# syzhang092218-source/dgppo

Measured on AMD Instinct MI355X. Metric: env-steps/sec whole node, LidarSpread n=8 4096 envs, 1/2/4/8 GPUs, higher is better.
Workload: dtype f32

## Files before the change

dgppo_amd/csrc/attn.hip:

```cpp
#include "nn_attn.h"

static int32_t attn_check(const dgppo_env_cfg* cfg, int F, int H, int Kp, int G, AttnArgs& a) {
  int32_t rc = dgppo_validate_cfg(cfg);
  if (rc) return rc;
  a.t = make_topo(*cfg);
  DGPPO_REQUIRE(F >= 1 && F <= 64 && H >= 1 && H <= 8, "attn: bad F=%d H=%d", F, H);
  DGPPO_REQUIRE(Kp >= F + H * (F + 4) + 1, "attn: Kp=%d too small", Kp);
  DGPPO_REQUIRE(G >= 0, "attn: G < 0");
  a.F = F; a.H = H; a.Kp = Kp; a.G = G;
  return 0;
}

enum class AttnFamily { SLOT8, BD, MFMA, VALU, TILED };
size_t attn_image_bytes(const Topo& t, int F, int H, bool bwd) {
  if (bwd)
    return sizeof(float) * ((size_t)t.Ns * (F + 1) + (size_t)t.n * H * (F + 1) + (size_t)t.n * t.S * 4 + 2 * (size_t)t.n * t.S * H +
                            (size_t)t.n * H * (F + 5));
  return sizeof(float) * ((size_t)t.Ns * (F + 1) + (size_t)t.n * H * (F + 1) + (size_t)t.n * t.S * 5 + (size_t)t.n * t.S * H);
}
static AttnFamily attn_family(const Topo& t, int F, int H, int Kp, bool bwd, bool dXa) {
  int PS = 0;
  bool hits = false;
  if (attn_image_bytes(t, F, H, bwd) > 64 * 1024) return AttnFamily::TILED;
  if ((Kp & 3) == 0 && attn_slot8_shape(t, F, H) && !(bwd && dXa)) return AttnFamily::SLOT8;
  if ((Kp & 3) == 0 && attn_bd_shape(t, F, H, PS, hits)) return AttnFamily::BD;
  if ((F & 3) == 0 && (Kp & 3) == 0 && t.S <= 64 && attn_mfma_smem(t, F, H, bwd) <= 64 * 1024 && (!bwd || F >= 16)) return AttnFamily::MFMA;
  return AttnFamily::VALU;
}

static int32_t attn_launch(AttnFamily fam, AttnArgs& a, void* stream, bool bwd, const char* who) {
  const hipStream_t s = (hipStream_t)stream;
  bool launched = true;
  switch (fam) {
    case AttnFamily::SLOT8: launched = launch_attn_slot8(a, s, bwd); break;
    case AttnFamily::BD: launched = launch_attn_bd(a, s, bwd); break;
    case AttnFamily::MFMA: launch_attn_wg(a, s, bwd, true); break;
    case AttnFamily::VALU: launch_attn_wg(a, s, bwd, false); break;
    case AttnFamily::TILED: {
      const int32_t rc = launch_attn_tiled(a, s, bwd);
      if (rc) return rc;
      break;
    }
  }
  DGPPO_REQUIRE(launched, "%s: dispatch failed", who);
  DGPPO_LAUNCH_CHECK();
  return 0;
}
static void attn_set_fwd(AttnArgs& a, const float* qt, const float* Xa, const float* Xo, const float* efeat, const float* emask,
                         float* zcat, float* attn) {
  a.qt = qt; a.Xa = Xa; a.Xo = Xo; a.efeat = efeat; a.emask = emask; a.zcat = zcat; a.attn = attn;
}
static void attn_set_bwd(AttnArgs& a, const float* dzcat, const float* attn, const float* qt, const float* Xa, const float* Xo,
                         const float* efeat, float* dqt, float* dXa, float* dXo) {
  a.dzcat = dzcat; a.attn = (float*)attn; a.qt = qt; a.Xa = Xa; a.Xo = Xo; a.efeat = efeat; a.dqt = dqt; a.dXa = dXa; a.dXo = dXo;
}

extern "C" int32_t dgppo_attn_fwd(const dgppo_env_cfg* cfg, int32_t F, int32_t H, int32_t Kp, const float* qt,
                                  const float* Xa, const float* Xo, const float* efeat, const float* emask, float* zcat,
                                  float* attn, int32_t G, void* stream) {
  AttnArgs a{};
  int32_t rc = attn_check(cfg, F, H, Kp, G, a);
  if (rc) return rc;
  if (G == 0) return 0;
  DGPPO_REQUIRE(qt && Xa && efeat && emask && zcat, "attn_fwd: NULL operand");
  DGPPO_REQUIRE(a.t.Ns == a.t.n || Xo, "attn_fwd: Xo is NULL");
  attn_set_fwd(a, qt, Xa, Xo, efeat, emask, zcat, attn);
  return attn_launch(attn_family(a.t, F, H, Kp, false, false), a, stream, false, "attn_fwd");
}

extern "C" int32_t dgppo_attn_bwd(const dgppo_env_cfg* cfg, int32_t F, int32_t H, int32_t Kp, const float* dzcat,
                                  const float* attn, const float* qt, const float* Xa, const float* Xo,
                                  const float* efeat, float* dqt, float* dXa, float* dXo, int32_t relu_xo, int32_t G,
                                  void* stream) {
  AttnArgs a{};
  int32_t rc = attn_check(cfg, F, H, Kp, G, a);
  if (rc) return rc;
  if (G == 0) return 0;
  DGPPO_REQUIRE(dzcat && attn && qt && Xa && efeat && dqt, "attn_bwd: NULL operand");
  DGPPO_REQUIRE(a.t.Ns == a.t.n || Xo, "attn_bwd: Xo is NULL");
  DGPPO_REQUIRE(!(dXo && !dXa), "attn_bwd: dXo needs dXa");
  attn_set_bwd(a, dzcat, attn, qt, Xa, Xo, efeat, dqt, dXa, dXo);
  const AttnFamily fam = attn_family(a.t, F, H, Kp, true, dXa != nullptr);
  a.relu_xo = (relu_xo && dXo && fam == AttnFamily::BD) ? 1 : 0;
  rc = attn_launch(fam, a, stream, true, "attn_bwd");
  if (rc) return rc;
  if (relu_xo && dXo && !a.relu_xo)
    return dgppo_relu_bwd(dXo, Xo, (int64_t)G * (a.t.Ns - a.t.n) * F, stream);
  return 0;
}

static bool attn_xo_ok(const Topo& t, int F, int H, int Kp) {
  return t.Ns > t.n && attn_family(t, F, H, Kp, true, true) == AttnFamily::BD;
}
extern "C" int32_t dgppo_attn_xo_supported(const dgppo_env_cfg* cfg, int32_t F, int32_t H, int32_t Kp) {
  AttnArgs a{};
  if (attn_check(cfg, F, H, Kp, 0, a)) return 0;
  return attn_xo_ok(a.t, F, H, Kp) ? 1 : 0;
}
static int32_t attn_set_xo(AttnArgs& a, const float* Xo_raw, const float* Wo, int ldwo, const float* bo, const char* who) {
  DGPPO_REQUIRE(attn_xo_ok(a.t, a.F, a.H, a.Kp), "%s: no fused kernel for this topology (ask dgppo_attn_xo_supported)", who);
  a.Xo_raw = Xo_raw; a.Wo = Wo; a.ldwo = ldwo; a.bo = bo;
  return 0;
}
extern "C" int32_t dgppo_attn_fwd_xo(const dgppo_env_cfg* cfg, int32_t F, int32_t H, int32_t Kp, const float* qt, const float* Xa,
                                     const float* Xo_raw, const float* Wo, int32_t ldwo, const float* bo, const float* efeat,
                                     const float* emask, float* zcat, float* attn, int32_t G, void* stream) {
  AttnArgs a{};
  int32_t rc = attn_check(cfg, F, H, Kp, G, a);
  if (rc) return rc;
  if (G == 0) return 0;
  DGPPO_REQUIRE(qt && Xa && Xo_raw && Wo && bo && efeat && emask && zcat, "attn_fwd_xo: NULL operand");
  DGPPO_REQUIRE(ldwo >= 32, "attn_fwd_xo: ldwo=%d < 32", ldwo);
  rc = attn_set_xo(a, Xo_raw, Wo, ldwo, bo, "attn_fwd_xo");
  if (rc) return rc;
  attn_set_fwd(a, qt, Xa, nullptr, efeat, emask, zcat, attn);
  return attn_launch(AttnFamily::BD, a, stream, false, "attn_fwd_xo");
}
extern "C" int32_t dgppo_attn_bwd_xo(const dgppo_env_cfg* cfg, int32_t F, int32_t H, int32_t Kp, const float* dzcat,
                                     const float* attn, const float* qt, const float* Xa, const float* Xo_raw, const float* Wo,
                                     int32_t ldwo, const float* bo, const float* efeat, float* dqt, float* dXa, float* dXo,
                                     int32_t relu_xo, int32_t G, void* stream) {
  AttnArgs a{};
  int32_t rc = attn_check(cfg, F, H, Kp, G, a);
  if (rc) return rc;
  if (G == 0) return 0;
  DGPPO_REQUIRE(dzcat && attn && qt && Xa && Xo_raw && Wo && bo && efeat && dqt, "attn_bwd_xo: NULL operand");
  DGPPO_REQUIRE(ldwo >= 32, "attn_bwd_xo: ldwo=%d < 32", ldwo);
  DGPPO_REQUIRE(!(dXo && !dXa), "attn_bwd_xo: dXo needs dXa");
  rc = attn_set_xo(a, Xo_raw, Wo, ldwo, bo, "attn_bwd_xo");
  if (rc) return rc;
  attn_set_bwd(a, dzcat, attn, qt, Xa, nullptr, efeat, dqt, dXa, dXo);
  a.relu_xo = (relu_xo && dXo) ? 1 : 0;
  return attn_launch(AttnFamily::BD, a, stream, true, "attn_bwd_xo");
}

static bool attn_rows_ok(const dgppo_env_cfg& c, const Topo& t, int F, int H, int Kp) {
  return attn_slot8_rows_ok(c, t, F, H) && attn_family(t, F, H, Kp, false, false) == AttnFamily::SLOT8 &&
         attn_family(t, F, H, Kp, true, false) == AttnFamily::SLOT8;
}
extern "C" int32_t dgppo_attn_rows_supported(const dgppo_env_cfg* cfg, int32_t F, int32_t H) {
  AttnArgs a{};
  const int Kp = (F + H * (F + 4) + 1 + 3) / 4 * 4;
  if (F < 1 || H < 1 || attn_check(cfg, F, H, Kp, 0, a)) return 0;
  return attn_rows_ok(*cfg, a.t, F, H, Kp) ? 1 : 0;
}
extern "C" int32_t dgppo_attn_fwd_rows(const dgppo_env_cfg* cfg, int32_t F, int32_t H, int32_t Kp, const float* qt,
                                       const float* Xa, const float* Xo, const float* emask, float* zcat, float* attn,
                                       int32_t G, void* stream) {
  AttnArgs a{};
  int32_t rc = attn_check(cfg, F, H, Kp, G, a);
  if (rc) return rc;
  DGPPO_REQUIRE(attn_rows_ok(*cfg, a.t, F, H, Kp), "attn_fwd_rows: no such kernel for this configuration (ask dgppo_attn_rows_supported)");
  if (G == 0) return 0;
  DGPPO_REQUIRE(qt && Xa && emask && zcat, "attn_fwd_rows: NULL operand");
  DGPPO_REQUIRE(a.t.Ns == a.t.n || Xo, "attn_fwd_rows: Xo is NULL");
  attn_set_fwd(a, qt, Xa, Xo, nullptr, emask, zcat, attn);
  return attn_launch(AttnFamily::SLOT8, a, stream, false, "attn_fwd_rows");
}
extern "C" int32_t dgppo_attn_bwd_rows(const dgppo_env_cfg* cfg, int32_t F, int32_t H, int32_t Kp, const float* dzcat,
                                       const float* attn, const float* qt, const float* emask, const float* Xa, const float* Xo,
                                       float* dqt, int32_t G, void* stream) {
  AttnArgs a{};
  int32_t rc = attn_check(cfg, F, H, Kp, G, a);
  if (rc) return rc;
  DGPPO_REQUIRE(attn_rows_ok(*cfg, a.t, F, H, Kp), "attn_bwd_rows: no such kernel for this configuration (ask dgppo_attn_rows_supported)");
  if (G == 0) return 0;
  DGPPO_REQUIRE(dzcat && Xa && dqt, "attn_bwd_rows: NULL operand");
  DGPPO_REQUIRE(attn || (qt && emask), "attn_bwd_rows: without attn the weights need qt and emask");
  DGPPO_REQUIRE(a.t.Ns == a.t.n || Xo, "attn_bwd_rows: Xo is NULL");
  attn_set_bwd(a, dzcat, attn, qt, Xa, Xo, nullptr, dqt, nullptr, nullptr);
  a.emask = emask;
  return attn_launch(AttnFamily::SLOT8, a, stream, true, "attn_bwd_rows");
}

extern "C" int64_t dgppo_attn_xo_workspace_bytes(int32_t G) { return G < 0 ? 0 : (int64_t)G * ABD_DW_STRIDE * (int64_t)sizeof(float); }
extern "C" int32_t dgppo_attn_bwd_xo_dw(const dgppo_env_cfg* cfg, int32_t F, int32_t H, int32_t Kp, const float* dzcat,
                                        const float* attn, const float* qt, const float* Xa, const float* Xo_raw, const float* Wo,
                                        int32_t ldwo, const float* bo, const float* efeat, float* dqt, float* dXa, float* dWo,
                                        int32_t lddwo, float* dbo, float* workspace, int64_t workspace_bytes, int32_t G,
                                        void* stream) {
  AttnArgs a{};
  int32_t rc = attn_check(cfg, F, H, Kp, G, a);
  if (rc) return rc;
  if (G == 0) return 0;
  DGPPO_REQUIRE(dzcat && attn && qt && Xa && Xo_raw && Wo && bo && efeat && dqt && dXa && dWo && dbo && workspace,
                "attn_bwd_xo_dw: NULL operand");
  DGPPO_REQUIRE(ldwo >= 32 && lddwo >= 32, "attn_bwd_xo_dw: ldwo=%d lddwo=%d < 32", ldwo, lddwo);
  DGPPO_REQUIRE(workspace_bytes >= dgppo_attn_xo_workspace_bytes(G) && (reinterpret_cast<uintptr_t>(workspace) & 15) == 0,
                "attn_bwd_xo_dw: workspace too small or not 16-byte aligned");
  rc = attn_set_xo(a, Xo_raw, Wo, ldwo, bo, "attn_bwd_xo_dw");
  if (rc) return rc;
  attn_set_bwd(a, dzcat, attn, qt, Xa, nullptr, efeat, dqt, dXa, nullptr);
  a.relu_xo = 1;
  a.dwo_slab = workspace;
  const bool launched = launch_attn_bd(a, (hipStream_t)stream, true);
  DGPPO_REQUIRE(launched, "attn_bwd_xo_dw: dispatch failed");
  launch_attn_xo_dw_reduce(workspace, G, dWo, lddwo, dbo, (hipStream_t)stream);
  DGPPO_LAUNCH_CHECK();
  return 0;
}
```

dgppo_amd/csrc/attn_bd.hip:

```cpp
#include "nn_attn.h"

#ifdef DGPPO_STAMPS
__device__ unsigned long long g_astamps[32];
#define ASTAMP(i) do { if (blockIdx.x == 0 && threadIdx.x == 0) g_astamps[i] = __builtin_amdgcn_s_memtime(); } while (0)
extern "C" int32_t dgppo_debug_stamps_attn(unsigned long long* out) {
  return (int32_t)hipMemcpyFromSymbol(out, HIP_SYMBOL(g_astamps), sizeof(unsigned long long) * 32);
}
#else
#define ASTAMP(i)
#endif

#define ABD_XL 36
#define ABD_DZL 40
__device__ inline f32x4g mfma4(float a_, float b_, f32x4g c_) { return __builtin_amdgcn_mfma_f32_4x4x1f32(a_, b_, c_, 0, 0, 0); }
__device__ inline const float* f4e(const float4& v) { return reinterpret_cast<const float*>(&v); }

__device__ inline int opaque_zero(int bits) {
  asm("v_and_b32 %0, 0, %0" : "+v"(bits));
  return bits;
}
__device__ inline int f4bits(const float4& v) { return __float_as_int(v.x) | __float_as_int(v.y) | __float_as_int(v.z) | __float_as_int(v.w); }

template <int PS, bool HITS> struct AbdLds {
  static constexpr int NSP = PS * 8, PC = NSP + (HITS ? 8 : 0), PL = PC + 4;
  static constexpr int XS = NSP * ABD_XL, XH = HITS ? 64 * ABD_XL + 64 : 0;
  static constexpr int QP = (32 * ABD_XL > 32 * PL) ? 32 * ABD_XL : 32 * PL;
  static constexpr int FWD = XS + XH + QP;
  static constexpr int DZ = 32 * ABD_DZL, PTL = NSP + 1, PT = 32 * PTL, DL = 32 * PL;
  static constexpr int BWD = XS + XH + DZ + PT + DL;
};

#define ABD_KR 8
template <int GT> struct AbdXoRegs { float ag[GT][2], ah[4][2], wo[2][2], bo[2]; };
template <int GT, bool HITS>
__device__ inline void abd_xo_load(AbdXoRegs<GT>& x, const AttnArgs& a, const float* raw, int n_shared_other, int ng, int hit0,
                                   int n_hits, int li, int lq, bool first) {
  if (first) {
#pragma unroll
    for (int s_ = 0; s_ < 2; ++s_)
#pragma unroll
      for (int ct = 0; ct < 2; ++ct) x.wo[s_][ct] = a.Wo[(lq + 4 * s_) * a.ldwo + ct * 16 + li];
#pragma unroll
    for (int ct = 0; ct < 2; ++ct) x.bo[ct] = a.bo[ct * 16 + li];
#pragma unroll
    for (int t = 0; t < GT; ++t) {
      int o = t * 16 + li;
      o = o < n_shared_other ? o : n_shared_other - 1;
      o = o < 0 ? 0 : o;
#pragma unroll
      for (int s_ = 0; s_ < 2; ++s_) x.ag[t][s_] = raw[o * ABD_KR + lq + 4 * s_];
    }
  }
  if constexpr (HITS) {
#pragma unroll
    for (int t = 0; t < 4; ++t) {
      int hb = hit0 + t * 16 + li;
      hb = hb < n_hits ? hb : n_hits - 1;
#pragma unroll
      for (int s_ = 0; s_ < 2; ++s_) x.ah[t][s_] = raw[(ng + hb) * ABD_KR + lq + 4 * s_];
    }
  }
}
template <int GT, bool HITS>
__device__ inline void abd_xo_emit(const AbdXoRegs<GT>& x, float* XS, float* XH, int n, int n_shared_other, int li, int lq, bool first) {
  auto tile = [&](const float (&ar)[2], f32x4g (&v)[2]) {
#pragma unroll
    for (int ct = 0; ct < 2; ++ct) {
      v[ct] = f32x4g{0.f, 0.f, 0.f, 0.f};
      v[ct] = __builtin_amdgcn_mfma_f32_16x16x4f32(ar[0], x.wo[0][ct], v[ct], 0, 0, 0);
      v[ct] = __builtin_amdgcn_mfma_f32_16x16x4f32(ar[1], x.wo[1][ct], v[ct], 0, 0, 0);
    }
  };
  if (first) {
#pragma unroll
    for (int t = 0; t < GT; ++t) {
      f32x4g v[2];
      tile(x.ag[t], v);
#pragma unroll
      for (int ct = 0; ct < 2; ++ct)
#pragma unroll
        for (int r = 0; r < 4; ++r) {
          const int o = t * 16 + lq * 4 + r;
          if (o < n_shared_other) XS[(n + o) * ABD_XL + ct * 16 + li] = relu_nan(v[ct][r] + x.bo[ct]);
        }
    }
  }
  if constexpr (HITS) {
#pragma unroll
    for (int t = 0; t < 4; ++t) {
      f32x4g v[2];
      tile(x.ah[t], v);
#pragma unroll
      for (int ct = 0; ct < 2; ++ct)
#pragma unroll
        for (int r = 0; r < 4; ++r) {
          const int hr = t * 16 + lq * 4 + r;
          XH[hr * ABD_XL + (hr >> 3) * 8 + ct * 16 + li] = relu_nan(v[ct][r] + x.bo[ct]);
        }
    }
  }
}
template <int GT> __device__ inline int abd_xo_bits(const AbdXoRegs<GT>& x, bool hits) {
  int b = 0;
#pragma unroll
  for (int t = 0; t < GT; ++t) b |= __float_as_int(x.ag[t][0]) | __float_as_int(x.ag[t][1]);
  if (hits) {
#pragma unroll
    for (int t = 0; t < 4; ++t) b |= __float_as_int(x.ah[t][0]) | __float_as_int(x.ah[t][1]);
  }
  b |= __float_as_int(x.wo[0][0]) | __float_as_int(x.wo[0][1]) | __float_as_int(x.wo[1][0]) | __float_as_int(x.wo[1][1]);
  b |= __float_as_int(x.bo[0]) | __float_as_int(x.bo[1]);
  return b;
}

template <int PS, bool HITS>
__device__ __forceinline__ int abd_slot(const Topo& t, int NSH, int ic, int p, int sub) {
  if (HITS && p == PS) return t.n + t.gs + sub;
  const int j = p * 8 + sub;
  return (j < NSH) ? slot_of(t, j, ic) : -1;
}

template <int PS, bool HITS, int AB, bool XOF>
__global__ void __launch_bounds__(128) attn_fwd_bd_kernel(AttnArgs a) {
  extern __shared__ float4 abd_sm[];
  using L = AbdLds<PS, HITS>;
  constexpr int F = 32, NSP = L::NSP, PC = L::PC, PL = L::PL, NPR = PS + (HITS ? 1 : 0), Wd = F + 4;
  const Topo& t = a.t;
  const int lane = threadIdx.x & 63, wave = threadIdx.x >> 6;
  const int g = __builtin_amdgcn_readfirstlane(blockIdx.x * 2 + wave);
  if (g >= a.G) return;
  const int n = t.n, S = t.S, Ns = t.Ns, H = a.H, Kp = a.Kp;
  const int NSH = HITS ? t.n + t.ng : Ns;
  const int kc = F + H * Wd;
  float* XS = reinterpret_cast<float*>(abd_sm) + wave * L::FWD;
  float* XH = XS + L::XS;
  float* QP = XH + L::XH;
  const float4* Xa4 = reinterpret_cast<const float4*>(a.Xa + (size_t)g * n * F);
  const float4* Xo4 = reinterpret_cast<const float4*>(a.Xo + (size_t)g * (Ns - n) * F);
  const float4* qt4 = reinterpret_cast<const float4*>(a.qt + (size_t)g * n * H * F);
  float* zc = a.zcat + (size_t)g * n * Kp;
  const int il = lane >> 3, sub = lane & 7, g2 = (lane >> 2) & 1, c = lane & 3, hA = lane & 3;
  ASTAMP(0);
  float4 vs[PS];
#pragma unroll
  for (int p = 0; p < PS; ++p) {
    const int row = p * 8 + il;
    const int ra = row < n ? row : n - 1, ro = (row < NSH ? row : NSH - 1) - n;
    const float4* src = (XOF || row < n || NSH == n) ? Xa4 + ra * 8 + sub : Xo4 + ro * 8 + sub;
    vs[p] = *src;
  }
  constexpr int GT = (NSP + 15) / 16;
  AbdXoRegs<GT> xo;
  const float* raw = XOF ? a.Xo_raw + (size_t)g * (Ns - n) * ABD_KR : nullptr;
  const int li_ = lane & 15, lq_ = lane >> 4;
  const float* mk = a.emask + (size_t)g * n * S;
  const float4* ef4 = reinterpret_cast<const float4*>(a.efeat + (size_t)g * n * S * 4);
  float* at = a.attn + (size_t)g * n * S * H;
#pragma unroll
  for (int ab = 0; ab < AB; ++ab) {
    const int i = ab * 8 + il;
    const bool live = i < n;
    const int ic = live ? i : n - 1;
    float4 vh[HITS ? 8 : 1], vq[4];
    if constexpr (XOF) abd_xo_load<GT, HITS>(xo, a, raw, NSH - n, t.ng, ab * 64, n * 8, li_, lq_, ab == 0);
    if constexpr (HITS && !XOF) {
#pragma unroll
      for (int k = 0; k < 8; ++k) {
        int hb = ab * 64 + k * 8 + il;
        hb = hb < n * 8 ? hb : n * 8 - 1;
        vh[k] = Xo4[(t.ng + hb) * 8 + sub];
      }
    }
#pragma unroll
    for (int k = 0; k < 4; ++k) {
      const int row = k * 8 + il;
      int ri = ab * 8 + (row >> 2), rh = row & 3;
      ri = ri < n ? ri : n - 1; rh = rh < H ? rh : H - 1;
      vq[k] = qt4[(ri * H + rh) * 8 + sub];
    }
    int slot[NPR];
    float mkv[NPR];
    float4 efv[NPR];
#pragma unroll
    for (int p = 0; p < NPR; ++p) {
      const int sl = abd_slot<PS, HITS>(t, NSH, ic, p, sub);
      slot[p] = live ? sl : -1;
      const int sc = sl < 0 ? 0 : sl;
      mkv[p] = mk[ic * S + sc];
      efv[p] = ef4[ic * S + sc];
    }
    ASTAMP(1);
    int pin = 0;
#pragma unroll
    for (int p = 0; p < NPR; ++p) pin |= __float_as_int(mkv[p]) | f4bits(efv[p]);
    if constexpr (XOF) pin |= abd_xo_bits<GT>(xo, HITS);
    const int pin0 = opaque_zero(pin);
    if (ab == 0) {
#pragma unroll
      for (int p = 0; p < PS; ++p) {
        float4 v = vs[p];
        if (XOF && p * 8 + il >= n) v = make_float4(0.f, 0.f, 0.f, 0.f);
        *reinterpret_cast<float4*>(XS + pin0 + (p * 8 + il) * ABD_XL + sub * 4) = v;
      }
    }
    if constexpr (XOF) abd_xo_emit<GT, HITS>(xo, XS + pin0, XH + pin0, n, NSH - n, li_, lq_, ab == 0);
    if constexpr (HITS && !XOF) {
#pragma unroll
      for (int k = 0; k < 8; ++k) *reinterpret_cast<float4*>(XH + pin0 + (k * 8 + il) * ABD_XL + k * 8 + sub * 4) = vh[k];
    }
#pragma unroll
    for (int k = 0; k < 4; ++k) *reinterpret_cast<float4*>(QP + pin0 + (k * 8 + il) * ABD_XL + sub * 4) = vq[k];
#pragma unroll
    for (int p = 0; p < NPR; ++p) mkv[p] = (slot[p] >= 0) ? mkv[p] : 0.0f;
    if constexpr (HITS) {
      if (mkv[PS] == 0.0f) {
#pragma unroll
        for (int k = 0; k < 8; ++k) *reinterpret_cast<float4*>(XH + lane * ABD_XL + il * 8 + k * 4) = make_float4(0.f, 0.f, 0.f, 0.f);
      }
    }
    ASTAMP(2);
    f32x4g acc[NPR];
#pragma unroll
    for (int p = 0; p < NPR; ++p) acc[p] = f32x4g{0.f, 0.f, 0.f, 0.f};
    {
      const float* qrow = QP + (il * 4 + hA) * ABD_XL;
#pragma unroll
      for (int k = 0; k < 8; ++k) {
        const float4 q = *reinterpret_cast<const float4*>(qrow + k * 4);
        float4 x[NPR];
#pragma unroll
        for (int p = 0; p < NPR; ++p) {
          if (HITS && p == PS) x[p] = *reinterpret_cast<const float4*>(XH + lane * ABD_XL + il * 8 + k * 4);
          else x[p] = *reinterpret_cast<const float4*>(XS + (p * 8 + sub) * ABD_XL + k * 4);
        }
#pragma unroll
        for (int u = 0; u < 4; ++u)
#pragma unroll
          for (int p = 0; p < NPR; ++p) acc[p] = mfma4(f4e(q)[u], f4e(x[p])[u], acc[p]);
      }
    }
    ASTAMP(3);
    float* PT = QP;
#pragma unroll
    for (int h = 0; h < 4; ++h) {
      if (h < H) {
        float l[NPR];
        float mx = -INFINITY;
#pragma unroll
        for (int p = 0; p < NPR; ++p) { l[p] = (mkv[p] != 0.0f) ? acc[p][h] : -INFINITY; mx = fmaxf(mx, l[p]); }
        mx = grp8_max(mx);
        float den = 0.0f;
#pragma unroll
        for (int p = 0; p < NPR; ++p) { l[p] = (l[p] == -INFINITY) ? 0.0f : __expf(l[p] - mx); den += l[p]; }
        den = grp8_sum(den);
        const float inv = (den > 0.0f) ? 1.0f / den : 0.0f;
        float z0 = 0.f, z1 = 0.f, z2 = 0.f, z3 = 0.f;
#pragma unroll
        for (int p = 0; p < NPR; ++p) {
          const float av = l[p] * inv;
          acc[p][h] = av;
          if (slot[p] >= 0) {
            if (a.attn != nullptr) at[(i * S + slot[p]) * H + h] = av;
            if (av != 0.0f) {
              const float4 e = efv[p];
              z0 = fmaf(av, e.x, z0); z1 = fmaf(av, e.y, z1); z2 = fmaf(av, e.z, z2); z3 = fmaf(av, e.w, z3);
            }
          }
        }
        z0 = grp8_sum(z0); z1 = grp8_sum(z1); z2 = grp8_sum(z2); z3 = grp8_sum(z3);
        if (live && sub == 0) *reinterpret_cast<float4*>(zc + i * Kp + F + h * Wd + F) = make_float4(z0, z1, z2, z3);
      } else {
#pragma unroll
        for (int p = 0; p < NPR; ++p) acc[p][h] = 0.0f;
      }
#pragma unroll
      for (int p = 0; p < NPR; ++p) PT[(il * 4 + h) * PL + p * 8 + sub] = acc[p][h];
    }
    ASTAMP(4);
    {
      float pa[PC];
#pragma unroll
      for (int k = 0; k < PC / 4; ++k) {
        const float4 v = *reinterpret_cast<const float4*>(PT + (il * 4 + hA) * PL + k * 4);
        pa[k * 4] = v.x; pa[k * 4 + 1] = v.y; pa[k * 4 + 2] = v.z; pa[k * 4 + 3] = v.w;
      }
      f32x4g az[4];
#pragma unroll
      for (int q = 0; q < 4; ++q) az[q] = f32x4g{0.f, 0.f, 0.f, 0.f};
      const int fq = (g2 * 4 + c) * 4;
#pragma unroll
      for (int kk = 0; kk < NSP; ++kk) {
        const float4 b = *reinterpret_cast<const float4*>(XS + kk * ABD_XL + fq);
#pragma unroll
        for (int q = 0; q < 4; ++q) az[q] = mfma4(pa[kk], f4e(b)[q], az[q]);
      }
      if constexpr (HITS) {
#pragma unroll
        for (int m = 0; m < 8; ++m) {
          const float4 b = *reinterpret_cast<const float4*>(XH + (il * 8 + m) * ABD_XL + il * 8 + fq);
#pragma unroll
          for (int q = 0; q < 4; ++q) az[q] = mfma4(pa[NSP + m], f4e(b)[q], az[q]);
        }
      }
      if (live) {
#pragma unroll
        for (int h = 0; h < 4; ++h)
          if (h < H) *reinterpret_cast<float4*>(zc + i * Kp + F + h * Wd + fq) = make_float4(az[0][h], az[1][h], az[2][h], az[3][h]);
      }
    }
  }
  ASTAMP(5);
#pragma unroll
  for (int p = 0; p < PS; ++p) {
    const int row = p * 8 + il;
    if (row < n) *reinterpret_cast<float4*>(zc + row * Kp + sub * 4) = *reinterpret_cast<const float4*>(XS + row * ABD_XL + sub * 4);
  }
  {
    const int wpad = Kp - kc;
    for (int i = lane; i < n; i += 64)
      for (int cc = 0; cc < wpad; ++cc) zc[i * Kp + kc + cc] = (cc == 0) ? ones_col(a.t, mk + i * S) : 0.0f;
  }
  ASTAMP(6);
}

template <int PS, bool HITS, bool XOF>
struct AbdFwdRegs {
  float4 vs[PS], vq[4], vh[(HITS && !XOF) ? 8 : 1];
  AbdXoRegs<(PS * 8 + 15) / 16> xo;
  float mkv[PS + (HITS ? 1 : 0)];
  float4 efv[PS + (HITS ? 1 : 0)];
};
template <int PS, bool HITS, bool XOF>
__global__ void __launch_bounds__(128) attn_fwd_bdp_kernel(AttnArgs a) {
  extern __shared__ float4 abd_sm[];
  using L = AbdLds<PS, HITS>;
  constexpr int F = 32, NSP = L::NSP, PC = L::PC, PL = L::PL, NPR = PS + (HITS ? 1 : 0), Wd = F + 4, GT = (NSP + 15) / 16;
  const Topo& t = a.t;
  const int lane = threadIdx.x & 63, wave = threadIdx.x >> 6;
  int g = __builtin_amdgcn_readfirstlane(blockIdx.x * 2 + wave);
  const int stride = gridDim.x * 2;
  if (g >= a.G) return;
  const int n = t.n, S = t.S, Ns = t.Ns, H = a.H, Kp = a.Kp;
  const int NSH = HITS ? t.n + t.ng : Ns;
  const int kc = F + H * Wd;
  float* XS = reinterpret_cast<float*>(abd_sm) + wave * L::FWD;
  float* XH = XS + L::XS;
  float* QP = XH + L::XH;
  const int il = lane >> 3, sub = lane & 7, g2 = (lane >> 2) & 1, c = lane & 3, hA = lane & 3;
  const int li_ = lane & 15, lq_ = lane >> 4;
  const int i = il;
  const bool live = i < n;
  const int ic = live ? i : n - 1;
  int slot[NPR], sc[NPR];
#pragma unroll
  for (int p = 0; p < NPR; ++p) {
    const int sl = abd_slot<PS, HITS>(t, NSH, ic, p, sub);
    slot[p] = live ? sl : -1;
    sc[p] = sl < 0 ? 0 : sl;
  }
  using Regs = AbdFwdRegs<PS, HITS, XOF>;
  auto load = [&](int gg, Regs& R) {
    const float4* Xa4 = reinterpret_cast<const float4*>(a.Xa + (size_t)gg * n * F);
    const float4* Xo4 = reinterpret_cast<const float4*>(a.Xo + (size_t)gg * (Ns - n) * F);
    const float4* qt4 = reinterpret_cast<const float4*>(a.qt + (size_t)gg * n * H * F);
#pragma unroll
    for (int p = 0; p < PS; ++p) {
      const int row = p * 8 + il;
      const int ra = row < n ? row : n - 1, ro = (row < NSH ? row : NSH - 1) - n;
      const float4* src = (XOF || row < n || NSH == n) ? Xa4 + ra * 8 + sub : Xo4 + ro * 8 + sub;
      R.vs[p] = *src;
    }
    if constexpr (XOF) abd_xo_load<GT, HITS>(R.xo, a, a.Xo_raw + (size_t)gg * (Ns - n) * ABD_KR, NSH - n, t.ng, 0, n * 8, li_, lq_, true);
    if constexpr (HITS && !XOF) {
#pragma unroll
      for (int k = 0; k < 8; ++k) {
        int hb = k * 8 + il;
        hb = hb < n * 8 ? hb : n * 8 - 1;
        R.vh[k] = Xo4[(t.ng + hb) * 8 + sub];
      }
    }
#pragma unroll
    for (int k = 0; k < 4; ++k) {
      const int row = k * 8 + il;
      int ri = row >> 2, rh = row & 3;
      ri = ri < n ? ri : n - 1; rh = rh < H ? rh : H - 1;
      R.vq[k] = qt4[(ri * H + rh) * 8 + sub];
    }
    const float* mk = a.emask + (size_t)gg * n * S;
    const float4* ef4 = reinterpret_cast<const float4*>(a.efeat + (size_t)gg * n * S * 4);
#pragma unroll
    for (int p = 0; p < NPR; ++p) {
      R.mkv[p] = mk[ic * S + sc[p]];
      R.efv[p] = ef4[ic * S + sc[p]];
    }
  };
  auto stage = [&](Regs& R) {
    int pin = 0;
#pragma unroll
    for (int p = 0; p < NPR; ++p) pin |= __float_as_int(R.mkv[p]) | f4bits(R.efv[p]);
    if constexpr (XOF) pin |= abd_xo_bits<GT>(R.xo, HITS);
    const int pin0 = opaque_zero(pin);
#pragma unroll
    for (int p = 0; p < PS; ++p) {
      float4 v = R.vs[p];
      if (XOF && p * 8 + il >= n) v = make_float4(0.f, 0.f, 0.f, 0.f);
      *reinterpret_cast<float4*>(XS + pin0 + (p * 8 + il) * ABD_XL + sub * 4) = v;
    }
    if constexpr (XOF) abd_xo_emit<GT, HITS>(R.xo, XS + pin0, XH + pin0, n, NSH - n, li_, lq_, true);
    if constexpr (HITS && !XOF) {
#pragma unroll
      for (int k = 0; k < 8; ++k) *reinterpret_cast<float4*>(XH + pin0 + (k * 8 + il) * ABD_XL + k * 8 + sub * 4) = R.vh[k];
    }
#pragma unroll
    for (int k = 0; k < 4; ++k) *reinterpret_cast<float4*>(QP + pin0 + (k * 8 + il) * ABD_XL + sub * 4) = R.vq[k];
#pragma unroll
    for (int p = 0; p < NPR; ++p) R.mkv[p] = (slot[p] >= 0) ? R.mkv[p] : 0.0f;
    if constexpr (HITS) {
      if (R.mkv[PS] == 0.0f) {
#pragma unroll
        for (int k = 0; k < 8; ++k) *reinterpret_cast<float4*>(XH + lane * ABD_XL + il * 8 + k * 4) = make_float4(0.f, 0.f, 0.f, 0.f);
      }
    }
  };
  auto compute = [&](int gg, const Regs& R) {
    float* zc = a.zcat + (size_t)gg * n * Kp;
    float* at = a.attn + (size_t)gg * n * S * H;
    f32x4g acc[NPR];
#pragma unroll
    for (int p = 0; p < NPR; ++p) acc[p] = f32x4g{0.f, 0.f, 0.f, 0.f};
    {
      const float* qrow = QP + (il * 4 + hA) * ABD_XL;
#pragma unroll
      for (int k = 0; k < 8; ++k) {
        const float4 q = *reinterpret_cast<const float4*>(qrow + k * 4);
        float4 x[NPR];
#pragma unroll
        for (int p = 0; p < NPR; ++p) {
          if (HITS && p == PS) x[p] = *reinterpret_cast<const float4*>(XH + lane * ABD_XL + il * 8 + k * 4);
          else x[p] = *reinterpret_cast<const float4*>(XS + (p * 8 + sub) * ABD_XL + k * 4);
        }
#pragma unroll
        for (int u = 0; u < 4; ++u)
#pragma unroll
          for (int p = 0; p < NPR; ++p) acc[p] = mfma4(f4e(q)[u], f4e(x[p])[u], acc[p]);
      }
    }
    float* PT = QP;
#pragma unroll
    for (int h = 0; h < 4; ++h) {
      if (h < H) {
        float l[NPR];
        float mx = -INFINITY;
#pragma unroll
        for (int p = 0; p < NPR; ++p) { l[p] = (R.mkv[p] != 0.0f) ? acc[p][h] : -INFINITY; mx = fmaxf(mx, l[p]); }
        mx = grp8_max(mx);
        float den = 0.0f;
#pragma unroll
        for (int p = 0; p < NPR; ++p) { l[p] = (l[p] == -INFINITY) ? 0.0f : __expf(l[p] - mx); den += l[p]; }
        den = grp8_sum(den);
        const float inv = (den > 0.0f) ? 1.0f / den : 0.0f;
        float z0 = 0.f, z1 = 0.f, z2 = 0.f, z3 = 0.f;
#pragma unroll
        for (int p = 0; p < NPR; ++p) {
          const float av = l[p] * inv;
          acc[p][h] = av;
          if (slot[p] >= 0) {
            if (a.attn != nullptr) at[(i * S + slot[p]) * H + h] = av;
            if (av != 0.0f) {
              const float4 e = R.efv[p];
              z0 = fmaf(av, e.x, z0); z1 = fmaf(av, e.y, z1); z2 = fmaf(av, e.z, z2); z3 = fmaf(av, e.w, z3);
            }
          }
        }
        z0 = grp8_sum(z0); z1 = grp8_sum(z1); z2 = grp8_sum(z2); z3 = grp8_sum(z3);
        if (live && sub == 0) *reinterpret_cast<float4*>(zc + i * Kp + F + h * Wd + F) = make_float4(z0, z1, z2, z3);
      } else {
#pragma unroll
        for (int p = 0; p < NPR; ++p) acc[p][h] = 0.0f;
      }
#pragma unroll
      for (int p = 0; p < NPR; ++p) PT[(il * 4 + h) * PL + p * 8 + sub] = acc[p][h];
    }
    {
      float pa[PC];
#pragma unroll
      for (int k = 0; k < PC / 4; ++k) {
        const float4 v = *reinterpret_cast<const float4*>(PT + (il * 4 + hA) * PL + k * 4);
        pa[k * 4] = v.x; pa[k * 4 + 1] = v.y; pa[k * 4 + 2] = v.z; pa[k * 4 + 3] = v.w;
      }
      f32x4g az[4];
#pragma unroll
      for (int q = 0; q < 4; ++q) az[q] = f32x4g{0.f, 0.f, 0.f, 0.f};
      const int fq = (g2 * 4 + c) * 4;
#pragma unroll
      for (int kk = 0; kk < NSP; ++kk) {
        const float4 b = *reinterpret_cast<const float4*>(XS + kk * ABD_XL + fq);
#pragma unroll
        for (int q = 0; q < 4; ++q) az[q] = mfma4(pa[kk], f4e(b)[q], az[q]);
      }
      if constexpr (HITS) {
#pragma unroll
        for (int m = 0; m < 8; ++m) {
          const float4 b = *reinterpret_cast<const float4*>(XH + (il * 8 + m) * ABD_XL + il * 8 + fq);
#pragma unroll
          for (int q = 0; q < 4; ++q) az[q] = mfma4(pa[NSP + m], f4e(b)[q], az[q]);
        }
      }
      if (live) {
#pragma unroll
        for (int h = 0; h < 4; ++h)
          if (h < H) *reinterpret_cast<float4*>(zc + i * Kp + F + h * Wd + fq) = make_float4(az[0][h], az[1][h], az[2][h], az[3][h]);
      }
    }
#pragma unroll
    for (int p = 0; p < PS; ++p) {
      const int row = p * 8 + il;
      if (row < n) *reinterpret_cast<float4*>(zc + row * Kp + sub * 4) = *reinterpret_cast<const float4*>(XS + row * ABD_XL + sub * 4);
    }
    {
      const int wpad = Kp - kc;
      for (int ii = lane; ii < n; ii += 64)
        for (int cc = 0; cc < wpad; ++cc) zc[ii * Kp + kc + cc] = (cc == 0) ? ones_col(a.t, a.emask + ((size_t)gg * n + ii) * a.t.S) : 0.0f;
    }
  };
  Regs cur;
  load(g, cur);
  for (;;) {
    stage(cur);
    const int gn = g + stride;
    const bool more = gn < a.G;
    Regs nxt;
    if (more) load(gn, nxt);
    compute(g, cur);
    if (!more) break;
    cur = nxt;
    g = gn;
  }
}

template <int PS, bool HITS, int AB, bool XOF>
__global__ void __launch_bounds__(64) attn_bwd_bd_kernel(AttnArgs a) {
  extern __shared__ float4 abd_sm[];
  using L = AbdLds<PS, HITS>;
  constexpr int F = 32, NSP = L::NSP, PC = L::PC, PL = L::PL, PTL = L::PTL, NPR = PS + (HITS ? 1 : 0), Wd = F + 4;
  constexpr int RTS = (NSP + 15) / 16;
  const Topo& t = a.t;
  const int lane = threadIdx.x & 63;
  const int g = blockIdx.x;
  if (g >= a.G) return;
  const int n = t.n, S = t.S, Ns = t.Ns, H = a.H, Kp = a.Kp;
  const int NSH = HITS ? t.n + t.ng : Ns;
  float* XS = reinterpret_cast<float*>(abd_sm);
  float* XH = XS + L::XS;
  float* DZ = XH + L::XH;
  float* PT = DZ + L::DZ;
  float* DL = PT + L::PT;
  const float4* Xa4 = reinterpret_cast<const float4*>(a.Xa + (size_t)g * n * F);
  const float4* Xo4 = reinterpret_cast<const float4*>(a.Xo + (size_t)g * (Ns - n) * F);
  const float* qt = a.qt + (size_t)g * n * H * F;
  const float* dzc = a.dzcat + (size_t)g * n * Kp;
  const bool want_dx = a.dXa != nullptr;
  const int il = lane >> 3, sub = lane & 7, g2 = (lane >> 2) & 1, c = lane & 3, hA = lane & 3;
  const int li = lane & 15, lq = lane >> 4;
  float4 vs[PS];
#pragma unroll
  for (int p = 0; p < PS; ++p) {
    const int row = p * 8 + il;
    const int ra = row < n ? row : n - 1, ro = (row < NSH ? row : NSH - 1) - n;
    const float4* src = (XOF || row < n || NSH == n) ? Xa4 + ra * 8 + sub : Xo4 + ro * 8 + sub;
    vs[p] = *src;
  }
  constexpr int GT = (NSP + 15) / 16;
  AbdXoRegs<GT> xo;
  const float* raw = XOF ? a.Xo_raw + (size_t)g * (Ns - n) * ABD_KR : nullptr;
  const int li_ = lane & 15, lq_ = lane >> 4;
  float dir[RTS][2][4];
#pragma unroll
  for (int rt = 0; rt < RTS; ++rt)
#pragma unroll
    for (int ft = 0; ft < 2; ++ft)
#pragma unroll
      for (int r = 0; r < 4; ++r) {
        const int node = rt * 16 + lq * 4 + r;
        dir[rt][ft][r] = dzc[(node < n ? node : n - 1) * Kp + ft * 16 + li];
      }
  f32x4g dxs[RTS][2];
#pragma unroll
  for (int rt = 0; rt < RTS; ++rt)
#pragma unroll
    for (int ft = 0; ft < 2; ++ft) dxs[rt][ft] = f32x4g{0.f, 0.f, 0.f, 0.f};
  f32x4g dwacc[2] = {f32x4g{0.f, 0.f, 0.f, 0.f}, f32x4g{0.f, 0.f, 0.f, 0.f}};
  float rbg[NSP / 4];
  const float4* ef4 = reinterpret_cast<const float4*>(a.efeat + (size_t)g * n * S * 4);
  const float* at = a.attn + (size_t)g * n * S * H;
#pragma unroll
  for (int ab = 0; ab < AB; ++ab) {
    const int i = ab * 8 + il;
    const bool live = i < n;
    const int ic = live ? i : n - 1;
    float4 vh[HITS ? 8 : 1], vz[5];
    if constexpr (XOF) abd_xo_load<GT, HITS>(xo, a, raw, NSH - n, t.ng, ab * 64, n * 8, li_, lq_, ab == 0);
    float rbh[HITS ? 16 : 1];
    if constexpr (XOF && HITS) {
#pragma unroll
      for (int s_ = 0; s_ < 16; ++s_) {
        int hb = ab * 64 + s_ * 4 + lq;
        hb = hb < n * 8 ? hb : n * 8 - 1;
        rbh[s_] = raw[(t.ng + hb) * ABD_KR + (li & 7)];
      }
    }
    if constexpr (XOF) {
      if (ab == 0) {
#pragma unroll
        for (int s_ = 0; s_ < NSP / 4; ++s_) {
          int o = s_ * 4 + lq;
          o = o < NSH - n ? o : NSH - n - 1;
          o = o < 0 ? 0 : o;
          rbg[s_] = raw[o * ABD_KR + (li & 7)];
        }
      }
    }
    if constexpr (HITS && !XOF) {
#pragma unroll
      for (int k = 0; k < 8; ++k) {
        int hb = ab * 64 + k * 8 + il;
        hb = hb < n * 8 ? hb : n * 8 - 1;
        vh[k] = Xo4[(t.ng + hb) * 8 + sub];
      }
    }
#pragma unroll
    for (int k = 0; k < 5; ++k) {
      int tt = k * 64 + lane;
      tt = tt < 288 ? tt : 287;
      const int row = tt / 9, ch = tt - row * 9;
      int ri = ab * 8 + (row >> 2), rh = row & 3;
      ri = ri < n ? ri : n - 1; rh = rh < H ? rh : H - 1;
      vz[k] = *reinterpret_cast<const float4*>(dzc + ri * Kp + F + rh * Wd + ch * 4);
    }
    int slot[NPR];
    float4 efv[NPR];
    float av[NPR][4];
#pragma unroll
    for (int p = 0; p < NPR; ++p) {
      const int sl = abd_slot<PS, HITS>(t, NSH, ic, p, sub);
      slot[p] = live ? sl : -1;
      const int sc = sl < 0 ? 0 : sl;
      efv[p] = ef4[ic * S + sc];
#pragma unroll
      for (int h = 0; h < 4; ++h) av[p][h] = at[(ic * S + sc) * H + (h < H ? h : H - 1)];
    }
    float4 q8[4][2];
    if constexpr (HITS) {
#pragma unroll
      for (int h = 0; h < 4; ++h) {
        const float4* qr = reinterpret_cast<const float4*>(qt + (size_t)(ic * H + (h < H ? h : H - 1)) * F + c * 8);
        q8[h][0] = qr[0]; q8[h][1] = qr[1];
      }
    }
    float bQ[8][2];
#pragma unroll
    for (int ks = 0; ks < 8; ++ks) {
      const int ri = ab * 8 + ks;
      const float* qr = qt + (size_t)((ri < n ? ri : n - 1) * H + (lq < H ? lq : H - 1)) * F;
#pragma unroll
      for (int ft = 0; ft < 2; ++ft) bQ[ks][ft] = qr[ft * 16 + li];
    }
    int pin = 0;
#pragma unroll
    for (int p = 0; p < NPR; ++p) {
      pin |= f4bits(efv[p]);
#pragma unroll
      for (int h = 0; h < 4; ++h) pin |= __float_as_int(av[p][h]);
    }
    if constexpr (HITS) {
#pragma unroll
      for (int h = 0; h < 4; ++h) pin |= f4bits(q8[h][0]) | f4bits(q8[h][1]);
    }
#pragma unroll
    for (int ks = 0; ks < 8; ++ks) pin |= __float_as_int(bQ[ks][0]) | __float_as_int(bQ[ks][1]);
    if (ab == 0) {
#pragma unroll
      for (int rt = 0; rt < RTS; ++rt)
#pragma unroll
        for (int ft = 0; ft < 2; ++ft)
#pragma unroll
          for (int r = 0; r < 4; ++r) pin |= __float_as_int(dir[rt][ft][r]);
    }
    if constexpr (XOF) pin |= abd_xo_bits<GT>(xo, HITS);
    if constexpr (XOF && HITS) {
#pragma unroll
      for (int s_ = 0; s_ < 16; ++s_) pin |= __float_as_int(rbh[s_]);
    }
    if constexpr (XOF) {
      if (ab == 0) {
#pragma unroll
        for (int s_ = 0; s_ < NSP / 4; ++s_) pin |= __float_as_int(rbg[s_]);
      }
    }
    const int pin0 = opaque_zero(pin);
    if (ab == 0) {
#pragma unroll
      for (int p = 0; p < PS; ++p) {
        float4 v = vs[p];
        if (XOF && p * 8 + il >= n) v = make_float4(0.f, 0.f, 0.f, 0.f);
        *reinterpret_cast<float4*>(XS + pin0 + (p * 8 + il) * ABD_XL + sub * 4) = v;
      }
    }
    if constexpr (XOF) abd_xo_emit<GT, HITS>(xo, XS + pin0, XH + pin0, n, NSH - n, li_, lq_, ab == 0);
    if constexpr (HITS && !XOF) {
#pragma unroll
      for (int k = 0; k < 8; ++k) *reinterpret_cast<float4*>(XH + pin0 + (k * 8 + il) * ABD_XL + k * 8 + sub * 4) = vh[k];
    }
#pragma unroll
    for (int k = 0; k < 5; ++k) {
      const int tt = k * 64 + lane, row = tt / 9, ch = tt - row * 9;
      if (tt < 288) *reinterpret_cast<float4*>(DZ + pin0 + row * ABD_DZL + ch * 4) = vz[k];
    }
#pragma unroll
    for (int p = 0; p < NPR; ++p)
#pragma unroll
      for (int h = 0; h < 4; ++h) av[p][h] = (slot[p] >= 0 && h < H) ? av[p][h] : 0.0f;
    if constexpr (HITS) {
      if (av[PS][0] == 0.0f && av[PS][1] == 0.0f && av[PS][2] == 0.0f && av[PS][3] == 0.0f) {
#pragma unroll
        for (int k = 0; k < 8; ++k) *reinterpret_cast<float4*>(XH + lane * ABD_XL + il * 8 + k * 4) = make_float4(0.f, 0.f, 0.f, 0.f);
      }
    }
    f32x4g acc[NPR];
#pragma unroll
    for (int p = 0; p < NPR; ++p) acc[p] = f32x4g{0.f, 0.f, 0.f, 0.f};
    {
      const float* zrow = DZ + (il * 4 + hA) * ABD_DZL;
#pragma unroll
      for (int k = 0; k < 8; ++k) {
        const float4 q = *reinterpret_cast<const float4*>(zrow + k * 4);
        float4 x[NPR];
#pragma unroll
        for (int p = 0; p < NPR; ++p) {
          if (HITS && p == PS) x[p] = *reinterpret_cast<const float4*>(XH + lane * ABD_XL + il * 8 + k * 4);
          else x[p] = *reinterpret_cast<const float4*>(XS + (p * 8 + sub) * ABD_XL + k * 4);
        }
#pragma unroll
        for (int u = 0; u < 4; ++u)
#pragma unroll
          for (int p = 0; p < NPR; ++p) acc[p] = mfma4(f4e(q)[u], f4e(x[p])[u], acc[p]);
      }
    }
#pragma unroll
    for (int h = 0; h < 4; ++h) {
      const float4 dze = *reinterpret_cast<const float4*>(DZ + (il * 4 + h) * ABD_DZL + F);
      float dot = 0.0f;
#pragma unroll
      for (int p = 0; p < NPR; ++p) {
        const float w = av[p][h];
        const float4 e = efv[p];
        const float dA = (w != 0.0f) ? acc[p][h] + fmaf(dze.x, e.x, fmaf(dze.y, e.y, fmaf(dze.z, e.z, dze.w * e.w))) : 0.0f;
        acc[p][h] = dA;
        dot = fmaf(w, dA, dot);
      }
      dot = grp8_sum(dot);
#pragma unroll
      for (int p = 0; p < NPR; ++p) {
        acc[p][h] = av[p][h] * (acc[p][h] - dot);
        DL[(il * 4 + h) * PL + p * 8 + sub] = acc[p][h];
        if (p < PS) PT[(il * 4 + h) * PTL + p * 8 + sub] = av[p][h];
      }
    }
    {
      float pa[PC];
#pragma unroll
      for (int k = 0; k < PC / 4; ++k) {
        const float4 v = *reinterpret_cast<const float4*>(DL + (il * 4 + hA) * PL + k * 4);
        pa[k * 4] = v.x; pa[k * 4 + 1] = v.y; pa[k * 4 + 2] = v.z; pa[k * 4 + 3] = v.w;
      }
      f32x4g az[4];
#pragma unroll
      for (int q = 0; q < 4; ++q) az[q] = f32x4g{0.f, 0.f, 0.f, 0.f};
      const int fq = (g2 * 4 + c) * 4;
#pragma unroll
      for (int kk = 0; kk < NSP; ++kk) {
        const float4 b = *reinterpret_cast<const float4*>(XS + kk * ABD_XL + fq);
#pragma unroll
        for (int q = 0; q < 4; ++q) az[q] = mfma4(pa[kk], f4e(b)[q], az[q]);
      }
      if constexpr (HITS) {
#pragma unroll
        for (int m = 0; m < 8; ++m) {
          const float4 b = *reinterpret_cast<const float4*>(XH + (il * 8 + m) * ABD_XL + il * 8 + fq);
#pragma unroll
          for (int q = 0; q < 4; ++q) az[q] = mfma4(pa[NSP + m], f4e(b)[q], az[q]);
        }
      }
      if (live) {
        float* dq = a.dqt + ((size_t)g * n + i) * H * F;
#pragma unroll
        for (int h = 0; h < 4; ++h)
          if (h < H) *reinterpret_cast<float4*>(dq + h * F + fq) = make_float4(az[0][h], az[1][h], az[2][h], az[3][h]);
      }
    }
    if (want_dx) {
#pragma unroll
      for (int ks = 0; ks < 8; ++ks) {
        const int prow = ks * 4 + lq;
        float bD[2];
#pragma unroll
        for (int ft = 0; ft < 2; ++ft) bD[ft] = DZ[prow * ABD_DZL + ft * 16 + li];
#pragma unroll
        for (int rt = 0; rt < RTS; ++rt) {
          const int col = (rt * 16 + li < NSP) ? rt * 16 + li : NSP - 1;
          const float aP = PT[prow * PTL + col], aL = DL[prow * PL + col];
#pragma unroll
          for (int ft = 0; ft < 2; ++ft) {
            dxs[rt][ft] = __builtin_amdgcn_mfma_f32_16x16x4f32(aP, bD[ft], dxs[rt][ft], 0, 0, 0);
            dxs[rt][ft] = __builtin_amdgcn_mfma_f32_16x16x4f32(aL, bQ[ks][ft], dxs[rt][ft], 0, 0, 0);
          }
        }
      }
      if constexpr (HITS) {
        if (a.dXo != nullptr || (XOF && a.dwo_slab != nullptr)) {
          f32x4g af[8];
#pragma unroll
          for (int q = 0; q < 8; ++q) af[q] = f32x4g{0.f, 0.f, 0.f, 0.f};
#pragma unroll
          for (int h = 0; h < 4; ++h) {
            const float4 d0 = *reinterpret_cast<const float4*>(DZ + (il * 4 + h) * ABD_DZL + c * 8);
            const float4 d1 = *reinterpret_cast<const float4*>(DZ + (il * 4 + h) * ABD_DZL + c * 8 + 4);
            const float pw = av[PS][h], dw = acc[PS][h];
#pragma unroll
            for (int q = 0; q < 4; ++q) {
              af[q] = mfma4(pw, f4e(d0)[q], af[q]);
              af[q + 4] = mfma4(pw, f4e(d1)[q], af[q + 4]);
              af[q] = mfma4(dw, f4e(q8[h][0])[q], af[q]);
              af[q + 4] = mfma4(dw, f4e(q8[h][1])[q], af[q + 4]);
            }
          }
          float4 x0[4], x1[4];
#pragma unroll
          for (int m = 0; m < 4; ++m) {
            const float* xr = XH + (il * 8 + g2 * 4 + m) * ABD_XL + il * 8 + c * 8;
            x0[m] = *reinterpret_cast<const float4*>(xr);
            x1[m] = *reinterpret_cast<const float4*>(xr + 4);
          }
          const bool to_slab = XOF && a.dwo_slab != nullptr;
#pragma unroll
          for (int m = 0; m < 4; ++m) {
            const int hb = ab * 64 + il * 8 + g2 * 4 + m;
            float4 v0 = make_float4(af[0][m], af[1][m], af[2][m], af[3][m]);
            float4 v1 = make_float4(af[4][m], af[5][m], af[6][m], af[7][m]);
            if (a.relu_xo || to_slab) {
              v0.x = x0[m].x > 0.f ? v0.x : 0.f; v0.y = x0[m].y > 0.f ? v0.y : 0.f; v0.z = x0[m].z > 0.f ? v0.z : 0.f; v0.w = x0[m].w > 0.f ? v0.w : 0.f;
              v1.x = x1[m].x > 0.f ? v1.x : 0.f; v1.y = x1[m].y > 0.f ? v1.y : 0.f; v1.z = x1[m].z > 0.f ? v1.z : 0.f; v1.w = x1[m].w > 0.f ? v1.w : 0.f;
            }
            if (to_slab) {
              float* xr = XH + (il * 8 + g2 * 4 + m) * ABD_XL + il * 8 + c * 8;
              *reinterpret_cast<float4*>(xr) = v0;
              *reinterpret_cast<float4*>(xr + 4) = v1;
            } else if (hb < n * 8) {
              float* o = a.dXo + ((size_t)g * (Ns - n) + t.ng + hb) * F + c * 8;
              *reinterpret_cast<float4*>(o) = v0;
              *reinterpret_cast<float4*>(o + 4) = v1;
            }
          }
          if constexpr (XOF) {
            if (to_slab) {
#pragma unroll
              for (int s_ = 0; s_ < 16; ++s_) {
                const int hr = s_ * 4 + lq;
                const float bv = li < 8 ? rbh[s_] : (li == 8 ? 1.0f : 0.0f);
#pragma unroll
                for (int ft = 0; ft < 2; ++ft) {
                  const float av_ = XH[hr * ABD_XL + (hr >> 3) * 8 + ft * 16 + li];
                  dwacc[ft] = __builtin_amdgcn_mfma_f32_16x16x4f32(av_, bv, dwacc[ft], 0, 0, 0);
                }
              }
            }
          }
        }
      }
    }
  }
  if (want_dx) {
    float xm[RTS][2][4];
#pragma unroll
    for (int rt = 0; rt < RTS; ++rt)
#pragma unroll
      for (int ft = 0; ft < 2; ++ft)
#pragma unroll
        for (int r = 0; r < 4; ++r) {
          const int node = rt * 16 + lq * 4 + r;
          xm[rt][ft][r] = (node < NSP) ? XS[node * ABD_XL + ft * 16 + li] : 0.0f;
        }
#pragma unroll
    for (int rt = 0; rt < RTS; ++rt)
#pragma unroll
      for (int ft = 0; ft < 2; ++ft)
#pragma unroll
        for (int r = 0; r < 4; ++r) {
          const int node = rt * 16 + lq * 4 + r, f = ft * 16 + li;
          float v = dxs[rt][ft][r];
          if (node < n) a.dXa[((size_t)g * n + node) * F + f] = v + dir[rt][ft][r];
          else if (XOF && a.dwo_slab != nullptr) {
            if (node < NSP) XS[node * ABD_XL + f] = (node < NSH && xm[rt][ft][r] > 0.0f) ? v : 0.0f;
          } else if (node < NSH && a.dXo != nullptr) {
            if (a.relu_xo) v = (xm[rt][ft][r] > 0.0f) ? v : 0.0f;
            a.dXo[((size_t)g * (Ns - n) + (node - n)) * F + f] = v;
          }
        }
    if constexpr (XOF) {
      if (a.dwo_slab != nullptr) {
        const int nsho = NSH - n;
#pragma unroll
        for (int s_ = 0; s_ < NSP / 4; ++s_) {
          const int o = s_ * 4 + lq;
          const float bv = li < 8 ? rbg[s_] : (li == 8 ? 1.0f : 0.0f);
#pragma unroll
          for (int ft = 0; ft < 2; ++ft) {
            const int node = n + o;
            const float av_ = (o < nsho && node < NSP) ? XS[(node < NSP ? node : NSP - 1) * ABD_XL + ft * 16 + li] : 0.0f;
            dwacc[ft] = __builtin_amdgcn_mfma_f32_16x16x4f32(av_, bv, dwacc[ft], 0, 0, 0);
          }
        }
        if (li <= 8) {
          float* o = a.dwo_slab + (size_t)g * ABD_DW_STRIDE + li * 32 + lq * 4;
#pragma unroll
          for (int ft = 0; ft < 2; ++ft)
            *reinterpret_cast<float4*>(o + ft * 16) = make_float4(dwacc[ft][0], dwacc[ft][1], dwacc[ft][2], dwacc[ft][3]);
        }
      }
    }
  }
}

bool attn_bd_shape(const Topo& t, int F, int H, int& PS, bool& hits) {
  if (F != 32 || H < 1 || H > 4 || t.n > 16) return false;
  const int n_priv = t.Ns - t.n - t.ng;
  hits = t.lidar && n_priv > 0;
  if (hits && (t.per != 8 || n_priv != t.n * 8)) return false;
  const int nsh = hits ? t.n + t.ng : t.Ns;
  PS = (nsh + 7) / 8;
  return PS >= 1 && PS <= 4;
}
template <int PS, bool HITS, int AB, bool XOF>
static void launch_attn_bd_x(const AttnArgs& a, hipStream_t s, bool bwd) {
  using L = AbdLds<PS, HITS>;
  if (bwd) { hipLaunchKernelGGL((attn_bwd_bd_kernel<PS, HITS, AB, XOF>), dim3(a.G), dim3(64), sizeof(float) * L::BWD, s, a); return; }
  if constexpr (AB == 1) {
    static thread_local int cap = 0;
    if (cap == 0) {
      int per_cu = 0, dev = 0, cus = 256;
      if (hipOccupancyMaxActiveBlocksPerMultiprocessor(&per_cu, reinterpret_cast<const void*>(&attn_fwd_bdp_kernel<PS, HITS, XOF>), 128,
                                                       sizeof(float) * 2 * L::FWD) != hipSuccess || per_cu < 1) per_cu = 1;
      if (hipGetDevice(&dev) != hipSuccess || hipDeviceGetAttribute(&cus, hipDeviceAttributeMultiprocessorCount, dev) != hipSuccess ||
          cus < 1) cus = 256;
      cap = per_cu * cus;
    }
    if ((a.G + 1) / 2 > 2 * cap) {
      hipLaunchKernelGGL((attn_fwd_bdp_kernel<PS, HITS, XOF>), dim3(cap), dim3(128), sizeof(float) * 2 * L::FWD, s, a);
      return;
    }
  }
  hipLaunchKernelGGL((attn_fwd_bd_kernel<PS, HITS, AB, XOF>), dim3((a.G + 1) / 2), dim3(128), sizeof(float) * 2 * L::FWD, s, a);
}
template <int PS, bool HITS, int AB>
static void launch_attn_bd_one(const AttnArgs& a, hipStream_t s, bool bwd) {
  if (a.Xo_raw != nullptr) launch_attn_bd_x<PS, HITS, AB, true>(a, s, bwd);
  else launch_attn_bd_x<PS, HITS, AB, false>(a, s, bwd);
}
bool launch_attn_bd(const AttnArgs& a, hipStream_t s, bool bwd) {
  int PS = 0;
  bool hits = false;
  if (!attn_bd_shape(a.t, a.F, a.H, PS, hits)) return false;
  const int AB = (a.t.n + 7) / 8;
  switch ((PS * 2 + (hits ? 1 : 0)) * 4 + AB) {
#define DGPPO_BD(P, HT, B) case ((P) * 2 + (HT)) * 4 + (B): launch_attn_bd_one<P, (HT) != 0, B>(a, s, bwd); return true;
    DGPPO_BD(1, 0, 1) DGPPO_BD(1, 1, 1) DGPPO_BD(2, 0, 1) DGPPO_BD(2, 1, 1) DGPPO_BD(2, 0, 2) DGPPO_BD(2, 1, 2)
    DGPPO_BD(3, 0, 1) DGPPO_BD(3, 1, 1) DGPPO_BD(3, 0, 2) DGPPO_BD(3, 1, 2)
    DGPPO_BD(4, 0, 1) DGPPO_BD(4, 1, 1) DGPPO_BD(4, 0, 2) DGPPO_BD(4, 1, 2)
#undef DGPPO_BD
    default: return false;
  }
}

__global__ void __launch_bounds__(320) attn_xo_dw_reduce_kernel(const float* slab, int G, float* dWo, int lddwo, float* dbo) {
  const int e = threadIdx.x;
  if (e >= 288) return;
  const int per = (G + gridDim.x - 1) / gridDim.x;
  const int g0 = blockIdx.x * per, g1 = min(G, g0 + per);
  float sacc[8] = {0.f, 0.f, 0.f, 0.f, 0.f, 0.f, 0.f, 0.f};
  int g = g0;
  for (; g + 7 < g1; g += 8) {
#pragma unroll
    for (int u = 0; u < 8; ++u) sacc[u] += slab[(size_t)(g + u) * ABD_DW_STRIDE + e];
  }
  for (; g < g1; ++g) sacc[0] += slab[(size_t)g * ABD_DW_STRIDE + e];
  const float sum = ((sacc[0] + sacc[1]) + (sacc[2] + sacc[3])) + ((sacc[4] + sacc[5]) + (sacc[6] + sacc[7]));
  if (g0 >= g1) return;
  if (e < 256) atomicAdd(dWo + (size_t)(e >> 5) * lddwo + (e & 31), sum);
  else atomicAdd(dbo + (e - 256), sum);
}
void launch_attn_xo_dw_reduce(const float* slab, int G, float* dWo, int lddwo, float* dbo, hipStream_t s) {
  int blocks = (G + 31) / 32;
  blocks = blocks < 1 ? 1 : (blocks > 1024 ? 1024 : blocks);
  hipLaunchKernelGGL(attn_xo_dw_reduce_kernel, dim3(blocks), dim3(320), 0, s, slab, G, dWo, lddwo, dbo);
}
```

dgppo_amd/csrc/nn_attn.h:

```cpp
#pragma once
#include "graph_topo.h"

__device__ inline int slot_of(const Topo& t, int nd, int i) {
  if (nd < t.n) return nd;
  if (nd < t.n + t.ng) {
    const int g = nd - t.n;
    return t.spread ? t.n + g : (g == i ? t.n : -1);
  }
  const int q = nd - t.n - t.ng;
  if (t.lidar) return (q / t.per == i) ? t.n + t.gs + (q - i * t.per) : -1;
  return t.n + t.gs + q;
}

__device__ inline float ones_col(const Topo& t, const float* mrow) {
  if (t.gs > 0) return 1.0f;
  for (int s = 0; s < t.S; ++s)
    if (mrow[s] != 0.0f) return 1.0f;
  return 0.0f;
}

#define ABD_DW_STRIDE 320
struct AttnArgs {
  Topo t;
  int F, H, Kp;
  const float* qt;
  const float* Xa;
  const float* Xo;
  const float* efeat;
  const float* emask;
  float* zcat;
  float* attn;
  const float* dzcat;
  float* dqt;
  float* dXa;
  float* dXo;
  int relu_xo;
  int G;
  const float* Xo_raw; const float* Wo; const float* bo; int ldwo;
  float* dwo_slab;
  int TI;
};

using f32x4g = __attribute__((ext_vector_type(4))) float;

template <typename FA, typename FB, typename FC>
__device__ inline void mfma_tiles(int RTn, int CTn, int K4, int wave, int lane, FA fa, FB fb, FC fc) {
  const int li = lane & 15, lq = lane >> 4;
  for (int tile = wave; tile < RTn * CTn; tile += 4) {
    const int rt = tile / CTn, ct = tile - rt * CTn;
    f32x4g acc = {0.f, 0.f, 0.f, 0.f};
    int k4 = 0;
    for (; k4 + 4 <= K4; k4 += 4) {
      float av[4], bv[4];
#pragma unroll
      for (int u = 0; u < 4; ++u) { av[u] = fa(rt * 16 + li, (k4 + u) * 4 + lq); bv[u] = fb((k4 + u) * 4 + lq, ct * 16 + li); }
#pragma unroll
      for (int u = 0; u < 4; ++u) acc = __builtin_amdgcn_mfma_f32_16x16x4f32(av[u], bv[u], acc, 0, 0, 0);
    }
    for (; k4 < K4; ++k4) acc = __builtin_amdgcn_mfma_f32_16x16x4f32(fa(rt * 16 + li, k4 * 4 + lq), fb(k4 * 4 + lq, ct * 16 + li), acc, 0, 0, 0);
#pragma unroll
    for (int r = 0; r < 4; ++r) fc(rt * 16 + lq * 4 + r, ct * 16 + li, acc[r]);
  }
}

__device__ inline void put4(float* d, float4 v) { d[0] = v.x; d[1] = v.y; d[2] = v.z; d[3] = v.w; }

template <int CTRL> __device__ inline float dpp_f(float v) {
  return __int_as_float(__builtin_amdgcn_update_dpp(0, __float_as_int(v), CTRL, 0xf, 0xf, false));
}
__device__ inline float grp8_sum(float v) {
  v += dpp_f<0xB1>(v);
  v += dpp_f<0x4E>(v);
  v += dpp_f<0x141>(v);
  return v;
}
__device__ inline float grp8_max(float v) {
  v = fmaxf(v, dpp_f<0xB1>(v));
  v = fmaxf(v, dpp_f<0x4E>(v));
  v = fmaxf(v, dpp_f<0x141>(v));
  return v;
}

#pragma GCC visibility push(hidden)
size_t attn_image_bytes(const Topo& t, int F, int H, bool bwd);
size_t attn_mfma_smem(const Topo& t, int F, int H, bool bwd);
void launch_attn_wg(const AttnArgs& a, hipStream_t s, bool bwd, bool mfma);
bool attn_slot8_shape(const Topo& t, int F, int H);
bool attn_slot8_rows_ok(const dgppo_env_cfg& c, const Topo& t, int F, int H);
bool launch_attn_slot8(const AttnArgs& a, hipStream_t s, bool bwd);
bool attn_bd_shape(const Topo& t, int F, int H, int& PS, bool& hits);
bool launch_attn_bd(const AttnArgs& a, hipStream_t s, bool bwd);
void launch_attn_xo_dw_reduce(const float* slab, int G, float* dWo, int lddwo, float* dbo, hipStream_t s);
int32_t launch_attn_tiled(AttnArgs& a, hipStream_t s, bool bwd);
#pragma GCC visibility pop
```

dgppo_amd/engine.py:

```python
from __future__ import annotations

import dataclasses
from typing import Callable, Dict, Optional

import numpy as np
import os
import torch

from . import _native as N
from . import nets
from . import ops_algo as OA
from . import ops_env as OE
from . import ops_nn as K
from .utils import checkpoint as CK


@dataclasses.dataclass
class Hyper:
    gamma: float = 0.99
    gae_lambda: float = 0.95
    clip_eps: float = 0.25
    coef_ent: float = 1e-2
    max_grad_norm: float = 2.0
    lr_actor: float = 3e-4
    lr_Vl: float = 1e-3
    lr_Vh: float = 1e-3
    batch_size: int = 16384
    rnn_step: int = 16
    alpha: float = 10.0
    cbf_eps: float = 1e-2
    cbf_weight: float = 1.0
    cbf_schedule: bool = True
    train_steps: int = 100000
    actor_gnn_layers: int = 2
    Vl_gnn_layers: int = 2
    Vh_gnn_layers: int = 1
    use_rnn: bool = True
    use_lstm: bool = False
    rnn_layers: int = 1
    lagr_init: float = 0.78
    lr_lagr: float = 1e-7
    cost_weight: float = 0.0
    cost_schedule: bool = False


class RolloutData:

    def __init__(self, cfg: N.EnvCfg, B: int, T: int, device, stochastic: bool, carry_dim: int = nets.HID):
        n = cfg.n_agents
        self.cfg, self.B, self.T, self.stochastic = cfg, B, T, stochastic
        z = lambda *s: torch.empty(*s, device=device)
        step, env = OE.record_fields(cfg)
        self.step_tm = {k: z(T + 1, B, *shape) for k, shape in step.items()}
        self.env = {k: z(B, *shape) for k, shape in env.items()}
        self.step: Dict[str, torch.Tensor] = {}
        for k in OE.STEP_FIELDS:
            setattr(self, k + "_tm", self.step_tm.get(k))
            setattr(self, k, None)
        for k in OE.ENV_FIELDS:
            setattr(self, k, self.env.get(k))
        self.action_tm = z(T, B, n, 2)
        self.log_pi_tm = z(T, B, n) if stochastic else None
        self.rnn_tm = z(T + 1, B, n, carry_dim)
        self.reward_tm = z(T, B)
        self.cost_tm = z(T, B, n, cfg.n_cost)
        self._env_major = False
        views = {k: v.unbind(0) for k, v in self.step_tm.items()}
        self.states_tm = [OE.State({k: v[t] for k, v in views.items()}, self.env) for t in range(T + 1)]

    def finalize(self):
        if self._env_major:
            return self

        def tr(name, x):
            if x is None:
                return None
            cur = getattr(self, name, None)
            want = (x.shape[1], x.shape[0]) + tuple(x.shape[2:])
            if cur is None or tuple(cur.shape) != want:
                cur = torch.empty(want, device=x.device, dtype=x.dtype)
            cur.copy_(x.transpose(0, 1))
            return cur
        for k, v in self.step_tm.items():
            self.step[k] = tr(k, v)
            setattr(self, k, self.step[k])
        self.actions = tr("actions", self.action_tm)
        self.log_pis = tr("log_pis", self.log_pi_tm) if self.stochastic else None
        T, x = self.T, self.rnn_tm
        want = (x.shape[1], T + 2) + tuple(x.shape[2:])
        cur = getattr(self, "_rnn_em", None)
        if cur is None or tuple(cur.shape) != want:
            cur = torch.empty(want, device=x.device, dtype=x.dtype)
        cur[:, :T + 1].copy_(x.transpose(0, 1))
        self._rnn_em = cur
        self.rnn_states = self._rnn_em[:, :T] if self.stochastic else self._rnn_em[:, 1:T + 1]
        self.rewards = tr("rewards", self.reward_tm)
        self.costs = tr("costs", self.cost_tm)
        self._env_major = True
        return self


class OptState:
    def __init__(self, n: int, device):
        self.m = torch.zeros(n, device=device)
        self.v = torch.zeros(n, device=device)
        self.state = torch.zeros(N.OPT_STATE_FLOATS, device=device)


class Engine:
    def __init__(self, cfg: N.EnvCfg, hyper: Hyper, device, T: int = 128,
                 allreduce: Optional[Callable[[torch.Tensor], None]] = None, world: int = 1, prepass_graphs: int = 1 << 20,
                 use_graphs: bool = False, multi_stream: bool = False, algo: str = "dgppo", rank: int = 0,
                 fused_step: bool = True, lean_attn0: bool = True):
        self.cfg, self.hp, self.device, self.T = cfg, hyper, device, T
        assert algo in ("dgppo", "informarl", "hcbfcrpo", "informarl_lagr"), algo
        self.algo = algo
        self.use_graphs = use_graphs and os.environ.get("DGPPO_HIPGRAPH", "1") != "0"
        self.multi_stream = multi_stream and os.environ.get("DGPPO_MULTI_STREAM", "1") != "0"
        self._side_streams = None
        self.fused_step = bool(fused_step) and OE.act_step_feats_supported(cfg, nets.input_width(cfg), nets.H_HEADS)
        self.lean_attn0 = bool(lean_attn0)
        self._ro_cache: Dict[tuple, dict] = {}
        self._upd_graph: dict = {}
        self.n_cost = cfg.n_cost
        spec = [("policy", "policy", hyper.actor_gnn_layers, 2), ("Vl", "Vl", hyper.Vl_gnn_layers, 1)]
        if algo == "dgppo":
            spec.append(("Vh", "Vh", hyper.Vh_gnn_layers, self.n_cost))
        elif algo == "informarl_lagr":
            spec.append(("Vh", "Vhg", hyper.Vh_gnn_layers, self.n_cost))
        def rnn_kw(name):
            if not hyper.use_rnn:
                return dict(rnn="none", rnn_layers=0)
            if name == "Vh" and algo == "dgppo":
                return dict(rnn="gru", rnn_layers=1)
            return dict(rnn="lstm" if hyper.use_lstm else "gru", rnn_layers=hyper.rnn_layers)
        sizes = [nets.make_layout(kind, cfg.node_dim, layers, n_out, **rnn_kw(k)).size for k, kind, layers, n_out in spec]
        offs, tot = [], 0
        for sz in sizes:
            offs.append(tot)
            tot += (sz + 3) // 4 * 4
        self.flat_grads = torch.zeros(tot + 4 * 8, device=device)
        self.n_reduced = tot + 3 * 8
        self.stats = self.flat_grads[tot:tot + 32].view(4, 8)
        built = {k: nets.Net(kind, cfg, layers, n_out, device, grads=self.flat_grads[o:o + sz], lean_attn0=self.lean_attn0, **rnn_kw(k))
                 for (k, kind, layers, n_out), o, sz in zip(spec, offs, sizes)}
        if algo == "informarl_lagr":
            self.lagr = torch.full((cfg.n_agents, self.n_cost), float(hyper.lagr_init), device=device)
            self.lagr_sums = torch.zeros(cfg.n_agents * self.n_cost, device=device)
        self.policy, self.Vl, self.Vh = built["policy"], built["Vl"], built.get("Vh")
        self.HC = self.policy.carry_dim
        self.opt = {k: OptState(net.layout.size, device) for k, net in self.nets.items()}
        self.arena = nets.Arena(device)
        self.allreduce = allreduce
        self.world, self.rank = int(world), int(rank)
        assert self.world >= 1 and (allreduce is not None or self.world == 1), "world > 1 needs an allreduce"
        assert 0 <= self.rank < self.world, f"rank {rank} outside world {world}"
        self.prepass_graphs = int(os.environ.get("DGPPO_PREPASS_GRAPHS", prepass_graphs))
        self.lam_pow = OA.lam_pow_table(hyper.gae_lambda, T, device)
        self.eps_hat = torch.zeros(cfg.n_agents, 2, device=device)
        self.reset_failed = torch.zeros(1, dtype=torch.int32, device=device)
        self.grad_hook: Optional[Callable[[str, nets.Net, int], None]] = None
        self._mb = 0

    @property
    def nets(self) -> Dict[str, nets.Net]:
        d = {"policy": self.policy, "Vl": self.Vl}
        if self.Vh is not None:
            d["Vh"] = self.Vh
        return d

    def set_entropy_noise(self, seed: int):
        OE.randn(seed, 0, self.eps_hat.view(-1))

    _CFG_IDENTITY = ("kind", "n_agents", "n_obs", "n_rays", "top_k", "node_dim", "n_cost")

    def _identity(self) -> dict:
        ident = {"algo": CK.encode_str(self.algo)}
        ident.update({f"cfg.{k}": int(getattr(self.cfg, k)) for k in self._CFG_IDENTITY})
        for f in dataclasses.fields(Hyper):
            v = getattr(self.hp, f.name)
            ident[f"hyper.{f.name}"] = int(v) if isinstance(v, (bool, int)) else float(v)
        ident["T"], ident["world"] = int(self.T), int(self.world)
        ident.update({f"size.{k}": int(net.layout.size) for k, net in self.nets.items()})
        return ident

    def _state_tensors(self) -> Dict[str, torch.Tensor]:
        t = {}
        for k, net in self.nets.items():
            opt = self.opt[k]
            t.update({f"{k}/params": net.params, f"{k}/m": opt.m, f"{k}/v": opt.v, f"{k}/state": opt.state})
        t["eps_hat"] = self.eps_hat
        if self.algo == "informarl_lagr":
            t["lagr"] = self.lagr
        return t

    def state_dict(self) -> dict:
        out = {"identity": self._identity()}
        for path, x in self._state_tensors().items():
            node = out
            *dirs, leaf = path.split("/")
            for d in dirs:
                node = node.setdefault(d, {})
            node[leaf] = x.detach().cpu().numpy().copy()
        return out

    def load_state_dict(self, d: dict) -> None:
        mine, theirs = self._identity(), d.get("identity", {})
        show = lambda v: repr(CK.decode_str(v)) if isinstance(v, np.ndarray) else repr(v)
        for k, v in mine.items():
            if k not in theirs:
                raise ValueError(f"state dict does not fit this engine: it has no identity field '{k}'")
            if not np.array_equal(np.asarray(v), np.asarray(theirs[k])):
                raise ValueError(f"state dict does not fit this engine: '{k}' is {show(theirs[k])} there, {show(v)} here")
        src = {}
        for path, x in self._state_tensors().items():
            node = d
            for part in path.split("/"):
                node = node.get(part) if isinstance(node, dict) else None
            if not isinstance(node, np.ndarray) or node.dtype != np.float32 or node.shape != tuple(x.shape):
                raise ValueError(f"state dict does not fit this engine: '{path}' is not a float32 array of shape {tuple(x.shape)}")
            src[path] = node
        for path, x in self._state_tensors().items():
            x.copy_(torch.from_numpy(src[path]).to(self.device))
        for net in self.nets.values():
            net.prepare()

    def _feats(self, tag, st: OE.State, n_env, n_time=1, slots=1, env_ids=None):
        f = nets.GraphFeats(self.cfg, n_env * n_time, self.arena, tag)
        return f.compute_record(st.step, slots, st.env, env_ids, n_env, n_time)

    def _rollout_steps(self, ro: RolloutData, eps, B: int, stochastic: bool, start: int = 0):
        cfg, T, n = self.cfg, ro.T, self.cfg.n_agents
        tag = "ro" if stochastic else "rod"
        if self.fused_step:
            pol, R = self.policy, B * n
            feats = self._feats(tag, ro.states_tm[start], B)
            Mcat, cvec = pol.pp("gnn0.Mcat"), pol.pp("gnn0.cvec")
            qt0 = pol.arena.get(f"{tag}.qt0", R, Mcat.shape[1])
            K.dense_fwd(feats.Xa, Mcat, cvec, qt0)
            for t in range(start, T):
                act = pol.forward(feats, n_seq=R, T=1, h0=ro.rnn_tm[t].view(R, self.HC), tag=tag,
                                  hs_out=ro.rnn_tm[t + 1].view(R, self.HC), train=False, qt0=qt0)
                nxt = dict(Xa=feats.Xa, Xo=feats.Xo, efeat=feats.efeat, emask=feats.emask, Fp=feats.Fp, Mcat=Mcat, cvec=cvec,
                           qt0=qt0, H=nets.H_HEADS) if t + 1 < T else {}
                OE.act_step_feats(cfg, ro.states_tm[t], act["ms"], eps[t] if stochastic else None, ro.action_tm[t],
                                  ro.log_pi_tm[t] if stochastic else None, ro.states_tm[t + 1], ro.reward_tm[t], ro.cost_tm[t],
                                  **nxt)
                feats.edges_from_rows = cfg.state_dim == 4
            return
        for t in range(start, T):
            feats = self._feats(tag, ro.states_tm[t], B)
            act = self.policy.forward(feats, n_seq=B * n, T=1, h0=ro.rnn_tm[t].view(B * n, self.HC), tag=tag,
                                      hs_out=ro.rnn_tm[t + 1].view(B * n, self.HC), train=False)
            a_t = ro.action_tm[t].view(B * n, 2)
            if stochastic:
                K.policy_head(act["ms"], eps[t], None, a_t, ro.log_pi_tm[t].view(B * n), None, n, 0)
            else:
                K.policy_head(act["ms"], None, None, a_t, None, None, n, 1)
            OE.step(cfg, ro.states_tm[t], ro.action_tm[t], ro.states_tm[t + 1], ro.reward_tm[t], ro.cost_tm[t])

    def rollout(self, seeds: torch.Tensor, stochastic: bool, noise_seed: int = 0) -> RolloutData:
        cfg, T = self.cfg, self.T
        B = int(seeds.shape[0])
        n = cfg.n_agents
        slot = None
        if self.use_graphs:
            slot = self._ro_cache.setdefault((B, stochastic), {"ro": None, "graph": None, "gen": -1, "calls": 0})
            if slot["ro"] is None:
                slot["ro"] = RolloutData(cfg, B, T, self.device, stochastic, self.HC)
            ro = slot["ro"]
            ro._env_major = False
        else:
            ro = RolloutData(cfg, B, T, self.device, stochastic, self.HC)
        OE.reset(cfg, seeds, ro.states_tm[0], self.reset_failed)
        ro.rnn_tm[0].zero_()
        eps = None
        if stochastic:
            eps = self.arena.get("ro.eps", T, B * n, 2)
            OE.randn_rows(noise_seed, eps.view(T, B * n * 2), self.world * B * n * 2, self.rank * B * n * 2)
        if slot is None:
            self._rollout_steps(ro, eps, B, stochastic)
            return ro
        slot["calls"] += 1
        if slot["graph"] is not None and slot["gen"] != self._arena_generation():
            slot["graph"] = None
        if slot["graph"] is not None:
            slot["graph"].replay()
            K.FLOPS[0] += slot.get("flops", 0.0)
            return ro
        f0 = K.FLOPS[0]
        self._rollout_steps(ro, eps, B, stochastic)
        slot["flops"] = K.FLOPS[0] - f0
        if not slot.get("failed", False):
            graph = torch.cuda.CUDAGraph()
            try:
                f1 = K.FLOPS[0]
                with torch.cuda.graph(graph, capture_error_mode="thread_local"):
                    self._rollout_steps(ro, eps, B, stochastic)
                K.FLOPS[0] = f1 + slot["flops"]
                slot["graph"], slot["gen"] = graph, self._arena_generation()
                graph.replay()
            except Exception as ex:
                slot["failed"] = True
                torch.cuda.synchronize()
                print(f"[dgppo_amd] HIP-graph capture of the rollout loop failed ({type(ex).__name__}: {ex}); "
                      f"continuing with eager launches", flush=True)
        return ro

    def _update_generation(self) -> int:
        return self.arena.generation + sum(net.arena.generation + net.ws_arena.generation for net in self.nets.values())

    def _arena_generation(self) -> int:
        return self.arena.generation + self.policy.arena.generation

    def rollout_pair(self, seeds: torch.Tensor, det_seeds: torch.Tensor, noise_seed: int = 0):
        if not (self.multi_stream and self.device.type == "cuda"):
            return self.rollout(seeds, True, noise_seed), self.rollout(det_seeds, False)
        main = torch.cuda.current_stream(self.device)
        s0, s1 = self._net_streams()[:2]
        out = [None, None]
        for k, (st, sd, stoch) in enumerate(((s0, seeds, True), (s1, det_seeds, False))):
            st.wait_stream(main)
            with torch.cuda.stream(st):
                out[k] = self.rollout(sd, stoch, noise_seed if stoch else 0)
        main.wait_stream(s0)
        main.wait_stream(s1)
        return out[0], out[1]

    def _block_feats(self, tag, ro: RolloutData, e0, Eb, t0, n_time, env_ids=None):
        envs = slice(e0, None) if env_ids is None else slice(None)
        st = OE.State({k: v[envs, t0] for k, v in ro.step.items()}, {k: v[envs] for k, v in ro.env.items()})
        return self._feats(tag, st, Eb, n_time, self.T + 1, env_ids)

    def _vh_carry(self, ro: RolloutData, e0: int, Eb: int) -> torch.Tensor:
        return ro.rnn_states[e0:e0 + Eb][..., :nets.HID]

    def _final_carry(self, ro: RolloutData, e0: int, Eb: int) -> torch.Tensor:
        T, n, HC = self.T, self.cfg.n_agents, self.HC
        fin = self._block_feats("fin", ro, e0, Eb, T, 1)
        h_last = self.arena.get("pre.hlast", Eb * n, HC)
        h_last.view(Eb, n, HC).copy_(ro.rnn_states[e0:e0 + Eb, T - 1])
        hstar = self.arena.get("pre.hstar", Eb * n, HC)
        self.policy.forward(fin, n_seq=Eb * n, T=1, h0=h_last, tag="fin", hs_out=hstar, train=False)
        return hstar

    def values_prepass(self, ro: RolloutData, want_Vl: bool, want_Vh: bool = True):
        cfg, T, B = self.cfg, self.T, ro.B
        n, nh, H = cfg.n_agents, self.n_cost, nets.HID
        kind = "ro" if ro.stochastic else "det"
        Vl_buf = self.arena.get(f"tg.Vl.{kind}", B, T + 1) if want_Vl else None
        Vh_buf = self.arena.get(f"tg.Vh.{kind}", B, T + 1, n, nh) if want_Vh else None
        block = max(1, min(B, self.prepass_graphs // (T + 1)))
        for e0 in range(0, B, block):
            Eb = min(block, B - e0)
            feats = self._block_feats("pre", ro, e0, Eb, 0, T + 1)
            if want_Vl:
                act = self.Vl.forward(feats, n_seq=Eb, T=T + 1, h0=None, tag="pre", train=False)
                Vl_buf[e0:e0 + Eb].copy_(act["v"].view(Eb, T + 1))
            if not want_Vh:
                continue
            HC = self.HC
            hstar = self._final_carry(ro, e0, Eb)
            if not self.hp.use_rnn:
                h0 = None
            elif HC == H:
                s0 = 0 if ro.stochastic else 1
                ro._rnn_em[e0:e0 + Eb, s0 + T].copy_(hstar.view(Eb, n, H))
                h0 = K.H0Blocks(ro._rnn_em[e0, s0], (T + 1) * n, (T + 2) * n * H, Eb)
            else:
                h0_all = self.arena.get("pre.h0all", Eb, T + 1, n, H)
                h0_all[:, :T].copy_(self._vh_carry(ro, e0, Eb))
                h0_all[:, T].copy_(hstar.view(Eb, n, HC)[..., :H])
                h0 = h0_all.view(-1, H)
            act = self.Vh.forward(feats, n_seq=Eb * (T + 1) * n, T=1, h0=h0, tag="pre", train=False)
            Vh_buf[e0:e0 + Eb].copy_(act["v"].view(Eb, T + 1, n, nh))
        return Vl_buf, Vh_buf

    def require_landscape(self, what: str = "vh_landscape"):
        if self.algo != "dgppo":
            why = {"informarl_lagr": "its constraint-value net carries its own scan state, which needs a sequence pass first"}
            raise ValueError(f"{what}: algo '{self.algo}' is not supported: "
                             + why.get(self.algo, "it has no constraint-value network"))
        if self.cfg.is_vmas:
            raise ValueError(f"{what}: VMASReverseTransport is not supported")

    def vh_landscape(self, ro: RolloutData, env_index: int, agent_id: int, frame_ids, xs, ys,
                     events: Optional[list] = None) -> torch.Tensor:
        self.require_landscape()
        cfg, T = self.cfg, self.T
        n, nh, H = cfg.n_agents, self.n_cost, nets.HID
        ro.finalize()
        if not 0 <= int(env_index) < ro.B:
            raise ValueError(f"vh_landscape: env_index {env_index} outside [0, {ro.B})")
        if not 0 <= int(agent_id) < n:
            raise ValueError(f"vh_landscape: agent_id {agent_id} outside [0, {n})")
        frames = np.asarray(frame_ids, dtype=np.int64).reshape(-1)
        if frames.size == 0 or frames.min() < 0 or frames.max() >= T:
            raise ValueError(f"vh_landscape: frame_ids must be a non-empty subset of [0, {T})")
        xs, ys = K.sweep_axis(xs, "xs", self.device), K.sweep_axis(ys, "ys", self.device)
        nx, ny, F = int(xs.numel()), int(ys.numel()), int(frames.size)
        e = int(env_index)
        step = {k: v[e] for k, v in ro.step.items()}
        env = {k: v[e] for k, v in ro.env.items()}
        rc, rs = OE._rays(cfg, self.device)
        carry = self._vh_carry(ro, e, 1)[0] if self.hp.use_rnn else None
        out = torch.empty(F, ny, nx, n, nh, device=self.device)
        ids_dev = torch.from_numpy(frames.astype(np.int32)).to(self.device)
        cap = max(1, self.prepass_graphs)
        fb = max(1, cap // (ny * nx))
        yb = ny if cap >= ny * nx else max(1, cap // nx)
        xb = nx if cap >= nx else cap
        for f0 in range(0, F, fb):
            f1 = min(F, f0 + fb)
            fr = frames[f0:f1]
            for y0 in range(0, ny, yb):
                y1 = min(ny, y0 + yb)
                for x0 in range(0, nx, xb):
                    x1 = min(nx, x0 + xb)
                    P = (y1 - y0) * (x1 - x0)
                    Gb = (f1 - f0) * P
                    feats = nets.GraphFeats(cfg, Gb, self.arena, "land")
                    ev = [torch.cuda.Event(enable_timing=True) for _ in range(3)] if events is not None else None
                    if ev:
                        ev[0].record()
                    feats.compute_sweep(step, env, ids_dev[f0:f1], f1 - f0, agent_id, xs[x0:x1], ys[y0:y1], rc, rs,
                                        frame_max=int(fr.max()))
                    if ev:
                        ev[1].record()
                    h0 = None
                    if carry is not None:
                        h0 = self.arena.get("land.h0", Gb * n, H)
                        for j, t in enumerate(fr):
                            h0.view(f1 - f0, P, n, H)[j].copy_(carry[int(t)].unsqueeze(0).expand(P, n, H))
                    act = self.Vh.forward(feats, n_seq=Gb * n, T=1, h0=h0, tag="land", train=False)
                    out[f0:f1, y0:y1, x0:x1].copy_(act["v"].view(f1 - f0, y1 - y0, x1 - x0, n, nh))
                    if ev:
                        ev[2].record()
                        events.append(tuple(ev))
        return out

    def cost_landscape(self, ro: RolloutData, env_index: int, agent_id: int, frame_ids, xs, ys) -> torch.Tensor:
        cfg, T = self.cfg, self.T
        if cfg.is_vmas:
            raise ValueError("cost_landscape: VMASReverseTransport is not supported")
        n = cfg.n_agents
        ro.finalize()
        if not 0 <= int(env_index) < ro.B:
# ... 660 lines not shown
```

dgppo_amd/nets.py:

```python
from __future__ import annotations

import math
from typing import Dict, List, Optional, Tuple

import numpy as np
import torch

from . import _native as N
from . import ops_nn as K

H_HEADS = 3
MSG_DIM = 32
OUT_DIM = 64
HID = 64


def _ceil4(x):
    return (x + 3) // 4 * 4


class Layout:
    def __init__(self):
        self.entries: Dict[str, Tuple[int, Tuple[int, ...]]] = {}
        self.size = 0

    def add(self, name, *shape):
        n = int(np.prod(shape))
        self.size = (self.size + 3) // 4 * 4
        self.entries[name] = (self.size, tuple(shape))
        self.size += n

    def view(self, flat: torch.Tensor, name: str) -> torch.Tensor:
        off, shape = self.entries[name]
        return flat[off:off + math.prod(shape)].view(shape)


def make_layout(kind: str, node_dim: int, gnn_layers: int, n_out: int, rnn: str = "gru", rnn_layers: int = 1) -> Layout:
    L = Layout()
    f = node_dim
    for l in range(gnn_layers):
        d = OUT_DIM if l == gnn_layers - 1 else MSG_DIM
        hd = H_HEADS * d
        for nm, shp in (("Wq", (f, hd)), ("bq", (hd,)), ("Wk", (f, hd)), ("bk", (hd,)), ("Wv", (f, hd)), ("bv", (hd,)),
                        ("We", (4, hd)), ("Wu", (f, d)), ("bu", (d,))):
            L.add(f"gnn{l}.{nm}", *shp)
        f = d
    for i in (1, 2):
        L.add(f"mlp.W{i}", 2 * HID if (kind == "Vhg" and i == 1) else HID, HID)
        L.add(f"mlp.b{i}", HID)
        L.add(f"mlp.g{i}", HID)
        L.add(f"mlp.be{i}", HID)
    assert rnn in ("gru", "lstm", "none"), rnn
    for l in range(rnn_layers if rnn == "lstm" else 0):
        L.add(f"lstm{l}.Wi", HID, 4 * HID)
        L.add(f"lstm{l}.Wh", HID, 4 * HID)
        L.add(f"lstm{l}.bh", 4 * HID)
    for l in range(rnn_layers if rnn == "gru" else 0):
        pre = "gru" if l == 0 else f"gru{l}"
        L.add(f"{pre}.Wi", HID, 3 * HID)
        L.add(f"{pre}.bi", 3 * HID)
        L.add(f"{pre}.Wh", HID, 3 * HID)
        L.add(f"{pre}.bhn", HID)
    if kind == "policy":
        L.add("head.Ws", HID, HID)
        L.add("head.bs", HID)
        L.add("head.Wms", HID, 2 * n_out)
        L.add("head.bms", 2 * n_out)
    else:
        L.add("head.Wo", HID, n_out)
        L.add("head.bo", n_out)
    return L


class Arena:

    def __init__(self, device):
        self.device = device
        self.bufs: Dict[str, torch.Tensor] = {}
        self.generation = 0

    def get(self, name: str, *shape, dtype=torch.float32, zero=False) -> torch.Tensor:
        n = math.prod(shape)
        b = self.bufs.get(name)
        if b is None or b.numel() < n or b.dtype != dtype:
            if b is not None:
                self.generation += 1
            b = torch.empty(max(n, 1), dtype=dtype, device=self.device)
            self.bufs[name] = b
        v = b[:n].view(shape)
        if zero:
            v.zero_()
        return v


class GraphFeats:

    def __init__(self, cfg: N.EnvCfg, G: int, arena: Arena, tag: str):
        self.cfg, self.G = cfg, G
        n, S = cfg.n_agents, cfg.fan_in
        self.n_other = cfg.num_nodes - 1 - n
        self.Fp = input_width(cfg)
        self.Xa = arena.get(f"{tag}.Xa0", G * n, self.Fp)
        self.Xo = arena.get(f"{tag}.Xo0", max(G * self.n_other, 1), self.Fp)[:G * self.n_other]
        self.efeat = arena.get(f"{tag}.efeat", G * n, S, 4)
        self.emask = arena.get(f"{tag}.emask", G * n, S)
        self.edges_from_rows = False

    def compute(self, agent, agent_se, agent_st, goal, obst, hits, hits_se, hits_st, env_ids, n_env, n_time):
        assert n_env * n_time == self.G
        K.graph_feats(self.cfg, agent, agent_se, agent_st, goal, obst, hits, hits_se, hits_st, env_ids, n_env, n_time,
                      self.Xa, self.Xo if self.n_other > 0 else None, self.efeat, self.emask, self.Fp)
        self.edges_from_rows = self.cfg.state_dim == 4
        return self

    def compute_record(self, step, slots: int, env, env_ids, n_env, n_time):
        cfg, n = self.cfg, self.cfg.n_agents
        se, st = slots, int(slots > 1)
        if cfg.is_vmas:
            return self.compute_vmas(step["agent"], se * n * 4, st * n * 4, step["body"], se * 4, st * 4, env["scene"], env_ids,
                                     n_env, n_time)
        ia, ih = n * cfg.state_dim, n * cfg.top_k * 2
        return self.compute(step["agent"], se * ia, st * ia, env["goal"], env.get("obst"), step.get("hits"), se * ih, st * ih,
                            env_ids, n_env, n_time)

    def compute_sweep(self, step, env, frame_ids, n_frames, agent_id, xs, ys, ray_cos=None, ray_sin=None, hits_out=None,
                      frame_max=None):
        cfg, n = self.cfg, self.cfg.n_agents
        if cfg.is_vmas:
            raise ValueError("compute_sweep: VMASReverseTransport has no sweep entry point")
        K.graph_feats_sweep(cfg, step["agent"], n * cfg.state_dim, env["goal"], env.get("obst"), step.get("hits"),
                            n * cfg.top_k * 2, ray_cos, ray_sin, frame_ids, n_frames, agent_id, xs, ys, self.Xa,
                            self.Xo if self.n_other > 0 else None, self.efeat, self.emask, self.Fp, hits_out, frame_max)
        self.edges_from_rows = False
        return self

    def compute_action_sweep(self, step, env, frame_ids, n_frames, agent_id, us, vs, frame_max=None):
        cfg, n = self.cfg, self.cfg.n_agents
        if cfg.is_vmas:
            raise ValueError("compute_action_sweep: VMASReverseTransport has no sweep entry point")
        K.graph_feats_action_sweep(cfg, step["agent"], n * cfg.state_dim, env["goal"], env.get("obst"), step.get("hits"),
                                   n * cfg.top_k * 2, frame_ids, n_frames, agent_id, us, vs, self.Xa,
                                   self.Xo if self.n_other > 0 else None, self.efeat, self.emask, self.Fp, frame_max)
        self.edges_from_rows = False
        return self

    def compute_team_action_sweep(self, st, nst, a_pol, us, vs):
        if self.cfg.is_vmas:
            raise ValueError("compute_team_action_sweep: VMASReverseTransport has no sweep entry point")
        K.graph_feats_team_action_sweep(self.cfg, st.step["agent"], nst.step["agent"], st.env["goal"], st.env.get("obst"),
                                        nst.step.get("hits"), a_pol, us, vs, self.Xa, self.Xo if self.n_other > 0 else None,
                                        self.efeat, self.emask, self.Fp)
        self.edges_from_rows = False
        return self

    def compute_vmas(self, agent, agent_se, agent_st, body, body_se, body_st, scene, env_ids, n_env, n_time):
        assert n_env * n_time == self.G
        K.vmas_graph_feats(self.cfg, agent, agent_se, agent_st, body, body_se, body_st, scene, env_ids, n_env, n_time,
                           self.Xa, self.efeat, self.emask, self.Fp)
        self.edges_from_rows = False
        return self


def input_width(cfg: N.EnvCfg) -> int:
    return _ceil4(cfg.node_dim) if cfg.is_vmas else 8


class Net:

    def __init__(self, kind: str, cfg: N.EnvCfg, gnn_layers: int, n_out: int, device, grads: Optional[torch.Tensor] = None,
                 rnn: str = "gru", rnn_layers: int = 1, lean_attn0: bool = True):
        assert kind in ("policy", "Vl", "Vh", "Vhg")
        self.kind, self.cfg, self.gnn_layers, self.n_out, self.device = kind, cfg, gnn_layers, n_out, device
        self.rnn, self.rnn_layers = rnn, (rnn_layers if rnn != "none" else 0)
        self.lean_attn0 = bool(lean_attn0) and K.attn_rows_supported(cfg, input_width(cfg), H_HEADS)
        self.carry_dim = HID * max(self.rnn_layers, 1) * (2 if rnn == "lstm" else 1)
        self.layout = make_layout(kind, cfg.node_dim, gnn_layers, n_out, rnn, rnn_layers)
        self.params = torch.zeros(self.layout.size, device=device)
        if grads is None:
            grads = torch.zeros(self.layout.size, device=device)
        assert grads.shape == (self.layout.size,) and grads.is_contiguous() and grads.data_ptr() % 16 == 0
        self.grads = grads
        self.arena = Arena(device)
        self.ws_arena = Arena(device)
        self._views: Dict[tuple, torch.Tensor] = {}
        self.dims = []
        f = cfg.node_dim
        for l in range(gnn_layers):
            d = OUT_DIM if l == gnn_layers - 1 else MSG_DIM
            fp = input_width(cfg) if l == 0 else f
            kp = _ceil4(fp + H_HEADS * (fp + 4) + 1)
            self.dims.append((f, fp, d, kp))
            f = d
        self.prep_layout = Layout()
        for l, (f, fp, d, kp) in enumerate(self.dims):
            self.prep_layout.add(f"gnn{l}.Mcat", fp, H_HEADS * fp)
            self.prep_layout.add(f"gnn{l}.cvec", H_HEADS * fp)
            self.prep_layout.add(f"gnn{l}.Wout", kp, d)
        self.prep = torch.zeros(self.prep_layout.size, device=device)
        self.prep_grads = torch.zeros(self.prep_layout.size, device=device)

    def _cached(self, kind: str, layout, flat, name):
        key = (kind, name)
        v = self._views.get(key)
        if v is None:
            v = self._views[key] = layout.view(flat, name)
        return v

    def p(self, name):
        return self._cached("p", self.layout, self.params, name)

    def g(self, name):
        return self._cached("g", self.layout, self.grads, name)

    def pp(self, name):
        return self._cached("pp", self.prep_layout, self.prep, name)

    def pg(self, name):
        return self._cached("pg", self.prep_layout, self.prep_grads, name)

    def prepare(self):
        for l, (f, fp, d, kp) in enumerate(self.dims):
            q = lambda nm: self.p(f"gnn{l}.{nm}")
            K.gnn_prep(q("Wq"), q("bq"), q("Wk"), q("Wv"), q("bv"), q("We"), q("Wu"), self.pp(f"gnn{l}.Mcat"),
                       self.pp(f"gnn{l}.cvec"), self.pp(f"gnn{l}.Wout"), f, fp, d, H_HEADS, kp)

    def _xo_fusable(self, l: int) -> bool:
        if l != 0 or self.gnn_layers != 2:
            return False
        key = "_xo_ok"
        if not hasattr(self, key):
            f1, fp1, d1, kp1 = self.dims[1]
            setattr(self, key, self.dims[0][1] == 8 and self.dims[0][2] == 32 and fp1 == 32 and
                    K.attn_xo_supported(self.cfg, fp1, H_HEADS, kp1))
        return getattr(self, key)

    def zero_grads(self):
        self.grads.zero_()

    def forward(self, feats: GraphFeats, n_seq: int, T: int, h0: Optional[torch.Tensor], tag: str = "f",
                hs_out: Optional[torch.Tensor] = None, train: bool = True, qt0: Optional[torch.Tensor] = None):
        cfg, G, A = self.cfg, feats.G, self.arena
        n = cfg.n_agents
        R = G * n
        Ro = G * feats.n_other
        act = {"feats": feats, "G": G, "n_seq": n_seq, "T": T}
        Xa, Xo = feats.Xa, feats.Xo
        xo_fused = None
        for l, (f, fp, d, kp) in enumerate(self.dims):
            if l == 0 and qt0 is not None:
                assert tuple(qt0.shape) == (R, H_HEADS * fp), (tuple(qt0.shape), R, H_HEADS * fp)
                qt = qt0
            else:
                qt = A.get(f"{tag}.qt{l}", R, H_HEADS * fp)
                K.dense_fwd(Xa, self.pp(f"gnn{l}.Mcat"), self.pp(f"gnn{l}.cvec"), qt)
            zcat = A.get(f"{tag}.zcat{l}", R, kp)
            lean = l == 0 and self.lean_attn0 and feats.edges_from_rows
            attn = A.get(f"{tag}.attn{l}", R, cfg.fan_in, H_HEADS) if train and not lean else None
            if lean:
                K.attn_fwd_rows(cfg, fp, H_HEADS, kp, qt, Xa, Xo if Ro > 0 else None, feats.emask, zcat, None, G)
            elif xo_fused is not None:
                K.attn_fwd_xo(cfg, fp, H_HEADS, kp, qt, Xa, xo_fused[0], xo_fused[1], xo_fused[2], feats.efeat, feats.emask, zcat, attn, G)
            else:
                K.attn_fwd(cfg, fp, H_HEADS, kp, qt, Xa, Xo if Ro > 0 else None, feats.efeat, feats.emask, zcat, attn, G)
            act[f"xo_fused{l}"] = xo_fused
            xo_fused = None
            Xa_n = A.get(f"{tag}.Xa{l + 1}", R, d)
            K.dense_fwd(zcat, self.pp(f"gnn{l}.Wout"), self.p(f"gnn{l}.bu"), Xa_n, act=1)
            act[f"Xa{l}"], act[f"Xo{l}"], act[f"qt{l}"], act[f"zcat{l}"], act[f"attn{l}"] = Xa, Xo, qt, zcat, attn
            act[f"lean{l}"] = lean
            if l < self.gnn_layers - 1 and Ro > 0:
                if self._xo_fusable(l):
                    xo_fused = (Xo, self.pp(f"gnn{l}.Wout")[:fp], self.p(f"gnn{l}.bu"))
                    Xo = None
                else:
                    Xo_n = A.get(f"{tag}.Xo{l + 1}", Ro, d)
                    K.dense_fwd(Xo, self.pp(f"gnn{l}.Wout")[:fp], self.p(f"gnn{l}.bu"), Xo_n, act=1)
                    Xo = Xo_n
            Xa = Xa_n
        act[f"Xa{self.gnn_layers}"] = Xa
        if self.kind == "Vl":
            pooled = A.get(f"{tag}.pool", G, OUT_DIM)
            K.mean_agents(Xa, pooled, G, n, OUT_DIM)
            x, Rh, n_inner = pooled, G, 1
        else:
            x, Rh, n_inner = Xa, R, n
        if self.kind == "Vhg":
            pooled = A.get(f"{tag}.pool", G, OUT_DIM)
            K.mean_agents(Xa, pooled, G, n, OUT_DIM)
            xcat = A.get(f"{tag}.xcat", R, 2 * OUT_DIM)
            xcat[:, :OUT_DIM].copy_(Xa)
            xcat.view(G, n, 2 * OUT_DIM)[:, :, OUT_DIM:].copy_(pooled.view(G, 1, OUT_DIM).expand(G, n, OUT_DIM))
            x = xcat
        act["Rh"], act["n_inner"], act["mlp_in"] = Rh, n_inner, x
        gi = A.get(f"{tag}.gi", Rh, 3 * HID)
        if self.kind == "Vhg" or self.rnn != "gru":
            sv = {nm: A.get(f"{tag}.{nm}", Rh, w) for nm, w in (("p1", HID), ("y1", HID), ("st1", 2), ("p2", HID), ("y2", HID), ("st2", 2))}
            K.dense_fwd(x, self.p("mlp.W1"), self.p("mlp.b1"), sv["p1"])
            K.ln_relu_fwd(sv["p1"], self.p("mlp.g1"), self.p("mlp.be1"), sv["y1"], sv["st1"])
            K.dense_fwd(sv["y1"], self.p("mlp.W2"), self.p("mlp.b2"), sv["p2"])
            K.ln_relu_fwd(sv["p2"], self.p("mlp.g2"), self.p("mlp.be2"), sv["y2"], sv["st2"])
            if self.rnn == "gru":
                K.dense_fwd(sv["y2"], self.p("gru.Wi"), self.p("gru.bi"), gi)
            act.update(sv)
        else:
            saves = None
            if train:
                saves = tuple(A.get(f"{tag}.{nm}{i}", Rh, w) for i in (1, 2) for nm, w in (("p", HID), ("y", HID), ("st", 2)))
                for i in (1, 2):
                    act[f"p{i}"], act[f"y{i}"], act[f"st{i}"] = saves[3 * (i - 1):3 * i]
            K.mlp_gi_fwd(x, self.p("mlp.W1"), self.p("mlp.b1"), self.p("mlp.g1"), self.p("mlp.be1"), self.p("mlp.W2"),
                         self.p("mlp.b2"), self.p("mlp.g2"), self.p("mlp.be2"), self.p("gru.Wi"), self.p("gru.bi"), gi, saves)
        assert n_seq * T == Rh, (n_seq, T, Rh)
        L, CD = self.rnn_layers, self.carry_dim
        h0_blocks = isinstance(h0, K.H0Blocks)
        if h0_blocks:
            assert self.rnn == "gru" and L == 1 and T == 1 and not train and self.kind != "policy", \
                "a blocked h0 serves the one-cell GRU value nets' T = 1 inference pass"
        elif h0 is not None:
            assert tuple(h0.shape) == (n_seq, CD), (tuple(h0.shape), n_seq, CD)
        if hs_out is not None:
            assert tuple(hs_out.shape) == (Rh, CD), (tuple(hs_out.shape), Rh, CD)
        act["gi"] = gi
        simple = (self.rnn == "gru" and L == 1)
        if simple:
            hs = hs_out if hs_out is not None else A.get(f"{tag}.hs", Rh, HID)
            hprev_is_h0 = train and T == 1 and h0 is not None and self.kind != "policy"
            hprev = A.get(f"{tag}.hprev", Rh, HID) if (train and not hprev_is_h0) else None
            gates = A.get(f"{tag}.gates", Rh, 4 * HID) if train else None
            feat = hs
            act["hs"], act["hprev"], act["gates"] = hs, hprev, gates
        fused_tail = (simple and T == 1 and self.kind == "policy")
        if simple and not fused_tail:
            if h0_blocks:
                K.gru_fwd_h0_blocks(gi, self.p("gru.Wh"), self.p("gru.bhn"), h0, hs, hprev, gates, n_seq, T, n_inner)
            else:
                K.gru_fwd(gi, self.p("gru.Wh"), self.p("gru.bhn"), h0, hs, hprev, gates, n_seq, T, n_inner)
            if hprev_is_h0:
                act["hprev"] = act["h0"] = h0
        if self.rnn == "none":
            feat = act["y2"]
            if hs_out is not None:
                if h0 is not None and T == 1:
                    hs_out.copy_(h0)
                else:
                    hs_out.zero_()
        elif self.rnn == "lstm":
            x_l = act["y2"]
            act["stack"] = []
            for l in range(L):
                zi = A.get(f"{tag}.zi{l}", Rh, 4 * HID)
                for half in (slice(0, 2 * HID), slice(2 * HID, 4 * HID)):
                    K.dense_fwd(x_l, self.p(f"lstm{l}.Wi")[:, half], None, zi[:, half])
                c0_l = h0_l = None
                if h0 is not None:
                    c0_l, h0_l = A.get(f"{tag}.c0_{l}", n_seq, HID), A.get(f"{tag}.h0_{l}", n_seq, HID)
                    c0_l.copy_(h0[:, (2 * l) * HID:(2 * l + 1) * HID])
                    h0_l.copy_(h0[:, (2 * l + 1) * HID:(2 * l + 2) * HID])
                cs_l, hs_l = A.get(f"{tag}.cs{l}", Rh, HID), A.get(f"{tag}.hs{l}", Rh, HID)
                cprev_l = A.get(f"{tag}.cprev{l}", Rh, HID) if train else None
                hprev_l = A.get(f"{tag}.hprev{l}", Rh, HID) if train else None
                gates_l = A.get(f"{tag}.gates{l}", Rh, 4 * HID) if train else None
                K.lstm_fwd(zi, self.p(f"lstm{l}.Wh"), self.p(f"lstm{l}.bh"), c0_l, h0_l, cs_l, hs_l, cprev_l, hprev_l, gates_l,
                           n_seq, T, n_inner)
                if hs_out is not None:
                    hs_out[:, (2 * l) * HID:(2 * l + 1) * HID].copy_(cs_l)
                    hs_out[:, (2 * l + 1) * HID:(2 * l + 2) * HID].copy_(hs_l)
                act["stack"].append(dict(x=x_l, hs=hs_l, cprev=cprev_l, hprev=hprev_l, gates=gates_l))
                x_l = hs_l
            feat = x_l
        elif not simple:
            x_l = None
            act["stack"] = []
            for l in range(L):
                pre = "gru" if l == 0 else f"gru{l}"
                gi_l = gi if l == 0 else A.get(f"{tag}.gi{l}", Rh, 3 * HID)
                if l > 0:
                    K.dense_fwd(x_l, self.p(f"{pre}.Wi"), self.p(f"{pre}.bi"), gi_l)
                h0_l = None
                if h0 is not None:
                    h0_l = A.get(f"{tag}.h0_{l}", n_seq, HID)
                    h0_l.copy_(h0[:, l * HID:(l + 1) * HID])
                hs_l = A.get(f"{tag}.hs{l}", Rh, HID)
                hprev_l = A.get(f"{tag}.hprev{l}", Rh, HID) if train else None
                gates_l = A.get(f"{tag}.gates{l}", Rh, 4 * HID) if train else None
                K.gru_fwd(gi_l, self.p(f"{pre}.Wh"), self.p(f"{pre}.bhn"), h0_l, hs_l, hprev_l, gates_l, n_seq, T, n_inner)
                if hs_out is not None:
                    hs_out[:, l * HID:(l + 1) * HID].copy_(hs_l)
                act["stack"].append(dict(x=x_l, gi=gi_l, hs=hs_l, hprev=hprev_l, gates=gates_l))
                x_l = hs_l
            feat = x_l
        act["feat"] = feat
        if self.kind == "policy":
            u = A.get(f"{tag}.u", Rh, HID) if (train or not fused_tail) else None
            ms = A.get(f"{tag}.ms", Rh, 4)
            if fused_tail:
                K.gru1_head_fwd(gi, self.p("gru.Wh"), self.p("gru.bhn"), h0, self.p("head.Ws"), self.p("head.bs"),
                                self.p("head.Wms"), self.p("head.bms"), hs, hprev, gates, u, ms)
            else:
                K.dense_fwd(feat, self.p("head.Ws"), self.p("head.bs"), u)
                K.dense_fwd(u, self.p("head.Wms"), self.p("head.bms"), ms)
            act["u"], act["ms"] = u, ms
        else:
            v = A.get(f"{tag}.v", Rh, self.n_out)
            K.dense_fwd(feat, self.p("head.Wo"), self.p("head.bo"), v)
            act["v"] = v
        return act

    def backward(self, act, dout: torch.Tensor, tag: str = "b"):
        A = self.arena
        ws_floats = getattr(self, "_bwdw_floats", 16 << 20)

        def _alloc(n_floats):
            self._bwdw_floats = max(ws_floats, n_floats)
            return self.ws_arena.get(f"{tag}.bwdw_ws", self._bwdw_floats)
        batch = K.BwdWBatch(self.device, _alloc) if dout.is_cuda else None
        if batch is not None:
            batch.__enter__()
        try:
            self._backward_body(act, dout, tag)
        except BaseException:
            if batch is not None:
                batch.__exit__(RuntimeError, None, None)
            raise
        if batch is not None:
            batch.__exit__(None, None, None)
        for l, (f, fp, d, kp) in enumerate(self.dims):
            q = lambda nm: self.p(f"gnn{l}.{nm}")
            gq = lambda nm: self.g(f"gnn{l}.{nm}")
            K.gnn_unprep(self.pg(f"gnn{l}.Mcat"), self.pg(f"gnn{l}.cvec"), self.pg(f"gnn{l}.Wout"), q("Wq"), q("bq"), q("Wk"),
                         gq("Wq"), gq("bq"), gq("Wk"), gq("Wv"), gq("bv"), gq("We"), gq("Wu"), f, fp, d, H_HEADS, kp)
        self.prep_grads.zero_()

    @staticmethod
    def _gru_t1_in_pass(act, T, row_operands) -> bool:
        return (T == 1 and act.get("h0") is not None and act["hprev"] is act["h0"]
                and all(t.is_cuda and t.data_ptr() % 16 == 0 for t in row_operands))

    def _backward_body(self, act, dout: torch.Tensor, tag: str):
        cfg, A = self.cfg, self.arena
        G, Rh, n_inner, n_seq, T = act["G"], act["Rh"], act["n_inner"], act["n_seq"], act["T"]
        n = cfg.n_agents
        R = G * n
        feats: GraphFeats = act["feats"]
        Ro = G * feats.n_other
        feat = act["feat"]
        fused_trunk = self.rnn == "gru" and self.rnn_layers == 1 and self.kind != "Vhg" and dout.is_cuda
        dgi0 = None
        dhs = A.get(f"{tag}.dhs", Rh, HID)
        if dout.is_cuda:
            if self.kind == "policy":
                K.head_bwd(feat, act["u"], dout, self.p("head.Ws"), self.p("head.Wms"), dhs, self.g("head.Ws"), self.g("head.bs"),
                           self.g("head.Wms"), self.g("head.bms"))
            else:
                K.head_bwd(feat, None, dout, self.p("head.Wo"), None, dhs, self.g("head.Wo"), self.g("head.bo"))
        elif self.kind == "policy":
            K.dense_bwd_w(act["u"], dout, self.g("head.Wms"), self.g("head.bms"))
            du = A.get(f"{tag}.du", Rh, HID)
            K.dense_fwd(dout, self.p("head.Wms"), None, du, trans_w=True)
            K.dense_bwd_w(feat, du, self.g("head.Ws"), self.g("head.bs"))
            K.dense_fwd(du, self.p("head.Ws"), None, dhs, trans_w=True)
        else:
            K.dense_bwd_w(feat, dout, self.g("head.Wo"), self.g("head.bo"))
            K.dense_fwd(dout, self.p("head.Wo"), None, dhs, trans_w=True)
        if self.rnn == "none":
            dy = dhs
        elif self.rnn == "lstm":
            stack = act["stack"]
            for l in range(len(stack) - 1, -1, -1):
                st = stack[l]
                dz = A.get(f"{tag}.dz_lstm{l}", Rh, 4 * HID)
                K.lstm_bwd(dhs, self.p(f"lstm{l}.Wh"), st["cprev"], st["gates"], dz, n_seq, T, n_inner)
                for half in (slice(0, 2 * HID), slice(2 * HID, 4 * HID)):
                    K.dense_bwd_w(st["hprev"], dz[:, half], self.g(f"lstm{l}.Wh")[:, half], self.g(f"lstm{l}.bh")[half])
                    K.dense_bwd_w(st["x"], dz[:, half], self.g(f"lstm{l}.Wi")[:, half], None)
                dx = A.get(f"{tag}.dy" if l == 0 else f"{tag}.dx{l}", Rh, HID)
                K.dense_fwd(dz, self.p(f"lstm{l}.Wi"), None, dx, trans_w=True)
                dhs = dx
            dy = dhs
        else:
            stack = act.get("stack") or [dict(x=None, gi=act["gi"], hs=act["hs"], hprev=act["hprev"], gates=act["gates"])]
            if act.get("stack") is None and dout.is_cuda:
                st = stack[0]
                dgi = A.get(f"{tag}.dgi0", Rh, 3 * HID)
                gW = (self.g("gru.Wi"), self.g("gru.bi"), self.g("gru.Wh"), self.g("gru.bhn"))
                if self._gru_t1_in_pass(act, T, (act["y2"], st["hprev"], dhs, st["gates"], dgi)):
                    K.gru_bwd_w_t1(act["y2"], st["hprev"], dhs, st["gates"], dgi, *gW)
                else:
                    dhn = A.get(f"{tag}.dhn0", Rh, HID)
                    K.gru_bwd_dhn(dhs, self.p("gru.Wh"), st["hprev"], st["gates"], dgi, dhn, n_seq, T, n_inner)
                    K.gru_bwd_w(act["y2"], st["hprev"], dgi, dhn, *gW)
                if fused_trunk:
                    dgi0 = dgi
                else:
                    dhs = A.get(f"{tag}.dy", Rh, HID)
                    K.dense_fwd(dgi, self.p("gru.Wi"), None, dhs, trans_w=True)
                stack = []
            for l in range(len(stack) - 1, -1, -1):
                st = stack[l]
                pre = "gru" if l == 0 else f"gru{l}"
                dgi = A.get(f"{tag}.dgi{l}", Rh, 3 * HID)
                dgh = A.get(f"{tag}.dgh{l}", Rh, 3 * HID)
                K.gru_bwd(dhs, self.p(f"{pre}.Wh"), st["hprev"], st["gates"], dgi, dgh, n_seq, T, n_inner)
                K.dense_bwd_w(st["hprev"], dgh[:, :2 * HID], self.g(f"{pre}.Wh")[:, :2 * HID], None)
                K.dense_bwd_w(st["hprev"], dgh[:, 2 * HID:], self.g(f"{pre}.Wh")[:, 2 * HID:], self.g(f"{pre}.bhn"))
                x_l = act["y2"] if l == 0 else st["x"]
                K.dense_bwd_w(x_l, dgi, self.g(f"{pre}.Wi"), self.g(f"{pre}.bi"))
                if l == 0 and fused_trunk:
                    dgi0 = dgi
                    break
                dx = A.get(f"{tag}.dy" if l == 0 else f"{tag}.dx{l}", Rh, HID)
                K.dense_fwd(dgi, self.p(f"{pre}.Wi"), None, dx, trans_w=True)
                dhs = dx
            dy = dhs
        x_in = {1: act["mlp_in"], 2: act["y1"]}
        top = act[f"Xa{self.gnn_layers}"]
        if fused_trunk:
            dy = A.get(f"{tag}.dyy1", Rh, HID)
            K.mlp_gi_bwd_w(dgi0, self.p("gru.Wi"), self.p("mlp.W2"), self.p("mlp.W1"), self.p("mlp.g2"), self.p("mlp.g1"),
                           act["p2"], act["y2"], act["st2"], act["p1"], act["y1"], act["st1"], x_in[1],
                           top if self.kind in ("policy", "Vh") else None, dy,
                           self.g("mlp.g2"), self.g("mlp.be2"), self.g("mlp.g1"), self.g("mlp.be1"),
                           self.g("mlp.W2"), self.g("mlp.b2"), self.g("mlp.W1"), self.g("mlp.b1"))
        for i in (() if fused_trunk else (2, 1)):
            dpre = A.get(f"{tag}.dpre{i}", Rh, HID)
            K.ln_relu_bwd(act[f"p{i}"], act[f"y{i}"], act[f"st{i}"], self.p(f"mlp.g{i}"), dy, dpre, self.g(f"mlp.g{i}"),
                          self.g(f"mlp.be{i}"))
            K.dense_bwd_w(x_in[i], dpre, self.g(f"mlp.W{i}"), self.g(f"mlp.b{i}"))
            dy = A.get(f"{tag}.dyy{i}", Rh, HID if not (self.kind == "Vhg" and i == 1) else 2 * HID)
            K.dense_fwd(dpre, self.p(f"mlp.W{i}"), None, dy, trans_w=True,
                        relu_mask=top if (i == 1 and self.kind in ("policy", "Vh")) else None)
        if self.kind == "Vl":
            dXa = A.get(f"{tag}.dXaL", R, OUT_DIM)
            K.mean_agents(dy, dXa, G, n, OUT_DIM, backward=True, relu_mask=top)
        elif self.kind == "Vhg":
            dXa = A.get(f"{tag}.dXaL", R, OUT_DIM)
            dXa.copy_(dy[:, :OUT_DIM])
            dglob = A.get(f"{tag}.dglob", R, OUT_DIM)
            dglob.copy_(dy[:, OUT_DIM:])
            dpool = A.get(f"{tag}.dpool", G, OUT_DIM)
            K.mean_agents(dglob, dpool, G, n, OUT_DIM)
            K.mean_agents(dpool, dXa, G, n, OUT_DIM, backward=2, relu_mask=top)
        else:
            dXa = dy
        dXo = None
        for l in range(self.gnn_layers - 1, -1, -1):
            f, fp, d, kp = self.dims[l]
            dz = A.get(f"{tag}.dz{l}", R, kp)
            K.dense_bwd_xw(act[f"zcat{l}"], dXa, self.pp(f"gnn{l}.Wout"), dz, self.pg(f"gnn{l}.Wout"), self.g(f"gnn{l}.bu"))
            if dXo is not None:
                K.dense_bwd_w(act[f"Xo{l}"], dXo, self.pg(f"gnn{l}.Wout")[:fp], self.g(f"gnn{l}.bu"))
            dqt = A.get(f"{tag}.dqt{l}", R, H_HEADS * fp)
            need_dx = l > 0
            dXa_l = A.get(f"{tag}.dXa{l}", R, fp) if need_dx else None
            dXo_prev = dXo
            dXo_l = A.get(f"{tag}.dXo{l}", Ro, fp) if (need_dx and Ro > 0) else None
            more_dXo = dXo_prev is not None and dXo_l is not None
            xf = act.get(f"xo_fused{l}")
            if act.get(f"lean{l}"):
                K.attn_bwd_rows(cfg, fp, H_HEADS, kp, dz, None, act[f"qt{l}"], feats.emask, act[f"Xa{l}"],
                                act[f"Xo{l}"] if Ro > 0 else None, dqt, G)
            elif xf is not None and dXa_l is not None and not more_dXo:
                ws = A.get(f"{tag}.xo_ws", K.attn_xo_workspace_floats(G), 1).view(-1)
                K.attn_bwd_xo_dw(cfg, fp, H_HEADS, kp, dz, act[f"attn{l}"], act[f"qt{l}"], act[f"Xa{l}"], xf[0], xf[1], xf[2],
                                 feats.efeat, dqt, dXa_l, self.pg(f"gnn{l - 1}.Wout")[:self.dims[l - 1][1]], self.g(f"gnn{l - 1}.bu"), ws, G)
# ... 102 lines not shown
```

dgppo_amd/ops_nn.py:

```python
from __future__ import annotations

import ctypes as C
from typing import Optional

import numpy as np
import torch

from . import _native as N

FLOPS = [0.0]


def _mat(t: torch.Tensor, name: str):
    if t.dim() != 2:
        raise ValueError(f"{name} must be 2-D, got {tuple(t.shape)}")
    if not t.is_cuda:
        raise RuntimeError(f"{name} must live on the GPU (the HIP path has no CPU fallback)")
    if t.dtype != torch.float32:
        raise TypeError(f"{name} must be float32")
    if t.shape[1] > 1 and t.stride(1) != 1:
        raise ValueError(f"{name} must have unit inner stride")
    ld = t.stride(0) if t.shape[0] > 1 else max(t.shape[1], t.stride(0))
    return C.c_void_p(t.data_ptr()), int(ld), int(t.shape[0]), int(t.shape[1])

# ... 322 lines not shown
        _p(ray_cos, "ray_cos") if cast else null, _p(ray_sin, "ray_sin") if cast else null,
        _p(ids_dev, "frame_ids", torch.int32), C.c_int32(n_frames), C.c_int32(int(agent_id)), _p(xs, "xs"), C.c_int32(nx),
        _p(ys, "ys"), C.c_int32(ny), _p(Xa, "Xa"), _p(Xo, "Xo") if n_other > 0 else null, _p(efeat, "efeat"), _p(emask, "emask"),
        _p(hits_out, "hits_out") if (cast and hits_out is not None) else null, C.c_int32(Fp), N.stream_ptr())
    N.check(rc, "dgppo_graph_feats_sweep")


def cost_sweep(cfg: N.EnvCfg, agent, agent_st, obst, hits, hits_st, ray_cos, ray_sin, frame_ids, n_frames, agent_id, xs, ys,
               cost, hits_out=None, frame_max=None):
    fn = "cost_sweep"
    if cfg.is_vmas:
        raise ValueError(f"{fn}: VMASReverseTransport has no sweep entry point")
    if hits_out is not None and not (cfg.is_lidar and cfg.n_obs > 0):
        raise ValueError(f"{fn}: hits_out needs a LiDAR kind with obstacles (nothing is cast here)")
    nx, ny, ids, ids_dev, last = _sweep_grid(fn, cfg, frame_ids, n_frames, agent_id, xs, ys, frame_max)
    G = n_frames * ny * nx
    N.expect_shape(cost, (G, cfg.n_agents, cfg.n_cost), "cost")
    cast = _sweep_record(fn, cfg, agent, agent_st, obst, hits, hits_st, ray_cos, ray_sin, last, hits_out, G)
    if ids is not None:
        ids_dev = torch.from_numpy(ids.astype(np.int32)).to(agent.device)
    null = C.c_void_p(0)
    rc = N.lib().dgppo_cost_sweep(
        C.byref(cfg), C.c_void_p(agent.data_ptr()), C.c_int64(agent_st), _p(obst, "obst") if cfg.n_obs > 0 else null,
        C.c_void_p(hits.data_ptr()) if cast else null, C.c_int64(hits_st), _p(ray_cos, "ray_cos") if cast else null,
        _p(ray_sin, "ray_sin") if cast else null, _p(ids_dev, "frame_ids", torch.int32), C.c_int32(n_frames),
        C.c_int32(int(agent_id)), _p(xs, "xs"), C.c_int32(nx), _p(ys, "ys"), C.c_int32(ny), _p(cost, "cost"),
        _p(hits_out, "hits_out") if cast and hits_out is not None else null, N.stream_ptr())
    N.check(rc, "dgppo_cost_sweep")


ACTION_SWEEP_TILE = 64


def graph_feats_action_sweep(cfg: N.EnvCfg, agent, agent_st, goal, obst, hits, hits_st, frame_ids, n_frames, agent_id, us, vs,
                             Xa, Xo, efeat, emask, Fp, frame_max=None):
    fn = "graph_feats_action_sweep"
    if cfg.is_vmas:
        raise ValueError(f"{fn}: VMASReverseTransport has no sweep entry point")
    n, S = cfg.n_agents, cfg.fan_in
    nu, nv, ids, ids_dev, last = _sweep_grid(fn, cfg, frame_ids, n_frames, agent_id, us, vs, frame_max, ("us", "vs"))
    G = n_frames * nv * nu
    n_other = cfg.num_nodes - 1 - n
    N.expect_shape(Xa, (G * n, Fp), "Xa")
    if n_other > 0:
        N.expect_shape(Xo, (G * n_other, Fp), "Xo")
    N.expect_shape(efeat, (G * n, S, 4), "efeat")
    N.expect_shape(emask, (G * n, S), "emask")
    N.expect_shape(goal, (cfg.n_goals, cfg.state_dim), "goal")
    _check_strided(fn, "agent", agent, 0, agent_st, (n, cfg.state_dim), None, 1, last + 2)
    rec_hits = cfg.is_lidar and cfg.n_obs > 0
    discs = (not cfg.is_lidar) and cfg.n_obs > 0
    if rec_hits:
        if hits is None:
            raise ValueError(f"{fn}: hits is required for a LiDAR kind with obstacles")
        _check_strided(fn, "hits", hits, 0, hits_st, (n, cfg.top_k, 2), None, 1, last + 2)
    if discs:
        if obst is None:
            raise ValueError(f"{fn}: obst is required when n_obs > 0")
        N.expect_shape(obst, (cfg.n_obs, cfg.obst_stride), "obst")
    if ids is not None:
        ids_dev = torch.from_numpy(ids.astype(np.int32)).to(agent.device)
    null = C.c_void_p(0)
    rc = N.lib().dgppo_graph_feats_action_sweep(
        C.byref(cfg), C.c_void_p(agent.data_ptr()), C.c_int64(agent_st), _p(goal, "goal"), _p(obst, "obst") if discs else null,
        C.c_void_p(hits.data_ptr()) if rec_hits else null, C.c_int64(hits_st), _p(ids_dev, "frame_ids", torch.int32),
        C.c_int32(n_frames), C.c_int32(int(agent_id)), _p(us, "us"), C.c_int32(nu), _p(vs, "vs"), C.c_int32(nv), _p(Xa, "Xa"),
        _p(Xo, "Xo") if n_other > 0 else null, _p(efeat, "efeat"), _p(emask, "emask"), C.c_int32(Fp), N.stream_ptr())
    N.check(rc, "dgppo_graph_feats_action_sweep")


def _dense(fn: str, name: str, t_, shape, dtype=torch.float32):
    if not (torch.is_tensor(t_) and t_.is_cuda and t_.dtype == dtype and t_.is_contiguous()):
        raise ValueError(f"{fn}: {name} must be a contiguous {dtype} CUDA tensor")
    if tuple(t_.shape) != tuple(shape):
        raise ValueError(f"{fn}: {name}: expected shape {tuple(shape)}, got {tuple(t_.shape)}")


def _shield_axes(fn: str, us, vs):
    for name, t_ in (("us", us), ("vs", vs)):
        if not (torch.is_tensor(t_) and t_.is_cuda and t_.dtype == torch.float32 and t_.ndim == 1 and t_.is_contiguous()):
            raise ValueError(f"{fn}: {name} must be a dense 1-D float32 CUDA tensor (sweep_axis)")
        if t_.numel() == 0:
            raise ValueError(f"{fn}: {name} is empty")
    return int(us.numel()), int(vs.numel())


def graph_feats_team_action_sweep(cfg: N.EnvCfg, agent, next_agent, goal, obst, next_hits, a_pol, us, vs, Xa, Xo, efeat, emask,
                                  Fp):
    fn = "graph_feats_team_action_sweep"
    if cfg.is_vmas:
        raise ValueError(f"{fn}: VMASReverseTransport has no sweep entry point")
    n, S, sd = cfg.n_agents, cfg.fan_in, cfg.state_dim
    nu, nv = _shield_axes(fn, us, vs)
    if not (torch.is_tensor(agent) and agent.ndim == 3):
        raise ValueError(f"{fn}: agent must be a [B, n, state_dim] tensor")
    B = int(agent.shape[0])
    G = B * n * (1 + nu * nv)
    n_other = cfg.num_nodes - 1 - n
    _dense(fn, "agent", agent, (B, n, sd))
    _dense(fn, "next_agent", next_agent, (B, n, sd))
    _dense(fn, "goal", goal, (B, cfg.n_goals, sd))
    _dense(fn, "a_pol", a_pol, (B, n, 2))
    _dense(fn, "Xa", Xa, (G * n, Fp))
    if n_other > 0:
        _dense(fn, "Xo", Xo, (G * n_other, Fp))
    _dense(fn, "efeat", efeat, (G * n, S, 4))
    _dense(fn, "emask", emask, (G * n, S))
    rec_hits = cfg.is_lidar and cfg.n_obs > 0
    discs = (not cfg.is_lidar) and cfg.n_obs > 0
    if rec_hits:
        if next_hits is None:
            raise ValueError(f"{fn}: next_hits is required for a LiDAR kind with obstacles")
        _dense(fn, "next_hits", next_hits, (B, n, cfg.top_k, 2))
    if discs:
        if obst is None:
            raise ValueError(f"{fn}: obst is required when n_obs > 0")
        _dense(fn, "obst", obst, (B, cfg.n_obs, cfg.obst_stride))
    null = C.c_void_p(0)
    rc = N.lib().dgppo_graph_feats_team_action_sweep(
        C.byref(cfg), _p(agent, "agent"), _p(next_agent, "next_agent"), _p(goal, "goal"), _p(obst, "obst") if discs else null,
        _p(next_hits, "next_hits") if rec_hits else null, _p(a_pol, "a_pol"), C.c_int32(B), _p(us, "us"), C.c_int32(nu),
        _p(vs, "vs"), C.c_int32(nv), _p(Xa, "Xa"), _p(Xo, "Xo") if n_other > 0 else null, _p(efeat, "efeat"), _p(emask, "emask"),
        C.c_int32(Fp), N.stream_ptr())
    N.check(rc, "dgppo_graph_feats_team_action_sweep")


def shield_select(Vh_next, Vh_t, a_pol, us, vs, dt: float, alpha: float, margin: float, action, index, flag, h=None):
    fn = "shield_select"
    nu, nv = _shield_axes(fn, us, vs)
    P = 1 + nu * nv
    if not (torch.is_tensor(Vh_t) and Vh_t.ndim == 3):
        raise ValueError(f"{fn}: Vh_t must be a [E, n, n_cost] tensor")
    E, n, nh = (int(s) for s in Vh_t.shape)
    if n < 1 or nh < 1:
        raise ValueError(f"{fn}: Vh_t must have at least one agent and one cost component")
    for name, v in (("dt", dt), ("alpha", alpha), ("margin", margin)):
        if not np.isfinite(float(v)):
            raise ValueError(f"{fn}: {name} must be finite")
    if not float(dt) > 0.0:
        raise ValueError(f"{fn}: dt must be > 0")
    _dense(fn, "Vh_t", Vh_t, (E, n, nh))
    _dense(fn, "Vh_next", Vh_next, (E * n * P * n, nh))
    _dense(fn, "a_pol", a_pol, (E, n, 2))
    _dense(fn, "action", action, (E, n, 2))
    _dense(fn, "index", index, (E, n), torch.int32)
    _dense(fn, "flag", flag, (E, n), torch.int32)
    if h is not None:
        _dense(fn, "h", h, (E, n, P))
    rc = N.lib().dgppo_shield_select(
        _p(Vh_next, "Vh_next"), _p(Vh_t, "Vh_t"), _p(a_pol, "a_pol"), C.c_int32(E), C.c_int32(n), C.c_int32(nh), _p(us, "us"),
        C.c_int32(nu), _p(vs, "vs"), C.c_int32(nv), C.c_float(float(dt)), C.c_float(float(alpha)), C.c_float(float(margin)),
        _p(action, "action"), _p(index, "index", torch.int32), _p(flag, "flag", torch.int32), _p(h, "h"), N.stream_ptr())
    N.check(rc, "dgppo_shield_select")


def _shaped(fn: str, operands):
    for name, t_, shape, *_ in operands:
        if not torch.is_tensor(t_) or tuple(t_.shape) != tuple(shape):
            got = tuple(t_.shape) if torch.is_tensor(t_) else type(t_).__name__
            raise ValueError(f"{fn}: {name}: expected shape {tuple(shape)}, got {got}")
    for name, t_, shape, *dtype in operands:
        _dense(fn, name, t_, shape, *dtype)


def lookahead_select(cost_tm, a_pol, us, vs, margin: float, action, index, flag, s=None):
    fn = "lookahead_select"
    if not (torch.is_tensor(a_pol) and a_pol.ndim == 3 and a_pol.shape[2] == 2 and a_pol.shape[1] >= 1):
        raise ValueError(f"{fn}: a_pol must be a [E, n, 2] tensor")
    E, n = int(a_pol.shape[0]), int(a_pol.shape[1])
    if not (torch.is_tensor(cost_tm) and cost_tm.ndim == 4):
        raise ValueError(f"{fn}: cost_tm must be a [K, G, n, nh] tensor")
    K_, nh = int(cost_tm.shape[0]), int(cost_tm.shape[3])
    if K_ < 1:
        raise ValueError(f"{fn}: K must be >= 1")
    if not 1 <= nh <= 3:
        raise ValueError(f"{fn}: n_cost {nh} outside [1, 3]")
    for name, t_ in (("us", us), ("vs", vs)):
        if not (torch.is_tensor(t_) and t_.ndim == 1 and t_.numel() > 0):
            raise ValueError(f"{fn}: {name} must be a non-empty 1-D tensor (sweep_axis)")
    P = 1 + int(us.numel()) * int(vs.numel())
    G = E * n * P
    if tuple(cost_tm.shape[1:]) != (G, n, nh):
        raise ValueError(f"{fn}: cost_tm: expected shape (K, {G}, {n}, {nh}), got {tuple(cost_tm.shape)}")
    if np.isnan(float(margin)):
        raise ValueError(f"{fn}: margin must not be NaN")
    _shaped(fn, [("a_pol", a_pol, (E, n, 2)), ("cost_tm[0]", cost_tm[0], (G, n, nh)), ("action", action, (E, n, 2)),
                 ("index", index, (E, n), torch.int32), ("flag", flag, (E, n), torch.int32)]
            + ([("s", s, (E, n, P))] if s is not None else []))
    nu, nv = _shield_axes(fn, us, vs)
    cost_st = int(cost_tm.stride(0)) if K_ > 1 else G * n * nh
    if cost_st < G * n * nh:
        raise ValueError(f"{fn}: the steps of cost_tm overlap (stride {cost_st} < {G * n * nh})")
    rc = N.lib().dgppo_lookahead_select(
        _p(cost_tm[0], "cost"), cost_st, K_, E, n, nh, _p(a_pol, "a_pol"), _p(us, "us"), nu, _p(vs, "vs"), nv, float(margin),
        _p(action, "action"), _p(index, "index", torch.int32), _p(flag, "flag", torch.int32), _p(s, "s"), N.stream_ptr())
    N.check(rc, "dgppo_lookahead_select")


def vmas_graph_feats(cfg: N.EnvCfg, agent, agent_se, agent_st, body, body_se, body_st, scene, env_ids, n_env, n_time,
                     Xa, efeat, emask, Fp):
    G = n_env * n_time
    n = cfg.n_agents
    N.expect_shape(Xa, (G * n, Fp), "Xa")
    N.expect_shape(efeat, (G * n, n, 4), "efeat")
    N.expect_shape(emask, (G * n, n), "emask")
    _check_strided("vmas_graph_feats", "agent", agent, agent_se, agent_st, (n, 4), env_ids, n_env, n_time)
    _check_strided("vmas_graph_feats", "body", body, body_se, body_st, (4,), env_ids, n_env, n_time)
    rc = N.lib().dgppo_vmas_graph_feats(
        C.byref(cfg), C.c_void_p(agent.data_ptr()), C.c_int64(agent_se), C.c_int64(agent_st), C.c_void_p(body.data_ptr()),
        C.c_int64(body_se), C.c_int64(body_st), _p(scene, "scene"), _p(env_ids, "env_ids", torch.int32), C.c_int32(n_env),
        C.c_int32(n_time), _p(Xa, "Xa"), _p(efeat, "efeat"), _p(emask, "emask"), C.c_int32(Fp), N.stream_ptr())
    N.check(rc, "dgppo_vmas_graph_feats")


def attn_fwd(cfg, F, H, Kp, qt, Xa, Xo, efeat, emask, zcat, attn, G):
    n, S = cfg.n_agents, cfg.fan_in
    N.expect_shape(qt, (G * n, H * F), "qt")
    N.expect_shape(Xa, (G * n, F), "Xa")
    N.expect_shape(zcat, (G * n, Kp), "zcat")
    if attn is not None:
        N.expect_shape(attn, (G * n, S, H), "attn")
    FLOPS[0] += 2.0 * G * n * H * S * (2 * F + 4)
    rc = N.lib().dgppo_attn_fwd(C.byref(cfg), F, H, Kp, _p(qt), _p(Xa), _p(Xo), _p(efeat), _p(emask), _p(zcat), _p(attn),
                                G, N.stream_ptr())
    N.check(rc, "dgppo_attn_fwd")


def attn_bwd(cfg, F, H, Kp, dzcat, attn, qt, Xa, Xo, efeat, dqt, dXa, dXo, G, relu_xo: bool = False):
    n = cfg.n_agents
    N.expect_shape(dzcat, (G * n, Kp), "dzcat")
    N.expect_shape(dqt, (G * n, H * F), "dqt")
    if dXa is not None:
        N.expect_shape(dXa, (G * n, F), "dXa")
    FLOPS[0] += 4.0 * G * n * H * cfg.fan_in * (2 * F + 4)
    rc = N.lib().dgppo_attn_bwd(C.byref(cfg), F, H, Kp, _p(dzcat), _p(attn), _p(qt), _p(Xa), _p(Xo), _p(efeat), _p(dqt),
                                _p(dXa), _p(dXo), int(relu_xo), G, N.stream_ptr())
    N.check(rc, "dgppo_attn_bwd")


def attn_rows_supported(cfg, F, H) -> bool:
    return bool(N.lib().dgppo_attn_rows_supported(C.byref(cfg), F, H))


def attn_fwd_rows(cfg, F, H, Kp, qt, Xa, Xo, emask, zcat, attn, G):
    n, S = cfg.n_agents, cfg.fan_in
    N.expect_shape(qt, (G * n, H * F), "qt")
    N.expect_shape(Xa, (G * n, F), "Xa")
    N.expect_shape(emask, (G * n, S), "emask")
    N.expect_shape(zcat, (G * n, Kp), "zcat")
    if attn is not None:
        N.expect_shape(attn, (G * n, S, H), "attn")
    FLOPS[0] += 2.0 * G * n * H * S * (2 * F + 4) + 4.0 * G * n * S
    rc = N.lib().dgppo_attn_fwd_rows(C.byref(cfg), F, H, Kp, _p(qt), _p(Xa), _p(Xo), _p(emask), _p(zcat), _p(attn), G,
                                     N.stream_ptr())
    N.check(rc, "dgppo_attn_fwd_rows")


def attn_bwd_rows(cfg, F, H, Kp, dzcat, attn, qt, emask, Xa, Xo, dqt, G):
    n, S = cfg.n_agents, cfg.fan_in
    N.expect_shape(dzcat, (G * n, Kp), "dzcat")
    N.expect_shape(Xa, (G * n, F), "Xa")
    N.expect_shape(dqt, (G * n, H * F), "dqt")
    FLOPS[0] += 4.0 * G * n * H * S * (2 * F + 4) + 4.0 * G * n * S
    if attn is None:
        N.expect_shape(qt, (G * n, H * F), "qt")
        N.expect_shape(emask, (G * n, S), "emask")
        FLOPS[0] += 2.0 * G * n * H * S * F
    else:
        N.expect_shape(attn, (G * n, S, H), "attn")
    rc = N.lib().dgppo_attn_bwd_rows(C.byref(cfg), F, H, Kp, _p(dzcat), _p(attn), _p(qt), _p(emask), _p(Xa), _p(Xo), _p(dqt), G,
                                     N.stream_ptr())
    N.check(rc, "dgppo_attn_bwd_rows")


def attn_xo_supported(cfg, F, H, Kp) -> bool:
    return bool(N.lib().dgppo_attn_xo_supported(C.byref(cfg), F, H, Kp))


def _wo_ptr(Wo):
    if not Wo.is_cuda or Wo.dtype != torch.float32:
        raise TypeError("Wo must be a float32 GPU tensor")
    return C.c_void_p(Wo.data_ptr())


def _wo_ld(Wo):
    if Wo.dim() != 2 or Wo.shape[0] != 8 or Wo.shape[1] < 32 or Wo.stride(1) != 1:
        raise ValueError(f"Wo must be [8, >= 32] with contiguous rows, got {tuple(Wo.shape)} strides {Wo.stride()}")
    return int(Wo.stride(0))


def attn_fwd_xo(cfg, F, H, Kp, qt, Xa, Xo_raw, Wo, bo, efeat, emask, zcat, attn, G):
    n, S = cfg.n_agents, cfg.fan_in
    N.expect_shape(qt, (G * n, H * F), "qt")
    N.expect_shape(Xa, (G * n, F), "Xa")
    N.expect_shape(zcat, (G * n, Kp), "zcat")
    N.expect_shape(Xo_raw, (G * (cfg.num_nodes - 1 - n), 8), "Xo_raw")
    N.expect_shape(bo, (32,), "bo")
    if attn is not None:
        N.expect_shape(attn, (G * n, S, H), "attn")
    FLOPS[0] += 2.0 * G * n * H * S * (2 * F + 4) + 2.0 * G * (cfg.num_nodes - 1 - n) * 8 * 32
    rc = N.lib().dgppo_attn_fwd_xo(C.byref(cfg), F, H, Kp, _p(qt), _p(Xa), _p(Xo_raw), _wo_ptr(Wo),
                                   _wo_ld(Wo), _p(bo), _p(efeat), _p(emask), _p(zcat), _p(attn), G, N.stream_ptr())
    N.check(rc, "dgppo_attn_fwd_xo")


def attn_bwd_xo(cfg, F, H, Kp, dzcat, attn, qt, Xa, Xo_raw, Wo, bo, efeat, dqt, dXa, dXo, G, relu_xo: bool = False):
    n = cfg.n_agents
    N.expect_shape(dzcat, (G * n, Kp), "dzcat")
    N.expect_shape(dqt, (G * n, H * F), "dqt")
    N.expect_shape(Xo_raw, (G * (cfg.num_nodes - 1 - n), 8), "Xo_raw")
    if dXa is not None:
        N.expect_shape(dXa, (G * n, F), "dXa")
    FLOPS[0] += 4.0 * G * n * H * cfg.fan_in * (2 * F + 4) + 2.0 * G * (cfg.num_nodes - 1 - n) * 8 * 32
    rc = N.lib().dgppo_attn_bwd_xo(C.byref(cfg), F, H, Kp, _p(dzcat), _p(attn), _p(qt), _p(Xa), _p(Xo_raw),
                                   _wo_ptr(Wo), _wo_ld(Wo), _p(bo), _p(efeat), _p(dqt), _p(dXa), _p(dXo),
                                   int(relu_xo), G, N.stream_ptr())
    N.check(rc, "dgppo_attn_bwd_xo")


def attn_xo_workspace_floats(G: int) -> int:
    return int(N.lib().dgppo_attn_xo_workspace_bytes(int(G))) // 4


def attn_bwd_xo_dw(cfg, F, H, Kp, dzcat, attn, qt, Xa, Xo_raw, Wo, bo, efeat, dqt, dXa, dWo, dbo, workspace, G):
    n = cfg.n_agents
    N.expect_shape(dzcat, (G * n, Kp), "dzcat")
    N.expect_shape(dqt, (G * n, H * F), "dqt")
    N.expect_shape(dXa, (G * n, F), "dXa")
    N.expect_shape(Xo_raw, (G * (cfg.num_nodes - 1 - n), 8), "Xo_raw")
    N.expect_shape(dbo, (32,), "dbo")
    FLOPS[0] += 4.0 * G * n * H * cfg.fan_in * (2 * F + 4) + 4.0 * G * (cfg.num_nodes - 1 - n) * 8 * 32
    rc = N.lib().dgppo_attn_bwd_xo_dw(C.byref(cfg), F, H, Kp, _p(dzcat), _p(attn), _p(qt), _p(Xa), _p(Xo_raw), _wo_ptr(Wo), _wo_ld(Wo),
                                      _p(bo), _p(efeat), _p(dqt), _p(dXa), _wo_ptr(dWo), _wo_ld(dWo), _p(dbo), _p(workspace),
                                      C.c_int64(workspace.numel() * 4), G, N.stream_ptr())
    N.check(rc, "dgppo_attn_bwd_xo_dw")


def gnn_prep(Wq, bq, Wk, Wv, bv, We, Wu, Mcat, cvec, Wout, F, Fp, D, H, Kp):
    rc = N.lib().dgppo_gnn_prep(_p(Wq), _p(bq), _p(Wk), _p(Wv), _p(bv), _p(We), _p(Wu), _p(Mcat), _p(cvec), _p(Wout),
                                F, Fp, D, H, Kp, N.stream_ptr())
    N.check(rc, "dgppo_gnn_prep")


def gnn_unprep(dMcat, dcvec, dWout, Wq, bq, Wk, dWq, dbq, dWk, dWv, dbv, dWe, dWu, F, Fp, D, H, Kp):
    rc = N.lib().dgppo_gnn_unprep(_p(dMcat), _p(dcvec), _p(dWout), _p(Wq), _p(bq), _p(Wk), _p(dWq), _p(dbq), _p(dWk),
                                  _p(dWv), _p(dbv), _p(dWe), _p(dWu), F, Fp, D, H, Kp, N.stream_ptr())
    N.check(rc, "dgppo_gnn_unprep")


def ln_relu_fwd(x, gamma, beta, y, stats):
    M = x.shape[0]
    N.expect_shape(x, (M, 64), "x")
    N.expect_shape(y, (M, 64), "y")
    rc = N.lib().dgppo_ln_relu_fwd(_p(x), _p(gamma), _p(beta), _p(y), _p(stats), M, N.stream_ptr())
    N.check(rc, "dgppo_ln_relu_fwd")


def ln_relu_bwd(x, y, stats, gamma, dy, dx, dgamma, dbeta):
    M = x.shape[0]
    rc = N.lib().dgppo_ln_relu_bwd(_p(x), _p(y), _p(stats), _p(gamma), _p(dy), _p(dx), _p(dgamma), _p(dbeta), M,
                                   N.stream_ptr())
    N.check(rc, "dgppo_ln_relu_bwd")


def gru_fwd(gi, Wh, bhn, h0, hs, hprev, gates, n_seq, T, n_inner):
    rows = n_seq * T
    N.expect_shape(gi, (rows, 192), "gi")
    N.expect_shape(hs, (rows, 64), "hs")
    N.expect_shape(Wh, (64, 192), "Wh")
    if h0 is not None:
        N.expect_shape(h0, (n_seq, 64), "h0")
    FLOPS[0] += 2.0 * rows * 64 * 192
    rc = N.lib().dgppo_gru_fwd(_p(gi), _p(Wh), _p(bhn), _p(h0), _p(hs), _p(hprev), _p(gates), n_seq, T, n_inner,
                               N.stream_ptr())
    N.check(rc, "dgppo_gru_fwd")


class H0Blocks:

    def __init__(self, base: torch.Tensor, rows_per_block: int, block_stride: int, n_blocks: int):
        assert base.dtype == torch.float32 and base.is_cuda
        st = base.untyped_storage()
        last = base.storage_offset() + (n_blocks - 1) * block_stride + rows_per_block * 64
        assert n_blocks >= 1 and last * 4 <= st.nbytes(), "H0Blocks: the blocks leave the storage of base"
        self.base, self.rows_per_block, self.block_stride, self.n_blocks = base, int(rows_per_block), int(block_stride), int(n_blocks)

    @property
    def n_seq(self) -> int:
        return self.n_blocks * self.rows_per_block


def gru_fwd_h0_blocks(gi, Wh, bhn, h0: H0Blocks, hs, hprev, gates, n_seq, T, n_inner):
    rows = n_seq * T
    N.expect_shape(gi, (rows, 192), "gi")
    N.expect_shape(hs, (rows, 64), "hs")
    N.expect_shape(Wh, (64, 192), "Wh")
    if n_seq > h0.n_seq:
        raise ValueError(f"h0: {h0.n_blocks} blocks of {h0.rows_per_block} rows hold fewer than n_seq = {n_seq} carries")
    FLOPS[0] += 2.0 * rows * 64 * 192
    rc = N.lib().dgppo_gru_fwd_h0_blocks(_p(gi), _p(Wh), _p(bhn), C.c_void_p(h0.base.data_ptr()), h0.rows_per_block,
                                         C.c_int64(h0.block_stride), _p(hs), _p(hprev), _p(gates), n_seq, T, n_inner,
                                         N.stream_ptr())
    N.check(rc, "dgppo_gru_fwd_h0_blocks")


class GatherDesc(C.Structure):
    _fields_ = [("src", C.c_void_p), ("dst", C.c_void_p), ("row_bytes", C.c_int64), ("src_stride", C.c_int64)]


GATHER_MAX = 8


def gather_rows(pairs, ids):
    if ids.dtype != torch.int32 or not ids.is_cuda or not ids.is_contiguous():
        raise TypeError("ids must be a contiguous int32 CUDA tensor")
    n_ids = int(ids.numel())
    if len(pairs) > GATHER_MAX:
        raise ValueError(f"gather_rows takes at most {GATHER_MAX} tensors per launch, got {len(pairs)}")
    descs = (GatherDesc * max(len(pairs), 1))()
    for k, (src, dst) in enumerate(pairs):
        if not (src.is_cuda and dst.is_cuda):
            raise RuntimeError("gather_rows: tensors must live on the GPU (the HIP path has no CPU fallback)")
        if src.dtype != dst.dtype or tuple(dst.shape) != (n_ids,) + tuple(src.shape[1:]):
            raise ValueError(f"gather_rows: pair {k}: dst {tuple(dst.shape)} {dst.dtype} does not fit src {tuple(src.shape)} "
                             f"{src.dtype} gathered by {n_ids} ids")
        if not dst.is_contiguous() or (src.shape[0] > 0 and not src[0].is_contiguous()):
            raise ValueError(f"gather_rows: pair {k}: dst and the rows of src must be contiguous")
        row = (src[0].numel() if src.shape[0] > 0 else 0) * src.element_size()
        descs[k] = GatherDesc(src.data_ptr(), dst.data_ptr(), row, src.stride(0) * src.element_size())
    rc = N.lib().dgppo_gather_rows(descs, len(pairs), C.c_void_p(ids.data_ptr()), n_ids, N.stream_ptr())
    N.check(rc, "dgppo_gather_rows")


def gru_bwd(dhs, Wh, hprev, gates, dgi, dgh, n_seq, T, n_inner):
    rows = n_seq * T
    N.expect_shape(dhs, (rows, 64), "dhs")
    N.expect_shape(dgi, (rows, 192), "dgi")
    N.expect_shape(dgh, (rows, 192), "dgh")
    FLOPS[0] += 2.0 * n_seq * (T - 1) * 64 * 192
    rc = N.lib().dgppo_gru_bwd(_p(dhs), _p(Wh), _p(hprev), _p(gates), _p(dgi), _p(dgh), n_seq, T, n_inner, N.stream_ptr())
    N.check(rc, "dgppo_gru_bwd")


def gru_bwd_dhn(dhs, Wh, hprev, gates, dgi, dhn, n_seq, T, n_inner):
    rows = n_seq * T
    N.expect_shape(dhs, (rows, 64), "dhs")
    N.expect_shape(dgi, (rows, 192), "dgi")
    N.expect_shape(dhn, (rows, 64), "dhn")
    FLOPS[0] += 2.0 * n_seq * (T - 1) * 64 * 192
    rc = N.lib().dgppo_gru_bwd_dhn(_p(dhs), _p(Wh), _p(hprev), _p(gates), _p(dgi), _p(dhn), n_seq, T, n_inner, N.stream_ptr())
    N.check(rc, "dgppo_gru_bwd_dhn")


def _gru_bwd_w_call(name, x, hprev, rows_in, dgi, dWi, dbi, dWh, dbhn):
    xp, ldx, M, Kx = _mat(x, "x")
    hp, ldh, Mh, Kh = _mat(hprev, "hprev")
    wip, ldwi, _, _ = _mat(dWi, "dWi")
    whp, ldwh, _, _ = _mat(dWh, "dWh")
    if Kx != 64 or (Mh, Kh) != (M, 64) or tuple(dWi.shape) != (64, 192) or tuple(dWh.shape) != (64, 192):
        raise ValueError(f"{name}: shape mismatch x{tuple(x.shape)} hprev{tuple(hprev.shape)} dWi{tuple(dWi.shape)} "
                         f"dWh{tuple(dWh.shape)}")
    for nm, (t, w) in rows_in.items():
        N.expect_shape(t, (M, w), nm)
    N.expect_shape(dgi, (M, 192), "dgi")
    N.expect_shape(dbi, (192,), "dbi"); N.expect_shape(dbhn, (64,), "dbhn")
    FLOPS[0] += 2.0 * M * 64 * (128 + 64 + 192)
    lib = N.lib()
    need = _workspace_bytes("dgppo_gru_bwd_w_workspace_bytes", x.device)
    batch = BwdWBatch._active.get((x.device.index, torch.cuda.current_stream(x.device).cuda_stream)) if x.is_cuda else None
    if batch is not None:
        ws = batch.region(need)
        d = (ReduceDesc * 3)()
        pend = d
    else:
        key = (x.device.index, torch.cuda.current_stream(x.device).cuda_stream, "gru")
        ws = _WS.get(key)
        if ws is None or ws.numel() * 4 < need:
            ws = _WS[key] = torch.empty(need // 4, dtype=torch.float32, device=x.device)
        pend = None
    mid = [_p(t, nm) for nm, (t, w) in rows_in.items()]
    if name == "dgppo_gru_bwd_w":
        mid = [_p(dgi, "dgi")] + mid
    else:
        mid = mid + [_p(dgi, "dgi")]
    rc = getattr(lib, name)(xp, ldx, hp, ldh, *mid, wip, ldwi, _p(dbi, "dbi"), whp, ldwh, _p(dbhn, "dbhn"), M,
                            _p(ws, "workspace"), C.c_int64(ws.numel() * 4), pend, N.stream_ptr())
    N.check(rc, name)
    if batch is not None:
        for i in range(3):
            if d[i].pending:
                batch.descs.append(ReduceDesc.from_buffer_copy(d[i]))


def gru_bwd_w(x, hprev, dgi, dhn, dWi, dbi, dWh, dbhn):
    _gru_bwd_w_call("dgppo_gru_bwd_w", x, hprev, {"dhn": (dhn, 64)}, dgi, dWi, dbi, dWh, dbhn)


def gru_bwd_w_t1(x, h0, dhs, gates, dgi, dWi, dbi, dWh, dbhn):
    _gru_bwd_w_call("dgppo_gru_bwd_w_t1", x, h0, {"dhs": (dhs, 64), "gates": (gates, 256)}, dgi, dWi, dbi, dWh, dbhn)


_WS_BYTES: dict = {}


def _workspace_bytes(query: str, device) -> int:
    key = (query, device.index)
    if key not in _WS_BYTES:
        fn = getattr(N.lib(), query)
        fn.restype = C.c_int64
        _WS_BYTES[key] = int(fn())
    return _WS_BYTES[key]


def mlp_gi_bwd_w(dgi, Wi, W2, W1, g2, g1, p2, y2, st2, p1, y1, st1, x, relu_mask, dx, dg2, db2, dg1, db1, dW2, dbias2, dW1,
                 dbias1, dpre2=None, dpre1=None):
    M = dgi.shape[0]
    N.expect_shape(dgi, (M, 192), "dgi")
    for t, shp, nm in ((Wi, (64, 192), "Wi"), (W2, (64, 64), "W2"), (W1, (64, 64), "W1"), (g2, (64,), "g2"), (g1, (64,), "g1"),
                       (p2, (M, 64), "p2"), (y2, (M, 64), "y2"), (st2, (M, 2), "st2"), (p1, (M, 64), "p1"), (y1, (M, 64), "y1"),
                       (st1, (M, 2), "st1"), (dx, (M, 64), "dx"), (dg2, (64,), "dg2"), (db2, (64,), "db2"), (dg1, (64,), "dg1"),
                       (db1, (64,), "db1"), (dbias2, (64,), "dbias2"), (dbias1, (64,), "dbias1")):
        N.expect_shape(t, shp, nm)
    for t, nm in ((dpre2, "dpre2"), (dpre1, "dpre1")):
        if t is not None:
            N.expect_shape(t, (M, 64), nm)
    xp, ldx, Mx, Kx = _mat(x, "x")
    w2p, ldw2, _, _ = _mat(dW2, "dW2")
    w1p, ldw1, _, _ = _mat(dW1, "dW1")
    if (Mx, Kx) != (M, 64) or tuple(dW2.shape) != (64, 64) or tuple(dW1.shape) != (64, 64):
        raise ValueError(f"mlp_gi_bwd_w: shape mismatch x{tuple(x.shape)} dW2{tuple(dW2.shape)} dW1{tuple(dW1.shape)}")
    mp, ldm = C.c_void_p(0), 0
    if relu_mask is not None:
        mp, ldm, Mm, Km = _mat(relu_mask, "relu_mask")
        if (Mm, Km) != (M, 64):
            raise ValueError(f"mlp_gi_bwd_w: relu_mask must be [M, 64], got {tuple(relu_mask.shape)}")
    FLOPS[0] += 2.0 * M * (64 * 64 * 2 + 64 * 192) + 2 * 2.0 * M * 64 * 64
    lib = N.lib()
    need = _workspace_bytes("dgppo_mlp_gi_bwd_w_workspace_bytes", dgi.device)
    batch = BwdWBatch._active.get((dgi.device.index, torch.cuda.current_stream(dgi.device).cuda_stream))
    d = (ReduceDesc * 2)()
    if batch is not None:
        ws = batch.region(need)
    else:
        key = (dgi.device.index, torch.cuda.current_stream(dgi.device).cuda_stream, "trunk")
        ws = _WS.get(key)
        if ws is None or ws.numel() * 4 < need:
            ws = _WS[key] = torch.empty(need // 4, dtype=torch.float32, device=dgi.device)
    rc = lib.dgppo_mlp_gi_bwd_w(_p(dgi), _p(Wi), _p(W2), _p(W1), _p(g2), _p(g1), _p(p2), _p(y2), _p(st2), _p(p1), _p(y1), _p(st1),
                                xp, ldx, mp, ldm, _p(dpre2), _p(dpre1), _p(dx), 64, _p(dg2), _p(db2), _p(dg1), _p(db1),
                                w2p, ldw2, _p(dbias2), w1p, ldw1, _p(dbias1), M, _p(ws, "workspace"), C.c_int64(ws.numel() * 4),
                                d if batch is not None else None, N.stream_ptr())
    N.check(rc, "dgppo_mlp_gi_bwd_w")
    if batch is not None:
        for i in range(2):
            if d[i].pending:
                batch.descs.append(ReduceDesc.from_buffer_copy(d[i]))


def head_bwd(feat, u, dout, W1, W2, dhs, dW1, db1, dW2=None, db2=None):
    fp, ldf, M, Kf = _mat(feat, "feat")
    n_out = int(dout.shape[1]) if dout.dim() == 2 else -1
    two = W2 is not None
    if Kf != 64 or not 1 <= n_out <= 16:
        raise ValueError(f"head_bwd: feat must be [M, 64] and dout [M, n_out <= 16], got {tuple(feat.shape)} {tuple(dout.shape)}")
    N.expect_shape(dout, (M, n_out), "dout"); N.expect_shape(dhs, (M, 64), "dhs")
    if two:
        N.expect_shape(u, (M, 64), "u"); N.expect_shape(W1, (64, 64), "W1"); N.expect_shape(W2, (64, n_out), "W2")
        N.expect_shape(db1, (64,), "db1"); N.expect_shape(db2, (n_out,), "db2")
        if tuple(dW1.shape) != (64, 64) or tuple(dW2.shape) != (64, n_out):
            raise ValueError(f"head_bwd: shape mismatch dW1{tuple(dW1.shape)} dW2{tuple(dW2.shape)}")
        w2p, ldw2, _, _ = _mat(dW2, "dW2")
        FLOPS[0] += 2.0 * M * (2 * 64 * n_out + 2 * 64 * 64)
    else:
        if u is not None or dW2 is not None or db2 is not None:
            raise ValueError("head_bwd: u, dW2, db2 belong to the two-layer form (W2 given)")
        N.expect_shape(W1, (64, n_out), "W1"); N.expect_shape(db1, (n_out,), "db1")
        if tuple(dW1.shape) != (64, n_out):
            raise ValueError(f"head_bwd: shape mismatch dW1{tuple(dW1.shape)}")
        w2p, ldw2 = C.c_void_p(0), 0
        FLOPS[0] += 2.0 * M * 2 * 64 * n_out
    w1p, ldw1, _, _ = _mat(dW1, "dW1")
    lib = N.lib()
    need = _workspace_bytes("dgppo_head_bwd_workspace_bytes", feat.device)
    batch = BwdWBatch._active.get((feat.device.index, torch.cuda.current_stream(feat.device).cuda_stream))
    d = (ReduceDesc * 2)()
    if batch is not None:
        ws = batch.region(need)
    else:
        key = (feat.device.index, torch.cuda.current_stream(feat.device).cuda_stream, "head")
        ws = _WS.get(key)
        if ws is None or ws.numel() * 4 < need:
            ws = _WS[key] = torch.empty(need // 4, dtype=torch.float32, device=feat.device)
    rc = lib.dgppo_head_bwd(fp, ldf, _p(u, "u"), _p(dout, "dout"), _p(W1, "W1"), _p(W2, "W2"), _p(dhs, "dhs"), w1p, ldw1,
                            _p(db1, "db1"), w2p, ldw2, _p(db2, "db2"), M, n_out, _p(ws, "workspace"), C.c_int64(ws.numel() * 4),
                            d if batch is not None else None, N.stream_ptr())
    N.check(rc, "dgppo_head_bwd")
    if batch is not None:
        for i in range(2):
            if d[i].pending:
                batch.descs.append(ReduceDesc.from_buffer_copy(d[i]))


def policy_head(ms, eps, action_in, action, log_pi, entropy, n_agents, mode, log_pi_old=None, adv=None, dms=None,
                stats=None, clip_eps=0.25, coef_ent=0.01):
    rows = ms.shape[0]
    N.expect_shape(ms, (rows, 4), "ms")
# ... 41 lines not shown
```

include/dgppo_hip.h:

```cpp
#ifndef DGPPO_HIP_H
#define DGPPO_HIP_H

#include <stdint.h>

#ifdef __cplusplus
extern "C" {
#endif

#define DGPPO_ABI_VERSION 3

enum {
  DGPPO_ENV_LIDAR_SPREAD = 0,
  DGPPO_ENV_LIDAR_TARGET = 1,
  DGPPO_ENV_LIDAR_BICYCLE_TARGET = 2,
  DGPPO_ENV_MPE_SPREAD = 3,
  DGPPO_ENV_MPE_TARGET = 4,
  DGPPO_ENV_LIDAR_LINE = 5,
  DGPPO_ENV_MPE_LINE = 6,
  DGPPO_ENV_MPE_FORMATION = 7,
  DGPPO_ENV_MPE_CORRIDOR = 8,
  DGPPO_ENV_MPE_CONNECT_SPREAD = 9,
  DGPPO_ENV_VMAS_REVERSE_TRANSPORT = 10
};
enum {
  DGPPO_GOALS_NODES = 0,
  DGPPO_GOALS_LINE = 1,
  DGPPO_GOALS_LINE_INTERIOR = 2,
  DGPPO_GOALS_CIRCLE = 3
};

#define DGPPO_RECT_STRIDE 16

typedef struct dgppo_env_cfg {
  int32_t kind;
  int32_t n_agents;
  int32_t n_goals;
  int32_t n_obs;
  int32_t n_rays;
  int32_t top_k;
  int32_t state_dim;
  int32_t node_dim;
  float area_size;
  float dt;
  float car_radius;
  float comm_radius;
  float obs_radius;
  float dist2goal;
  float two_car_radius;
  float lidar_mask_radius;
  float eye_offset;
  float car_plus_obs;
  float vel_limit;
  float reset_min_dist;
  int32_t reward_goals;
  int32_t n_cost;
  float obs_mask_radius;
  float y_limit;
  float connect_radius;
  float reset_side_y;
  float goal_shift_y;
  float line_min_dist;
} dgppo_env_cfg;

typedef struct dgppo_graph_out {
  float*   nodes;
  float*   edges;
  float*   states;
  int32_t* receivers;
  int32_t* senders;
  int32_t* node_type;
  int32_t* n_node;
  int32_t* n_edge;
} dgppo_graph_out;

int32_t     dgppo_abi_version(void);
const char* dgppo_last_error(void);

int32_t dgppo_env_num_nodes(const dgppo_env_cfg* cfg);
int32_t dgppo_env_num_edges(const dgppo_env_cfg* cfg);


int32_t dgppo_env_step(const dgppo_env_cfg* cfg,
                       const float* agent, const float* action, const float* goal,
                       const float* obst, const float* hits,
                       const float* ray_cos, const float* ray_sin,
                       float* next_agent, float* next_hits, float* reward, float* cost,
                       const dgppo_graph_out* gout, int32_t B, void* stream);

int32_t dgppo_env_act_step_feats_supported(const dgppo_env_cfg* cfg, int32_t Fp, int32_t H);
int32_t dgppo_env_act_step_feats(const dgppo_env_cfg* cfg, const float* agent, const float* goal, const float* obst,
                                 const float* hits, const float* ray_cos, const float* ray_sin, const float* ms,
                                 const float* eps, int32_t sample, float* action, float* log_pi, float* next_agent,
                                 float* next_hits, float* reward, float* cost, float* Xa, float* Xo, float* efeat,
                                 float* emask, int32_t Fp, const float* Mcat, const float* cvec, float* qt0, int32_t H,
                                 int32_t max_blocks, int32_t B, void* stream);

int32_t dgppo_graph_materialize(const dgppo_env_cfg* cfg,
                                const float* agent, const float* goal,
                                const float* obst, const float* hits,
                                const dgppo_graph_out* gout, int32_t B, void* stream);

int32_t dgppo_env_reset(const dgppo_env_cfg* cfg, const uint64_t* seeds,
                        float* agent, float* goal, float* obst, int32_t B, void* stream);
int32_t dgppo_env_reset_checked(const dgppo_env_cfg* cfg, const uint64_t* seeds, float* agent, float* goal, float* obst,
                                int32_t* n_failed, int32_t B, void* stream);


int32_t dgppo_vmas_reset_checked(const dgppo_env_cfg* cfg, const uint64_t* seeds, float* agent, float* body, float* scene,
                                 int32_t* n_failed, int32_t B, void* stream);
int32_t dgppo_vmas_step(const dgppo_env_cfg* cfg, const float* agent, const float* body, const float* scene,
                        const float* action, float* next_agent, float* next_body, float* reward, float* cost,
                        const dgppo_graph_out* gout, int32_t B, void* stream);
int32_t dgppo_vmas_graph_materialize(const dgppo_env_cfg* cfg, const float* agent, const float* body, const float* scene,
                                     const dgppo_graph_out* gout, int32_t B, void* stream);
int32_t dgppo_vmas_graph_feats(const dgppo_env_cfg* cfg, const float* agent, int64_t agent_se, int64_t agent_st,
                               const float* body, int64_t body_se, int64_t body_st, const float* scene,
                               const int32_t* env_ids, int32_t n_env, int32_t n_time, float* Xa, float* efeat, float* emask,
                               int32_t Fp, void* stream);

int32_t dgppo_randn(uint64_t seed, uint64_t offset, float* out, int64_t n_elem, void* stream);
int32_t dgppo_randn_rows(uint64_t seed, float* out, int64_t rows, int64_t row_len, int64_t global_row_len,
                         int64_t col_offset, void* stream);


int32_t dgppo_dense_fwd(const float* X, int32_t ldx, const float* W, int32_t ldw, const float* bias, float* Y,
                        int32_t ldy, int32_t M, int32_t K, int32_t N, int32_t act, int32_t accumulate,
                        int32_t trans_w, const float* relu_mask, int32_t ldm, void* stream);
int32_t dgppo_dense_bwd_w(const float* X, int32_t ldx, const float* dY, int32_t ldy, float* dW, int32_t ldw,
                          float* db, int32_t M, int32_t K, int32_t N, float* workspace, int64_t workspace_bytes,
                          void* stream);
int32_t dgppo_mlp_gi_fwd(const float* X, int32_t ldx, const float* W1, const float* b1, const float* g1, const float* be1,
                         const float* W2, const float* b2, const float* g2, const float* be2, const float* Wi,
                         const float* bi, float* p1, float* y1, float* st1, float* p2, float* y2, float* st2, float* gi,
                         int32_t M, void* stream);
int32_t dgppo_mlp_gi_bwd(const float* dgi, const float* Wi, const float* W2, const float* W1, const float* g2,
                         const float* g1, const float* p2, const float* y2, const float* st2, const float* p1,
                         const float* y1, const float* st1, const float* relu_mask, int32_t ldm, float* dpre2, float* dpre1,
                         float* dx, int32_t lddx, float* dg2, float* db2, float* dg1, float* db1, int32_t M, void* stream);
#define DGPPO_REDUCE_BATCH 16
typedef struct dgppo_reduce_desc {
  const float* part;
  float* dW;
  float* db;
  int32_t part_stride, slabs, ldw, K, N;
  int32_t pending;
} dgppo_reduce_desc;
int32_t dgppo_dense_bwd_w_deferred(const float* X, int32_t ldx, const float* dY, int32_t ldy, float* dW, int32_t ldw,
                                   float* db, int32_t M, int32_t K, int32_t N, float* workspace, int64_t workspace_bytes,
                                   dgppo_reduce_desc* pending, void* stream);
int32_t dgppo_dense_bwd_w_reduce_batch(const dgppo_reduce_desc* descs, int32_t n, void* stream);
int32_t dgppo_dense_bwd_xw(const float* X, int32_t ldx, const float* dY, int32_t ldy, const float* W, int32_t ldw, float* dX,
                           int32_t lddx, int32_t accumulate_mask, float* dW, int32_t lddw, float* db, int32_t M, int32_t K,
                           int32_t N, float* workspace, int64_t workspace_bytes, dgppo_reduce_desc* pending, void* stream);
int64_t dgppo_mlp_gi_bwd_w_workspace_bytes(void);
int32_t dgppo_mlp_gi_bwd_w(const float* dgi, const float* Wi, const float* W2, const float* W1, const float* g2,
                           const float* g1, const float* p2, const float* y2, const float* st2, const float* p1,
                           const float* y1, const float* st1, const float* x, int32_t ldx, const float* relu_mask,
                           int32_t ldm, float* dpre2, float* dpre1, float* dx, int32_t lddx, float* dg2, float* db2,
                           float* dg1, float* db1, float* dW2, int32_t ldw2, float* dbias2, float* dW1, int32_t ldw1,
                           float* dbias1, int32_t M, float* workspace, int64_t workspace_bytes, dgppo_reduce_desc* pending,
                           void* stream);
int64_t dgppo_head_bwd_workspace_bytes(void);
int32_t dgppo_head_bwd(const float* feat, int32_t ldf, const float* u, const float* dout, const float* W1, const float* W2,
                       float* dhs, float* dW1, int32_t ldw1, float* db1, float* dW2, int32_t ldw2, float* db2, int32_t M,
                       int32_t n_out, float* workspace, int64_t workspace_bytes, dgppo_reduce_desc* pending, void* stream);
int32_t dgppo_gru1_head_fwd(const float* gi, const float* Wh, const float* bhn, const float* h0, const float* W1,
                            const float* b1, const float* W2, const float* b2, float* hs, float* hprev, float* gates,
                            float* u, float* out, int32_t M, int32_t n_out, void* stream);
int64_t dgppo_dense_bwd_w_workspace_bytes(int32_t K, int32_t N);

#define DGPPO_GATHER_MAX 8
typedef struct dgppo_gather_desc {
  const void* src;
  void* dst;
  int64_t row_bytes, src_stride;
} dgppo_gather_desc;
int32_t dgppo_gather_rows(const dgppo_gather_desc* descs, int32_t n_desc, const int32_t* ids, int32_t n_ids, void* stream);

int32_t dgppo_graph_feats(const dgppo_env_cfg* cfg, const float* agent, int64_t agent_se, int64_t agent_st,
                          const float* goal, const float* obst, const float* hits, int64_t hits_se, int64_t hits_st,
                          const int32_t* env_ids, int32_t n_env, int32_t n_time, float* Xa, float* Xo, float* efeat,
                          float* emask, int32_t Fp, void* stream);

int32_t dgppo_graph_feats_sweep(const dgppo_env_cfg* cfg, const float* agent, int64_t agent_st, const float* goal,
                                const float* obst, const float* hits, int64_t hits_st, const float* ray_cos,
                                const float* ray_sin, const int32_t* frame_ids, int32_t n_frames, int32_t agent_id,
                                const float* xs, int32_t nx, const float* ys, int32_t ny, float* Xa, float* Xo,
                                float* efeat, float* emask, float* hits_out, int32_t Fp, void* stream);

int32_t dgppo_cost_sweep(const dgppo_env_cfg* cfg, const float* agent, int64_t agent_st, const float* obst, const float* hits,
                         int64_t hits_st, const float* ray_cos, const float* ray_sin, const int32_t* frame_ids,
                         int32_t n_frames, int32_t agent_id, const float* xs, int32_t nx, const float* ys, int32_t ny,
                         float* cost, float* hits_out, void* stream);

int32_t dgppo_graph_feats_action_sweep(const dgppo_env_cfg* cfg, const float* agent, int64_t agent_st, const float* goal,
                                       const float* obst, const float* hits, int64_t hits_st, const int32_t* frame_ids,
                                       int32_t n_frames, int32_t agent_id, const float* us, int32_t nu, const float* vs,
                                       int32_t nv, float* Xa, float* Xo, float* efeat, float* emask, int32_t Fp, void* stream);

int32_t dgppo_graph_feats_team_action_sweep(const dgppo_env_cfg* cfg, const float* agent, const float* next_agent,
                                            const float* goal, const float* obst, const float* next_hits, const float* a_pol,
                                            int32_t n_env, const float* us, int32_t nu, const float* vs, int32_t nv, float* Xa,
                                            float* Xo, float* efeat, float* emask, int32_t Fp, void* stream);

int32_t dgppo_shield_select(const float* Vh_next, const float* Vh_t, const float* a_pol, int32_t n_env, int32_t n_agents,
                            int32_t n_cost, const float* us, int32_t nu, const float* vs, int32_t nv, float dt, float alpha,
                            float margin, float* action, int32_t* index, int32_t* flag, float* h, void* stream);

int32_t dgppo_env_sweep_fork(const dgppo_env_cfg* cfg, const float* agent, int64_t agent_st, const float* goal,
                             const float* obst, const float* hits, int64_t hits_st, const float* ray_cos, const float* ray_sin,
                             const int32_t* frame_ids, int32_t n_frames, int32_t agent_id, const float* xs, int32_t nx,
                             const float* ys, int32_t ny, const float* carry, int64_t carry_st, int32_t HC, float* agent_out,
                             float* goal_out, float* obst_out, float* hits_out, float* carry_out, void* stream);

int32_t dgppo_constraint_return(const float* cost, int64_t cost_st, int32_t K, int32_t G, int32_t n_agents, int32_t nh,
                                float gamma, float one_minus_gamma, float* value, float* worst, void* stream);

int32_t dgppo_env_team_action_fork(const dgppo_env_cfg* cfg, const float* agent, const float* goal, const float* obst,
                                   const float* hits, const float* a_pol, const float* carry, int32_t HC, int32_t n_env,
                                   const float* us, int32_t nu, const float* vs, int32_t nv, float* agent_out, float* goal_out,
                                   float* obst_out, float* hits_out, float* action_out, float* carry_out, void* stream);

int32_t dgppo_lookahead_select(const float* cost, int64_t cost_st, int32_t K, int32_t n_env, int32_t n_agents, int32_t n_cost,
                               const float* a_pol, const float* us, int32_t nu, const float* vs, int32_t nv, float margin,
                               float* action, int32_t* index, int32_t* flag, float* s, void* stream);

int32_t dgppo_attn_fwd(const dgppo_env_cfg* cfg, int32_t F, int32_t H, int32_t Kp, const float* qt, const float* Xa,
                       const float* Xo, const float* efeat, const float* emask, float* zcat, float* attn, int32_t G,
                       void* stream);
int32_t dgppo_attn_bwd(const dgppo_env_cfg* cfg, int32_t F, int32_t H, int32_t Kp, const float* dzcat,
                       const float* attn, const float* qt, const float* Xa, const float* Xo, const float* efeat,
                       float* dqt, float* dXa, float* dXo, int32_t relu_xo, int32_t G, void* stream);
int32_t dgppo_attn_rows_supported(const dgppo_env_cfg* cfg, int32_t F, int32_t H);
int32_t dgppo_attn_fwd_rows(const dgppo_env_cfg* cfg, int32_t F, int32_t H, int32_t Kp, const float* qt, const float* Xa,
                            const float* Xo, const float* emask, float* zcat, float* attn, int32_t G, void* stream);
int32_t dgppo_attn_bwd_rows(const dgppo_env_cfg* cfg, int32_t F, int32_t H, int32_t Kp, const float* dzcat, const float* attn,
                            const float* qt, const float* emask, const float* Xa, const float* Xo, float* dqt, int32_t G,
                            void* stream);
int32_t dgppo_attn_xo_supported(const dgppo_env_cfg* cfg, int32_t F, int32_t H, int32_t Kp);
int32_t dgppo_attn_fwd_xo(const dgppo_env_cfg* cfg, int32_t F, int32_t H, int32_t Kp, const float* qt, const float* Xa,
                          const float* Xo_raw, const float* Wo, int32_t ldwo, const float* bo, const float* efeat,
                          const float* emask, float* zcat, float* attn, int32_t G, void* stream);
int32_t dgppo_attn_bwd_xo(const dgppo_env_cfg* cfg, int32_t F, int32_t H, int32_t Kp, const float* dzcat,
                          const float* attn, const float* qt, const float* Xa, const float* Xo_raw, const float* Wo,
                          int32_t ldwo, const float* bo, const float* efeat, float* dqt, float* dXa, float* dXo,
                          int32_t relu_xo, int32_t G, void* stream);
int64_t dgppo_attn_xo_workspace_bytes(int32_t G);
int32_t dgppo_attn_bwd_xo_dw(const dgppo_env_cfg* cfg, int32_t F, int32_t H, int32_t Kp, const float* dzcat,
                             const float* attn, const float* qt, const float* Xa, const float* Xo_raw, const float* Wo,
                             int32_t ldwo, const float* bo, const float* efeat, float* dqt, float* dXa, float* dWo,
                             int32_t lddwo, float* dbo, float* workspace, int64_t workspace_bytes, int32_t G, void* stream);

int32_t dgppo_gnn_prep(const float* Wq, const float* bq, const float* Wk, const float* Wv, const float* bv,
                       const float* We, const float* Wu, float* Mcat, float* cvec, float* Wout, int32_t F, int32_t Fp,
                       int32_t D, int32_t H, int32_t Kp, void* stream);
int32_t dgppo_gnn_unprep(const float* dMcat, const float* dcvec, const float* dWout, const float* Wq, const float* bq,
                         const float* Wk, float* dWq, float* dbq, float* dWk, float* dWv, float* dbv, float* dWe,
                         float* dWu, int32_t F, int32_t Fp, int32_t D, int32_t H, int32_t Kp, void* stream);

int32_t dgppo_ln_relu_fwd(const float* x, const float* gamma, const float* beta, float* y, float* stats, int32_t M,
                          void* stream);
int32_t dgppo_ln_relu_bwd(const float* x, const float* y, const float* stats, const float* gamma, const float* dy,
                          float* dx, float* dgamma, float* dbeta, int32_t M, void* stream);

int32_t dgppo_gru_fwd(const float* gi, const float* Wh, const float* bhn, const float* h0, float* hs, float* hprev,
                      float* gates, int32_t n_seq, int32_t T, int32_t n_inner, void* stream);
int32_t dgppo_gru_fwd_h0_blocks(const float* gi, const float* Wh, const float* bhn, const float* h0,
                                int32_t rows_per_block, int64_t block_stride, float* hs, float* hprev, float* gates,
                                int32_t n_seq, int32_t T, int32_t n_inner, void* stream);
int32_t dgppo_gru_bwd(const float* dhs, const float* Wh, const float* hprev, const float* gates, float* dgi,
                      float* dgh, int32_t n_seq, int32_t T, int32_t n_inner, void* stream);
int32_t dgppo_gru_bwd_dhn(const float* dhs, const float* Wh, const float* hprev, const float* gates, float* dgi,
                          float* dhn, int32_t n_seq, int32_t T, int32_t n_inner, void* stream);
int64_t dgppo_gru_bwd_w_workspace_bytes(void);
int32_t dgppo_gru_bwd_w(const float* x, int32_t ldx, const float* hprev, int32_t ldh, const float* dgi, const float* dhn,
                        float* dWi, int32_t ldwi, float* dbi, float* dWh, int32_t ldwh, float* dbhn, int32_t M,
                        float* workspace, int64_t workspace_bytes, dgppo_reduce_desc* pending, void* stream);
int32_t dgppo_gru_bwd_w_t1(const float* x, int32_t ldx, const float* h0, int32_t ldh, const float* dhs, const float* gates,
                           float* dgi, float* dWi, int32_t ldwi, float* dbi, float* dWh, int32_t ldwh, float* dbhn, int32_t M,
                           float* workspace, int64_t workspace_bytes, dgppo_reduce_desc* pending, void* stream);

int32_t dgppo_lstm_fwd(const float* zi, const float* Wh, const float* bh, const float* c0, const float* h0, float* cs,
                       float* hs, float* cprev, float* hprev, float* gates, int32_t n_seq, int32_t T, int32_t n_inner,
                       void* stream);
int32_t dgppo_lstm_bwd(const float* dhs, const float* Wh, const float* cprev, const float* gates, float* dz,
                       int32_t n_seq, int32_t T, int32_t n_inner, void* stream);

int32_t dgppo_policy_head(const float* ms, const float* eps, const float* action_in, float* action, float* log_pi,
                          float* entropy, int32_t rows, int32_t n_agents, int32_t mode, const float* log_pi_old,
                          const float* adv, float* dms, float* stats, float clip_eps, float coef_ent, void* stream);

int32_t dgppo_value_loss(const float* v, const float* target, float* dv, float* stats, int32_t count, void* stream);
int32_t dgppo_mean_agents(const float* x, float* y, int32_t G, int32_t n, int32_t D, int32_t backward,
                          const float* relu_mask, void* stream);
int32_t dgppo_relu_bwd(float* dy, const float* y, int64_t count, void* stream);


int32_t dgppo_gae(const float* costs, const float* rewards, const float* Vh, const float* Vl, const float* lam_pow,
                  float gamma, float one_minus_gamma, float one_minus_lam, float* Qh, float* Ql, int32_t B, int32_t T,
                  int32_t n, int32_t nh, void* stream);
int32_t dgppo_advantage(const float* Ql, const float* Vl, const float* Vh, float dt, float alpha, float cbf_eps,
                        float cbf_weight, float* adv, float* stats, int32_t B, int32_t T, int32_t n, int32_t nh,
                        void* stream);
int32_t dgppo_advantage_lagr(const float* Ql, const float* Vl, const float* Qh, const float* Vh, const float* lagr,
                             float* adv, float* Ah, int32_t B, int32_t T, int32_t n, int32_t nh, void* stream);
int32_t dgppo_lagr_update(const float* lp_new, const float* lp_old, const float* Vh, int64_t vh_env_stride,
                          const float* Ah, float* lagr, float* sums, int32_t n_env, int32_t T, int32_t n, int32_t nh,
                          float one_minus_gamma, float lr, void* stream);
int32_t dgppo_lagr_sums(const float* lp_new, const float* lp_old, const float* Vh, int64_t vh_env_stride, const float* Ah,
                        float* sums, int32_t n_env, int32_t T, int32_t n, int32_t nh, float one_minus_gamma, void* stream);
int32_t dgppo_lagr_apply(float* lagr, float* sums, int32_t count, int64_t rows_total, float lr, void* stream);
int32_t dgppo_relu_fwd(const float* x, float* out, int64_t count, void* stream);
int32_t dgppo_shaped_reward(const float* reward, const float* cost, float cost_weight, float* out, int64_t rows,
                            int32_t n, int32_t nh, void* stream);
#define DGPPO_OPT_PARTIALS 256
#define DGPPO_OPT_STATE_FLOATS (8 + 2 * DGPPO_OPT_PARTIALS)
int32_t dgppo_clip_adam_step(float* params, const float* grads, float* m, float* v, int64_t n, float* state, float lr,
                             float b1, float b2, float eps, float max_norm, float grad_scale, void* stream);

#define DGPPO_COMM_ID_BYTES 128
int32_t dgppo_comm_unique_id(uint8_t* id_out);
int32_t dgppo_comm_version(int32_t* version_out);
int32_t dgppo_comm_init(const uint8_t* id, int32_t rank, int32_t world, void** comm_out);
int32_t dgppo_comm_allreduce_sum_f32(void* comm, float* buf, int64_t count, void* stream);
int32_t dgppo_comm_destroy(void* comm);

#ifdef __cplusplus
}
#endif
#endif
```

Measured before the change: 4.647 million.

## Fuse query projection into BD attention forward kernel via MFMA

Adds attention forward variants that compute the per-head query projection (Xa·Mcat + cvec) inside the BD kernel with 16x16x4 MFMA, instead of running a separate dense_fwd and reading qt back from memory. In the persistent kernel the odd-head part of Mcat is staged in LDS, and the projected queries are written out only when training needs them. This removes a kernel launch and a round trip for qt on GNN layers 1 and up, at the cost of extra registers, LDS and MFMA work inside the attention kernel, which could reduce occupancy.

```diff
diff --git a/dgppo_amd/csrc/attn.hip b/dgppo_amd/csrc/attn.hip
--- a/dgppo_amd/csrc/attn.hip
+++ b/dgppo_amd/csrc/attn.hip
@@ -134,6 +134,55 @@
   return attn_launch(AttnFamily::BD, a, stream, true, "attn_bwd_xo");
 }
 
+static bool attn_q_ok(const Topo& t, int F, int H, int Kp) {
+  return attn_family(t, F, H, Kp, false, false) == AttnFamily::BD && attn_bd_q_shape(t, F, H);
+}
+extern "C" int32_t dgppo_attn_q_supported(const dgppo_env_cfg* cfg, int32_t F, int32_t H, int32_t Kp) {
+  AttnArgs a{};
+  if (F < 1 || H < 1 || attn_check(cfg, F, H, Kp, 0, a)) return 0;
+  return attn_q_ok(a.t, F, H, Kp) ? 1 : 0;
+}
+static int32_t attn_set_q(AttnArgs& a, const float* Xa, const float* Mcat, int ldm, const float* cvec, float* qt_out, const char* who) {
+  DGPPO_REQUIRE(attn_q_ok(a.t, a.F, a.H, a.Kp), "%s: no query-forming kernel for this shape (ask dgppo_attn_q_supported)", who);
+  DGPPO_REQUIRE(Mcat && cvec, "%s: NULL operand", who);
+  DGPPO_REQUIRE(ldm >= a.H * a.F && (ldm & 3) == 0, "%s: ldm=%d must be a multiple of 4 and >= H*F", who, ldm);
+  DGPPO_REQUIRE(((reinterpret_cast<uintptr_t>(Mcat) | reinterpret_cast<uintptr_t>(cvec) | reinterpret_cast<uintptr_t>(Xa) |
+                  reinterpret_cast<uintptr_t>(qt_out)) & 15) == 0, "%s: Xa, Mcat, cvec and qt_out must be 16-byte aligned", who);
+  a.Mcat = Mcat; a.ldm = ldm; a.cvec = cvec; a.qt_out = qt_out;
+  return 0;
+}
+extern "C" int32_t dgppo_attn_fwd_q(const dgppo_env_cfg* cfg, int32_t F, int32_t H, int32_t Kp, const float* Xa, const float* Mcat,
+                                    int32_t ldm, const float* cvec, const float* Xo, const float* efeat, const float* emask,
+                                    float* zcat, float* attn, float* qt_out, int32_t G, void* stream) {
+  AttnArgs a{};
+  int32_t rc = attn_check(cfg, F, H, Kp, G, a);
+  if (rc) return rc;
+  rc = attn_set_q(a, Xa, Mcat, ldm, cvec, qt_out, "attn_fwd_q");
+  if (rc) return rc;
+  if (G == 0) return 0;
+  DGPPO_REQUIRE(Xa && efeat && emask && zcat, "attn_fwd_q: NULL operand");
+  DGPPO_REQUIRE(a.t.Ns == a.t.n || Xo, "attn_fwd_q: Xo is NULL");
+  attn_set_fwd(a, nullptr, Xa, Xo, efeat, emask, zcat, attn);
+  return attn_launch(AttnFamily::BD, a, stream, false, "attn_fwd_q");
+}
+extern "C" int32_t dgppo_attn_fwd_xo_q(const dgppo_env_cfg* cfg, int32_t F, int32_t H, int32_t Kp, const float* Xa,
+                                       const float* Mcat, int32_t ldm, const float* cvec, const float* Xo_raw, const float* Wo,
+                                       int32_t ldwo, const float* bo, const float* efeat, const float* emask, float* zcat,
+                                       float* attn, float* qt_out, int32_t G, void* stream) {
+  AttnArgs a{};
+  int32_t rc = attn_check(cfg, F, H, Kp, G, a);
+  if (rc) return rc;
+  rc = attn_set_q(a, Xa, Mcat, ldm, cvec, qt_out, "attn_fwd_xo_q");
+  if (rc) return rc;
+  if (G == 0) return 0;
+  DGPPO_REQUIRE(Xa && Xo_raw && Wo && bo && efeat && emask && zcat, "attn_fwd_xo_q: NULL operand");
+  DGPPO_REQUIRE(ldwo >= 32, "attn_fwd_xo_q: ldwo=%d < 32", ldwo);
+  rc = attn_set_xo(a, Xo_raw, Wo, ldwo, bo, "attn_fwd_xo_q");
+  if (rc) return rc;
+  attn_set_fwd(a, nullptr, Xa, nullptr, efeat, emask, zcat, attn);
+  return attn_launch(AttnFamily::BD, a, stream, false, "attn_fwd_xo_q");
+}
+
 static bool attn_rows_ok(const dgppo_env_cfg& c, const Topo& t, int F, int H, int Kp) {
   return attn_slot8_rows_ok(c, t, F, H) && attn_family(t, F, H, Kp, false, false) == AttnFamily::SLOT8 &&
          attn_family(t, F, H, Kp, true, false) == AttnFamily::SLOT8;
diff --git a/dgppo_amd/csrc/attn_bd.hip b/dgppo_amd/csrc/attn_bd.hip
--- a/dgppo_amd/csrc/attn_bd.hip
+++ b/dgppo_amd/csrc/attn_bd.hip
@@ -113,6 +113,112 @@
   return b;
 }
 
+#define ABD_QM2 1024
+template <int QH> struct AbdQRegs {
+  static constexpr int N4 = QH / 2, N2 = QH & 1;
+  static constexpr int IMG = ABD_QM2 + QH * 32;
+  float4 m4[N4 ? N4 : 1][8], c4[N4 ? N4 : 1];
+  float2 m2[8], c2;
+};
+template <int QH>
+__device__ inline void abd_q_image(float* ql, const AttnArgs& a, int tid) {
+  using Q = AbdQRegs<QH>;
+  if constexpr (Q::N2 != 0) {
+#pragma unroll
+    for (int u = 0; u < 4; ++u) {
+      const int idx = u * 128 + tid, ks = idx >> 6, ln = idx & 63;
+      *reinterpret_cast<float2*>(ql + idx * 2) =
+          *reinterpret_cast<const float2*>(a.Mcat + (size_t)(ks * 4 + (ln >> 4)) * a.ldm + Q::N4 * 64 + (ln & 15) * 2);
+    }
+  }
+  if (tid < QH * 8) *reinterpret_cast<float4*>(ql + ABD_QM2 + tid * 4) = *reinterpret_cast<const float4*>(a.cvec + tid * 4);
+}
+template <int QH, bool MS = false>
+__device__ inline void abd_q_load(AbdQRegs<QH>& q, const AttnArgs& a, int li, int lq) {
+  using Q = AbdQRegs<QH>;
+#pragma unroll
+  for (int gi = 0; gi < Q::N4; ++gi) {
+#pragma unroll
+    for (int ks = 0; ks < 8; ++ks) q.m4[gi][ks] = *reinterpret_cast<const float4*>(a.Mcat + (size_t)(ks * 4 + lq) * a.ldm + gi * 64 + li * 4);
+    if constexpr (!MS) q.c4[gi] = *reinterpret_cast<const float4*>(a.cvec + gi * 64 + li * 4);
+  }
+  if constexpr (Q::N2 != 0 && !MS) {
+#pragma unroll
+    for (int ks = 0; ks < 8; ++ks) q.m2[ks] = *reinterpret_cast<const float2*>(a.Mcat + (size_t)(ks * 4 + lq) * a.ldm + Q::N4 * 64 + li * 2);
+    q.c2 = *reinterpret_cast<const float2*>(a.cvec + Q::N4 * 64 + li * 2);
+  }
+}
+template <int QH> __device__ inline int abd_q_bits(const AbdQRegs<QH>& q) {
+  using Q = AbdQRegs<QH>;
+  int b = 0;
+#pragma unroll
+  for (int gi = 0; gi < Q::N4; ++gi) {
+#pragma unroll
+    for (int ks = 0; ks < 8; ++ks) b |= f4bits(q.m4[gi][ks]);
+    b |= f4bits(q.c4[gi]);
+  }
+  if constexpr (Q::N2 != 0) {
+#pragma unroll
+    for (int ks = 0; ks < 8; ++ks) b |= __float_as_int(q.m2[ks].x) | __float_as_int(q.m2[ks].y);
+    b |= __float_as_int(q.c2.x) | __float_as_int(q.c2.y);
+  }
+  return b;
+}
+template <int QH, bool MS = false>
+__device__ inline void abd_q_emit(const AbdQRegs<QH>& q, const float* ql, const float* XS, float* QP, float* qo, int n, int lane) {
+  using Q = AbdQRegs<QH>;
+  const int li = lane & 15, lq = lane >> 4;
+  const int ar = (li & 7) < n ? (li & 7) : n - 1;
+  float av[8];
+#pragma unroll
+  for (int ks = 0; ks < 8; ++ks) av[ks] = XS[ar * ABD_XL + ks * 4 + lq];
+#pragma unroll
+  for (int gi = 0; gi < Q::N4; ++gi) {
+    f32x4g v[4];
+#pragma unroll
+    for (int t = 0; t < 4; ++t) {
+      v[t] = f32x4g{0.f, 0.f, 0.f, 0.f};
+#pragma unroll
+      for (int ks = 0; ks < 8; ++ks) v[t] = __builtin_amdgcn_mfma_f32_16x16x4f32(av[ks], f4e(q.m4[gi][ks])[t], v[t], 0, 0, 0);
+    }
+    if (lq < 2) {
+      const float4 c = MS ? *reinterpret_cast<const float4*>(ql + ABD_QM2 + gi * 64 + li * 4) : q.c4[gi];
+      const int h = gi * 2 + (li >> 3);
+#pragma unroll
+      for (int r = 0; r < 4; ++r)
+        *reinterpret_cast<float4*>(QP + ((lq * 4 + r) * 4 + h) * ABD_XL + (li & 7) * 4) =
+            make_float4(v[0][r] + c.x, v[1][r] + c.y, v[2][r] + c.z, v[3][r] + c.w);
+    }
+  }
+  if constexpr (Q::N2 != 0) {
+    float2 m2[8];
+#pragma unroll
+    for (int ks = 0; ks < 8; ++ks) m2[ks] = MS ? *reinterpret_cast<const float2*>(ql + (ks * 64 + lane) * 2) : q.m2[ks];
+    f32x4g v[2];
+#pragma unroll
+    for (int t = 0; t < 2; ++t) {
+      v[t] = f32x4g{0.f, 0.f, 0.f, 0.f};
+#pragma unroll
+      for (int ks = 0; ks < 8; ++ks) v[t] = __builtin_amdgcn_mfma_f32_16x16x4f32(av[ks], t == 0 ? m2[ks].x : m2[ks].y, v[t], 0, 0, 0);
+    }
+    if (lq < 2) {
+      const float2 c = MS ? *reinterpret_cast<const float2*>(ql + ABD_QM2 + Q::N4 * 64 + li * 2) : q.c2;
+#pragma unroll
+      for (int r = 0; r < 4; ++r)
+        *reinterpret_cast<float2*>(QP + ((lq * 4 + r) * 4 + QH - 1) * ABD_XL + li * 2) = make_float2(v[0][r] + c.x, v[1][r] + c.y);
+    }
+  }
+  if (qo != nullptr) {
+    const int il = lane >> 3, sub = lane & 7;
+#pragma unroll
+    for (int k = 0; k < 4; ++k) {
+      const int row = k * 8 + il, ri = row >> 2, rh = row & 3;
+      if (ri < n && rh < QH)
+        *reinterpret_cast<float4*>(qo + (ri * QH + rh) * 32 + sub * 4) = *reinterpret_cast<const float4*>(QP + row * ABD_XL + sub * 4);
+    }
+  }
+}
+
 template <int PS, bool HITS>
 __device__ __forceinline__ int abd_slot(const Topo& t, int NSH, int ic, int p, int sub) {
   if (HITS && p == PS) return t.n + t.gs + sub;
@@ -120,8 +226,9 @@
   return (j < NSH) ? slot_of(t, j, ic) : -1;
 }
 
-template <int PS, bool HITS, int AB, bool XOF>
+template <int PS, bool HITS, int AB, bool XOF, int QH = 0>
 __global__ void __launch_bounds__(128) attn_fwd_bd_kernel(AttnArgs a) {
+  static_assert(QH == 0 || AB == 1, "the query mode covers one agent batch");
   extern __shared__ float4 abd_sm[];
   using L = AbdLds<PS, HITS>;
   constexpr int F = 32, NSP = L::NSP, PC = L::PC, PL = L::PL, NPR = PS + (HITS ? 1 : 0), Wd = F + 4;
@@ -171,12 +278,16 @@
         vh[k] = Xo4[(t.ng + hb) * 8 + sub];
       }
     }
-#pragma unroll
-    for (int k = 0; k < 4; ++k) {
-      const int row = k * 8 + il;
-      int ri = ab * 8 + (row >> 2), rh = row & 3;
-      ri = ri < n ? ri : n - 1; rh = rh < H ? rh : H - 1;
-      vq[k] = qt4[(ri * H + rh) * 8 + sub];
+    AbdQRegs<QH ? QH : 1> qm;
+    if constexpr (QH != 0) abd_q_load<QH>(qm, a, li_, lq_);
+    if constexpr (QH == 0) {
+#pragma unroll
+      for (int k = 0; k < 4; ++k) {
+        const int row = k * 8 + il;
+        int ri = ab * 8 + (row >> 2), rh = row & 3;
+        ri = ri < n ? ri : n - 1; rh = rh < H ? rh : H - 1;
+        vq[k] = qt4[(ri * H + rh) * 8 + sub];
+      }
     }
     int slot[NPR];
     float mkv[NPR];
@@ -194,6 +305,7 @@
 #pragma unroll
     for (int p = 0; p < NPR; ++p) pin |= __float_as_int(mkv[p]) | f4bits(efv[p]);
     if constexpr (XOF) pin |= abd_xo_bits<GT>(xo, HITS);
+    if constexpr (QH != 0) pin |= abd_q_bits<QH>(qm);
     const int pin0 = opaque_zero(pin);
     if (ab == 0) {
 #pragma unroll
@@ -208,8 +320,12 @@
 #pragma unroll
       for (int k = 0; k < 8; ++k) *reinterpret_cast<float4*>(XH + pin0 + (k * 8 + il) * ABD_XL + k * 8 + sub * 4) = vh[k];
     }
-#pragma unroll
-    for (int k = 0; k < 4; ++k) *reinterpret_cast<float4*>(QP + pin0 + (k * 8 + il) * ABD_XL + sub * 4) = vq[k];
+    if constexpr (QH != 0)
+      abd_q_emit<QH>(qm, nullptr, XS + pin0, QP + pin0, a.qt_out ? a.qt_out + (size_t)g * n * QH * F : nullptr, n, lane);
+    if constexpr (QH == 0) {
+#pragma unroll
+      for (int k = 0; k < 4; ++k) *reinterpret_cast<float4*>(QP + pin0 + (k * 8 + il) * ABD_XL + sub * 4) = vq[k];
+    }
 #pragma unroll
     for (int p = 0; p < NPR; ++p) mkv[p] = (slot[p] >= 0) ? mkv[p] : 0.0f;
     if constexpr (HITS) {
@@ -323,14 +439,14 @@
   ASTAMP(6);
 }
 
-template <int PS, bool HITS, bool XOF>
+template <int PS, bool HITS, bool XOF, int QH = 0>
 struct AbdFwdRegs {
-  float4 vs[PS], vq[4], vh[(HITS && !XOF) ? 8 : 1];
+  float4 vs[PS], vq[QH ? 1 : 4], vh[(HITS && !XOF) ? 8 : 1];
   AbdXoRegs<(PS * 8 + 15) / 16> xo;
   float mkv[PS + (HITS ? 1 : 0)];
   float4 efv[PS + (HITS ? 1 : 0)];
 };
-template <int PS, bool HITS, bool XOF>
+template <int PS, bool HITS, bool XOF, int QH = 0>
 __global__ void __launch_bounds__(128) attn_fwd_bdp_kernel(AttnArgs a) {
   extern __shared__ float4 abd_sm[];
   using L = AbdLds<PS, HITS>;
@@ -339,6 +455,11 @@
   const int lane = threadIdx.x & 63, wave = threadIdx.x >> 6;
   int g = __builtin_amdgcn_readfirstlane(blockIdx.x * 2 + wave);
   const int stride = gridDim.x * 2;
+  const float* QL = reinterpret_cast<const float*>(abd_sm) + 2 * L::FWD;
+  if constexpr (QH != 0) {
+    abd_q_image<QH>(reinterpret_cast<float*>(abd_sm) + 2 * L::FWD, a, threadIdx.x);
+    __syncthreads();
+  }
   if (g >= a.G) return;
   const int n = t.n, S = t.S, Ns = t.Ns, H = a.H, Kp = a.Kp;
   const int NSH = HITS ? t.n + t.ng : Ns;
@@ -358,7 +479,9 @@
     slot[p] = live ? sl : -1;
     sc[p] = sl < 0 ? 0 : sl;
   }
-  using Regs = AbdFwdRegs<PS, HITS, XOF>;
+  using Regs = AbdFwdRegs<PS, HITS, XOF, QH>;
+  AbdQRegs<QH ? QH : 1> qm;
+  if constexpr (QH != 0) abd_q_load<QH, true>(qm, a, li_, lq_);
   auto load = [&](int gg, Regs& R) {
     const float4* Xa4 = reinterpret_cast<const float4*>(a.Xa + (size_t)gg * n * F);
     const float4* Xo4 = reinterpret_cast<const float4*>(a.Xo + (size_t)gg * (Ns - n) * F);
@@ -379,12 +502,17 @@
         R.vh[k] = Xo4[(t.ng + hb) * 8 + sub];
       }
     }
-#pragma unroll
-    for (int k = 0; k < 4; ++k) {
-      const int row = k * 8 + il;
-      int ri = row >> 2, rh = row & 3;
-      ri = ri < n ? ri : n - 1; rh = rh < H ? rh : H - 1;
-      R.vq[k] = qt4[(ri * H + rh) * 8 + sub];
+    if constexpr (QH == 0) {
+#pragma unroll
+      for (int k = 0; k < 4; ++k) {
+        const int row = k * 8 + il;
+        int ri = row >> 2, rh = row & 3;
+        ri = ri < n ? ri : n - 1; rh = rh < H ? rh : H - 1;
+        R.vq[k] = qt4[(ri * H + rh) * 8 + sub];
+      }
+    } else {
+      R.vq[0] = make_float4(0.f, 0.f, 0.f, 0.f);
+      if constexpr (!XOF) R.xo = AbdXoRegs<GT>{};
     }
     const float* mk = a.emask + (size_t)gg * n * S;
     const float4* ef4 = reinterpret_cast<const float4*>(a.efeat + (size_t)gg * n * S * 4);
@@ -411,8 +539,12 @@
 #pragma unroll
       for (int k = 0; k < 8; ++k) *reinterpret_cast<float4*>(XH + pin0 + (k * 8 + il) * ABD_XL + k * 8 + sub * 4) = R.vh[k];
     }
-#pragma unroll
-    for (int k = 0; k < 4; ++k) *reinterpret_cast<float4*>(QP + pin0 + (k * 8 + il) * ABD_XL + sub * 4) = R.vq[k];
+    if constexpr (QH != 0)
+      abd_q_emit<QH, true>(qm, QL, XS + pin0, QP + pin0, a.qt_out ? a.qt_out + (size_t)g * n * QH * F : nullptr, n, lane);
+    if constexpr (QH == 0) {
+#pragma unroll
+      for (int k = 0; k < 4; ++k) *reinterpret_cast<float4*>(QP + pin0 + (k * 8 + il) * ABD_XL + sub * 4) = R.vq[k];
+    }
 #pragma unroll
     for (int p = 0; p < NPR; ++p) R.mkv[p] = (slot[p] >= 0) ? R.mkv[p] : 0.0f;
     if constexpr (HITS) {
@@ -940,31 +1072,50 @@
   PS = (nsh + 7) / 8;
   return PS >= 1 && PS <= 4;
 }
-template <int PS, bool HITS, int AB, bool XOF>
+template <int PS, bool HITS, int AB, bool XOF, int QH = 0>
 static void launch_attn_bd_x(const AttnArgs& a, hipStream_t s, bool bwd) {
   using L = AbdLds<PS, HITS>;
-  if (bwd) { hipLaunchKernelGGL((attn_bwd_bd_kernel<PS, HITS, AB, XOF>), dim3(a.G), dim3(64), sizeof(float) * L::BWD, s, a); return; }
+  if constexpr (QH == 0) {
+    if (bwd) { hipLaunchKernelGGL((attn_bwd_bd_kernel<PS, HITS, AB, XOF>), dim3(a.G), dim3(64), sizeof(float) * L::BWD, s, a); return; }
+  }
   if constexpr (AB == 1) {
+    constexpr size_t smem_p = sizeof(float) * (2 * L::FWD + (QH ? AbdQRegs<QH ? QH : 1>::IMG : 0));
     static thread_local int cap = 0;
     if (cap == 0) {
       int per_cu = 0, dev = 0, cus = 256;
-      if (hipOccupancyMaxActiveBlocksPerMultiprocessor(&per_cu, reinterpret_cast<const void*>(&attn_fwd_bdp_kernel<PS, HITS, XOF>), 128,
-                                                       sizeof(float) * 2 * L::FWD) != hipSuccess || per_cu < 1) per_cu = 1;
+      if (hipOccupancyMaxActiveBlocksPerMultiprocessor(&per_cu, reinterpret_cast<const void*>(&attn_fwd_bdp_kernel<PS, HITS, XOF, QH>), 128,
+                                                       smem_p) != hipSuccess || per_cu < 1) per_cu = 1;
       if (hipGetDevice(&dev) != hipSuccess || hipDeviceGetAttribute(&cus, hipDeviceAttributeMultiprocessorCount, dev) != hipSuccess ||
           cus < 1) cus = 256;
       cap = per_cu * cus;
     }
     if ((a.G + 1) / 2 > 2 * cap) {
-      hipLaunchKernelGGL((attn_fwd_bdp_kernel<PS, HITS, XOF>), dim3(cap), dim3(128), sizeof(float) * 2 * L::FWD, s, a);
+      hipLaunchKernelGGL((attn_fwd_bdp_kernel<PS, HITS, XOF, QH>), dim3(cap), dim3(128), smem_p, s, a);
       return;
     }
   }
-  hipLaunchKernelGGL((attn_fwd_bd_kernel<PS, HITS, AB, XOF>), dim3((a.G + 1) / 2), dim3(128), sizeof(float) * 2 * L::FWD, s, a);
+  hipLaunchKernelGGL((attn_fwd_bd_kernel<PS, HITS, AB, XOF, QH>), dim3((a.G + 1) / 2), dim3(128), sizeof(float) * 2 * L::FWD, s, a);
+}
+#define ABD_QH 3
+bool attn_bd_q_shape(const Topo& t, int F, int H) {
+  int PS = 0;
+  bool hits = false;
+  return attn_bd_shape(t, F, H, PS, hits) && H == ABD_QH && t.n <= 8 && hits && PS <= 2;
 }
 template <int PS, bool HITS, int AB>
-static void launch_attn_bd_one(const AttnArgs& a, hipStream_t s, bool bwd) {
+static bool launch_attn_bd_one(const AttnArgs& a, hipStream_t s, bool bwd) {
+  if (a.Mcat != nullptr) {
+    if constexpr (AB == 1 && HITS && PS <= 2) {
+      if (bwd || a.H != ABD_QH) return false;
+      if (a.Xo_raw != nullptr) launch_attn_bd_x<PS, HITS, AB, true, ABD_QH>(a, s, false);
+      else launch_attn_bd_x<PS, HITS, AB, false, ABD_QH>(a, s, false);
+      return true;
+    }
+    return false;
+  }
   if (a.Xo_raw != nullptr) launch_attn_bd_x<PS, HITS, AB, true>(a, s, bwd);
   else launch_attn_bd_x<PS, HITS, AB, false>(a, s, bwd);
+  return true;
 }
 bool launch_attn_bd(const AttnArgs& a, hipStream_t s, bool bwd) {
   int PS = 0;
@@ -972,7 +1123,7 @@
   if (!attn_bd_shape(a.t, a.F, a.H, PS, hits)) return false;
   const int AB = (a.t.n + 7) / 8;
   switch ((PS * 2 + (hits ? 1 : 0)) * 4 + AB) {
-#define DGPPO_BD(P, HT, B) case ((P) * 2 + (HT)) * 4 + (B): launch_attn_bd_one<P, (HT) != 0, B>(a, s, bwd); return true;
+#define DGPPO_BD(P, HT, B) case ((P) * 2 + (HT)) * 4 + (B): return launch_attn_bd_one<P, (HT) != 0, B>(a, s, bwd);
     DGPPO_BD(1, 0, 1) DGPPO_BD(1, 1, 1) DGPPO_BD(2, 0, 1) DGPPO_BD(2, 1, 1) DGPPO_BD(2, 0, 2) DGPPO_BD(2, 1, 2)
     DGPPO_BD(3, 0, 1) DGPPO_BD(3, 1, 1) DGPPO_BD(3, 0, 2) DGPPO_BD(3, 1, 2)
     DGPPO_BD(4, 0, 1) DGPPO_BD(4, 1, 1) DGPPO_BD(4, 0, 2) DGPPO_BD(4, 1, 2)
diff --git a/dgppo_amd/csrc/nn_attn.h b/dgppo_amd/csrc/nn_attn.h
--- a/dgppo_amd/csrc/nn_attn.h
+++ b/dgppo_amd/csrc/nn_attn.h
@@ -39,6 +39,8 @@
   const float* Xo_raw; const float* Wo; const float* bo; int ldwo;
   float* dwo_slab;
   int TI;
+  const float* Mcat; const float* cvec; int ldm;
+  float* qt_out;
 };
 
 using f32x4g = __attribute__((ext_vector_type(4))) float;
@@ -90,6 +92,7 @@
 bool launch_attn_slot8(const AttnArgs& a, hipStream_t s, bool bwd);
 bool attn_bd_shape(const Topo& t, int F, int H, int& PS, bool& hits);
 bool launch_attn_bd(const AttnArgs& a, hipStream_t s, bool bwd);
+bool attn_bd_q_shape(const Topo& t, int F, int H);
 void launch_attn_xo_dw_reduce(const float* slab, int G, float* dWo, int lddwo, float* dbo, hipStream_t s);
 int32_t launch_attn_tiled(AttnArgs& a, hipStream_t s, bool bwd);
 #pragma GCC visibility pop
diff --git a/dgppo_amd/engine.py b/dgppo_amd/engine.py
--- a/dgppo_amd/engine.py
+++ b/dgppo_amd/engine.py
@@ -111,7 +111,7 @@
     def __init__(self, cfg: N.EnvCfg, hyper: Hyper, device, T: int = 128,
                  allreduce: Optional[Callable[[torch.Tensor], None]] = None, world: int = 1, prepass_graphs: int = 1 << 20,
                  use_graphs: bool = False, multi_stream: bool = False, algo: str = "dgppo", rank: int = 0,
-                 fused_step: bool = True, lean_attn0: bool = True):
+                 fused_step: bool = True, lean_attn0: bool = True, attn_q: bool = True):
         self.cfg, self.hp, self.device, self.T = cfg, hyper, device, T
         assert algo in ("dgppo", "informarl", "hcbfcrpo", "informarl_lagr"), algo
         self.algo = algo
@@ -120,6 +120,7 @@
         self._side_streams = None
         self.fused_step = bool(fused_step) and OE.act_step_feats_supported(cfg, nets.input_width(cfg), nets.H_HEADS)
         self.lean_attn0 = bool(lean_attn0)
+        self.attn_q = bool(attn_q)
         self._ro_cache: Dict[tuple, dict] = {}
         self._upd_graph: dict = {}
         self.n_cost = cfg.n_cost
@@ -142,7 +143,8 @@
         self.flat_grads = torch.zeros(tot + 4 * 8, device=device)
         self.n_reduced = tot + 3 * 8
         self.stats = self.flat_grads[tot:tot + 32].view(4, 8)
-        built = {k: nets.Net(kind, cfg, layers, n_out, device, grads=self.flat_grads[o:o + sz], lean_attn0=self.lean_attn0, **rnn_kw(k))
+        built = {k: nets.Net(kind, cfg, layers, n_out, device, grads=self.flat_grads[o:o + sz], lean_attn0=self.lean_attn0, attn_q=self.attn_q,
+                          **rnn_kw(k))
                  for (k, kind, layers, n_out), o, sz in zip(spec, offs, sizes)}
         if algo == "informarl_lagr":
             self.lagr = torch.full((cfg.n_agents, self.n_cost), float(hyper.lagr_init), device=device)
diff --git a/dgppo_amd/nets.py b/dgppo_amd/nets.py
--- a/dgppo_amd/nets.py
+++ b/dgppo_amd/nets.py
@@ -168,7 +168,7 @@
 class Net:
 
     def __init__(self, kind: str, cfg: N.EnvCfg, gnn_layers: int, n_out: int, device, grads: Optional[torch.Tensor] = None,
-                 rnn: str = "gru", rnn_layers: int = 1, lean_attn0: bool = True):
+                 rnn: str = "gru", rnn_layers: int = 1, lean_attn0: bool = True, attn_q: bool = True):
         assert kind in ("policy", "Vl", "Vh", "Vhg")
         self.kind, self.cfg, self.gnn_layers, self.n_out, self.device = kind, cfg, gnn_layers, n_out, device
         self.rnn, self.rnn_layers = rnn, (rnn_layers if rnn != "none" else 0)
@@ -191,6 +191,8 @@
             kp = _ceil4(fp + H_HEADS * (fp + 4) + 1)
             self.dims.append((f, fp, d, kp))
             f = d
+        self.attn_q = [bool(attn_q) and l >= 1 and K.attn_q_supported(cfg, fp, H_HEADS, kp)
+                       for l, (f, fp, d, kp) in enumerate(self.dims)]
         self.prep_layout = Layout()
         for l, (f, fp, d, kp) in enumerate(self.dims):
             self.prep_layout.add(f"gnn{l}.Mcat", fp, H_HEADS * fp)
@@ -251,15 +253,23 @@
                 assert tuple(qt0.shape) == (R, H_HEADS * fp), (tuple(qt0.shape), R, H_HEADS * fp)
                 qt = qt0
             else:
-                qt = A.get(f"{tag}.qt{l}", R, H_HEADS * fp)
-                K.dense_fwd(Xa, self.pp(f"gnn{l}.Mcat"), self.pp(f"gnn{l}.cvec"), qt)
+                fuse_q = self.attn_q[l]
+                qt = A.get(f"{tag}.qt{l}", R, H_HEADS * fp) if (train or not fuse_q) else None
+                if not fuse_q:
+                    K.dense_fwd(Xa, self.pp(f"gnn{l}.Mcat"), self.pp(f"gnn{l}.cvec"), qt)
+            q_ops = (Xa, self.pp(f"gnn{l}.Mcat"), self.pp(f"gnn{l}.cvec")) if (l >= 1 and self.attn_q[l]) else None
             zcat = A.get(f"{tag}.zcat{l}", R, kp)
             lean = l == 0 and self.lean_attn0 and feats.edges_from_rows
             attn = A.get(f"{tag}.attn{l}", R, cfg.fan_in, H_HEADS) if train and not lean else None
             if lean:
                 K.attn_fwd_rows(cfg, fp, H_HEADS, kp, qt, Xa, Xo if Ro > 0 else None, feats.emask, zcat, None, G)
+            elif xo_fused is not None and q_ops is not None:
+                K.attn_fwd_xo_q(cfg, fp, H_HEADS, kp, *q_ops, xo_fused[0], xo_fused[1], xo_fused[2], feats.efeat, feats.emask, zcat, attn,
+                                qt, G)
             elif xo_fused is not None:
                 K.attn_fwd_xo(cfg, fp, H_HEADS, kp, qt, Xa, xo_fused[0], xo_fused[1], xo_fused[2], feats.efeat, feats.emask, zcat, attn, G)
+            elif q_ops is not None:
+                K.attn_fwd_q(cfg, fp, H_HEADS, kp, *q_ops, Xo if Ro > 0 else None, feats.efeat, feats.emask, zcat, attn, qt, G)
             else:
                 K.attn_fwd(cfg, fp, H_HEADS, kp, qt, Xa, Xo if Ro > 0 else None, feats.efeat, feats.emask, zcat, attn, G)
             act[f"xo_fused{l}"] = xo_fused
diff --git a/dgppo_amd/ops_nn.py b/dgppo_amd/ops_nn.py
--- a/dgppo_amd/ops_nn.py
+++ b/dgppo_amd/ops_nn.py
@@ -648,6 +648,51 @@
     rc = N.lib().dgppo_attn_fwd_xo(C.byref(cfg), F, H, Kp, _p(qt), _p(Xa), _p(Xo_raw), _wo_ptr(Wo),
                                    _wo_ld(Wo), _p(bo), _p(efeat), _p(emask), _p(zcat), _p(attn), G, N.stream_ptr())
     N.check(rc, "dgppo_attn_fwd_xo")
+
+
+def attn_q_supported(cfg, F, H, Kp) -> bool:
+    return bool(N.lib().dgppo_attn_q_supported(C.byref(cfg), F, H, Kp))
+
+
+def _mcat_ld(Mcat, cvec, F, H):
+    if Mcat.dim() != 2 or Mcat.shape[0] != F or Mcat.shape[1] < H * F or Mcat.stride(1) != 1:
+        raise ValueError(f"Mcat must be [{F}, >= {H * F}] with contiguous rows, got {tuple(Mcat.shape)} strides {Mcat.stride()}")
+    N.expect_shape(cvec, (H * F,), "cvec")
+    return int(Mcat.stride(0))
+
+
+def attn_fwd_q(cfg, F, H, Kp, Xa, Mcat, cvec, Xo, efeat, emask, zcat, attn, qt_out, G):
+    n, S = cfg.n_agents, cfg.fan_in
+    N.expect_shape(Xa, (G * n, F), "Xa")
+    N.expect_shape(zcat, (G * n, Kp), "zcat")
+    ldm = _mcat_ld(Mcat, cvec, F, H)
+    if attn is not None:
+        N.expect_shape(attn, (G * n, S, H), "attn")
+    if qt_out is not None:
+        N.expect_shape(qt_out, (G * n, H * F), "qt_out")
+    FLOPS[0] += 2.0 * G * n * H * S * (2 * F + 4) + 2.0 * G * n * F * H * F
+    rc = N.lib().dgppo_attn_fwd_q(C.byref(cfg), F, H, Kp, _p(Xa), _wo_ptr(Mcat), ldm, _p(cvec), _p(Xo), _p(efeat), _p(emask),
+                                  _p(zcat), _p(attn), _p(qt_out), G, N.stream_ptr())
+    N.check(rc, "dgppo_attn_fwd_q")
+
+
+def attn_fwd_xo_q(cfg, F, H, Kp, Xa, Mcat, cvec, Xo_raw, Wo, bo, efeat, emask, zcat, attn, qt_out, G):
+    n, S = cfg.n_agents, cfg.fan_in
+    N.expect_shape(Xa, (G * n, F), "Xa")
+    N.expect_shape(zcat, (G * n, Kp), "zcat")
+    N.expect_shape(Xo_raw, (G * (cfg.num_nodes - 1 - n), 8), "Xo_raw")
+    N.expect_shape(bo, (32,), "bo")
+    ldm = _mcat_ld(Mcat, cvec, F, H)
+    if attn is not None:
+        N.expect_shape(attn, (G * n, S, H), "attn")
+    if qt_out is not None:
+        N.expect_shape(qt_out, (G * n, H * F), "qt_out")
+    FLOPS[0] += (2.0 * G * n * H * S * (2 * F + 4) + 2.0 * G * (cfg.num_nodes - 1 - n) * 8 * 32 +
+                 2.0 * G * n * F * H * F)
+    rc = N.lib().dgppo_attn_fwd_xo_q(C.byref(cfg), F, H, Kp, _p(Xa), _wo_ptr(Mcat), ldm, _p(cvec), _p(Xo_raw), _wo_ptr(Wo),
+                                     _wo_ld(Wo), _p(bo), _p(efeat), _p(emask), _p(zcat), _p(attn), _p(qt_out), G,
+                                     N.stream_ptr())
+    N.check(rc, "dgppo_attn_fwd_xo_q")
 
 
 def attn_bwd_xo(cfg, F, H, Kp, dzcat, attn, qt, Xa, Xo_raw, Wo, bo, efeat, dqt, dXa, dXo, G, relu_xo: bool = False):
diff --git a/include/dgppo_hip.h b/include/dgppo_hip.h
--- a/include/dgppo_hip.h
+++ b/include/dgppo_hip.h
@@ -250,6 +250,14 @@
                              const float* attn, const float* qt, const float* Xa, const float* Xo_raw, const float* Wo,
                              int32_t ldwo, const float* bo, const float* efeat, float* dqt, float* dXa, float* dWo,
                              int32_t lddwo, float* dbo, float* workspace, int64_t workspace_bytes, int32_t G, void* stream);
+int32_t dgppo_attn_q_supported(const dgppo_env_cfg* cfg, int32_t F, int32_t H, int32_t Kp);
+int32_t dgppo_attn_fwd_q(const dgppo_env_cfg* cfg, int32_t F, int32_t H, int32_t Kp, const float* Xa, const float* Mcat,
+                         int32_t ldm, const float* cvec, const float* Xo, const float* efeat, const float* emask, float* zcat,
+                         float* attn, float* qt_out, int32_t G, void* stream);
+int32_t dgppo_attn_fwd_xo_q(const dgppo_env_cfg* cfg, int32_t F, int32_t H, int32_t Kp, const float* Xa, const float* Mcat,
+                            int32_t ldm, const float* cvec, const float* Xo_raw, const float* Wo, int32_t ldwo, const float* bo,
+                            const float* efeat, const float* emask, float* zcat, float* attn, float* qt_out, int32_t G,
+                            void* stream);
 
 int32_t dgppo_gnn_prep(const float* Wq, const float* bq, const float* Wk, const float* Wv, const float* bv,
                        const float* We, const float* Wu, float* Mcat, float* cvec, float* Wout, int32_t F, int32_t Fp,
```

Result: no change. 4.689 million (median of 6 runs) (+0.9%).
